# skit-ai/N-Best-ASR-Transformer

Hardware: AMD Instinct MI355X
Metric: utterances/sec fine-tune (bert-base, seq128, n_best=5) (higher is better)
Workload: dtype bf16

## Files before the change

include/nbest_hip.h:

```cpp
#ifndef NBEST_HIP_H
#define NBEST_HIP_H

#include <stddef.h>
#include <stdint.h>

#ifdef __cplusplus
extern "C" {
#endif

#define NBEST_ABI_VERSION 1

enum { NBEST_OK = 0, NBEST_ERR_ARG = -1, NBEST_ERR_SHAPE = -2, NBEST_ERR_DTYPE = -3, NBEST_ERR_ALIGN = -4,
       NBEST_ERR_LAUNCH = -5, NBEST_ERR_WORKSPACE = -6 };
enum { NBEST_F32 = 0, NBEST_BF16 = 1 };

typedef void* nbest_stream_t;

int nbest_version(void);
int nbest_last_error(char* buf, size_t n);

int nbest_embed_ln_fwd(const int64_t* ids, const int64_t* seg, const int64_t* pos, const void* word,
                       const void* type, const void* ptab, const float* gamma, const float* beta, void* out,
                       float* stats, int64_t M, int H, float eps, int dtype, float drop_p, uint64_t seed,
                       uint32_t drop_stream, nbest_stream_t stream);
int nbest_embed_ln_bwd(const int64_t* ids, const int64_t* seg, const int64_t* pos, const int32_t* perm, const void* word,
                       const void* type, const void* ptab, const float* gamma, const float* stats,
                       const void* dout, float* dword, float* dtype_tab, float* dptab, float* dgamma,
                       float* dbeta, int B, int S, int H, int n_types, int dtype, int64_t word_pad_id,
                       int64_t pos_pad_id, int accumulate, int tables_accumulate, float drop_p, uint64_t seed,
                       uint32_t drop_stream, void* ws, size_t ws_bytes, nbest_stream_t stream);
size_t nbest_embed_bwd_ws_bytes(int64_t M, int64_t H);
int nbest_embed_ln_fwd_interp(const int64_t* ids, const int64_t* base_ids, const float* alpha, const int64_t* seg, const int64_t* pos,
                              const void* word, const void* type, const void* ptab, const float* gamma, const float* beta, void* out,
                              float* stats, int B, int S, int H, float eps, int dtype, float drop_p, uint64_t seed, uint32_t drop_stream,
                              nbest_stream_t stream);
int nbest_embed_attrib(const int64_t* ids, const int64_t* base_ids, const float* alpha, const int64_t* seg, const int64_t* pos,
                       const void* word, const void* type, const void* ptab, const float* gamma, const void* dhidden, float* attr,
                       int pairs, int m, int S, int H, float eps, int dtype, nbest_stream_t stream);

int nbest_rows_gather(const float* table, const int64_t* rows, int64_t n_rows, int64_t cap, int64_t* ids_out, float* vals_out, int H,
                      nbest_stream_t stream);
int nbest_rows_zero(float* table, const int64_t* ids, int64_t n, int H, nbest_stream_t stream);
int nbest_rows_add(float* table, const int64_t* ids, const float* vals, int64_t n, int H, nbest_stream_t stream);

enum {
  NBEST_EPI_NONE = 0,
  NBEST_EPI_BIAS = 1,
  NBEST_EPI_BIAS_GELU = 2,
  NBEST_EPI_BIAS_DROP_RES = 3,
  NBEST_EPI_DGELU = 4,
  NBEST_EPI_RES = 5,
  NBEST_EPI_F32_SPLITK = 6
};
typedef struct nbest_gemm_args {
  const void* A;
  const void* B;
  void* C;
  const float* bias;
  const void* R;
  void* U;
  void* ws;
  size_t ws_bytes;
  int64_t M, N, K;
  int64_t lda, ldb, ldc, ldr, ldu;
  int32_t trans_a, trans_b;
  int32_t epilogue;
  int32_t dtype;
  int32_t accumulate;
  float drop_p;
  uint32_t drop_stream;
  uint64_t seed;
  float* colsum_out;
  int32_t colsum_accumulate;
  int32_t flags;
  const void* B_packed;
  int32_t b_pack_bn;
  int32_t pad_;
} nbest_gemm_args;
#define NBEST_GEMM_DEFER_REDUCE 1
size_t nbest_gemm_ws_bytes(const nbest_gemm_args* a);
int nbest_gemm(const nbest_gemm_args* a, nbest_stream_t stream);

size_t nbest_wgrad_pair_ws_bytes(const nbest_gemm_args* a, const nbest_gemm_args* b);
int nbest_wgrad_pair(const nbest_gemm_args* a, const nbest_gemm_args* b, nbest_stream_t stream);

typedef struct nbest_gemm_fp8_args {
  const void* A;
  const void* B;
  void* C;
  const float* bias;
  const void* R;
  void* U;
  void* C8;
  int64_t M, N, K;
  int64_t lda, ldb, ldc, ldr, ldu, ldc8;
  int32_t epilogue;
  float out_scale;
  float drop_p;
  uint32_t drop_stream;
  uint64_t seed;
  const float* out_scale_dev;
  const uint32_t* a_amax;
  const uint32_t* c8_amax_prev;
  uint32_t* c8_amax_new;
  float* colsum_out;
  int32_t colsum_accumulate;
  int32_t pad;
  void* ws;
  size_t ws_bytes;
  const void* B_packed;
  int32_t b_pack_bn;
  int32_t pad3;
} nbest_gemm_fp8_args;
size_t nbest_gemm_fp8_ws_bytes(const nbest_gemm_fp8_args* a);
int nbest_gemm_fp8(const nbest_gemm_fp8_args* a, nbest_stream_t stream);
size_t nbest_wgrad_fp8_ws_bytes(int64_t M, int64_t N, int64_t K);
int nbest_wgrad_fp8(const void* dY8, const void* X8, float* dW, int64_t M, int64_t N, int64_t K, int64_t lda, int64_t ldb,
                    int64_t ldc, const uint32_t* a_amax, const uint32_t* x_amax, int accumulate, void* ws, size_t ws_bytes,
                    nbest_stream_t stream);
size_t nbest_wgrad_fp8_pair_ws_bytes(int64_t Ma, int64_t Mb, int64_t N, int64_t K);
int nbest_wgrad_fp8_pair(const void* dY8a, const void* X8a, float* dWa, int64_t Ma, int64_t lda_a, int64_t ldb_a, int64_t ldc_a,
                         const uint32_t* amax_a, const uint32_t* xamax_a, const void* dY8b, const void* X8b, float* dWb, int64_t Mb,
                         int64_t lda_b, int64_t ldb_b, int64_t ldc_b, const uint32_t* amax_b, const uint32_t* xamax_b, int64_t N, int64_t K,
                         int accumulate, void* ws, size_t ws_bytes, nbest_stream_t stream);
int nbest_cast_bf16_to_fp8(const void* src, void* dst, int64_t n, nbest_stream_t stream);

int nbest_attention_fwd(const void* qkv, const uint8_t* key_mask, void* ctx, float* lse, int B, int S,
                        int heads, int d, int dtype, float drop_p, uint64_t seed, uint32_t drop_stream,
                        nbest_stream_t stream);
int nbest_attention_cls_fwd(const void* q, int64_t ldq, const void* kv, int64_t ldkv, const uint8_t* key_mask, void* ctx,
                            int64_t ldctx, int B, int S, int heads, int d, int dtype, nbest_stream_t stream);
int nbest_attention_probs(const void* qkv, const uint8_t* key_mask, const float* lse, float* probs, int B, int S, int heads, int d,
                          int dtype, nbest_stream_t stream);
int nbest_attention_cls_probs(const void* q, int64_t ldq, const void* kv, int64_t ldkv, const uint8_t* key_mask, float* probs,
                              int64_t ldp, int B, int S, int heads, int d, int dtype, nbest_stream_t stream);
size_t nbest_attention_bwd_ws_bytes(int B, int S, int heads);
int nbest_attention_bwd(const void* qkv, const uint8_t* key_mask, const void* ctx, const void* dctx,
                        const float* lse, void* dqkv, float* dbias, int accumulate, void* ws, size_t ws_bytes,
                        int B, int S, int heads, int d, int dtype, float drop_p, uint64_t seed,
                        uint32_t drop_stream, nbest_stream_t stream);

size_t nbest_attention_keep_bytes(int B, int S, int heads);
int nbest_attention_fwd_keep(const void* qkv, const uint8_t* key_mask, void* ctx, float* lse, int B, int S,
                             int heads, int d, int dtype, float drop_p, uint64_t seed, uint32_t drop_stream,
                             void* keep, nbest_stream_t stream);
int nbest_attention_bwd_keep(const void* qkv, const uint8_t* key_mask, const void* ctx, const void* dctx,
                             const float* lse, void* dqkv, float* dbias, int accumulate, void* ws, size_t ws_bytes,
                             int B, int S, int heads, int d, int dtype, float drop_p, uint64_t seed,
                             uint32_t drop_stream, const void* keep, nbest_stream_t stream);

int nbest_layernorm_fwd(const void* x, const float* gamma, const float* beta, void* y, float* stats,
                        int64_t M, int H, float eps, int dtype, nbest_stream_t stream);
int nbest_layernorm_bwd(const void* dy, const void* x, const float* stats, const float* gamma, void* dx,
                        void* dx_drop, float* dgamma, float* dbeta, float* dbias, int64_t M, int H, int dtype,
                        int accumulate, float drop_p, uint64_t seed, uint32_t drop_stream, void* ws,
                        size_t ws_bytes, nbest_stream_t stream);
size_t nbest_rowred_ws_bytes(int64_t M, int64_t N);
int nbest_colsum(const void* X, float* out, int64_t M, int64_t N, int64_t ld, int dtype, int accumulate,
                 void* ws, size_t ws_bytes, nbest_stream_t stream);

typedef struct nbest_label_space {
  int32_t n_top, n_bottom, n_rows;
  const int32_t* bottom_off;
  const int32_t* bottom_ids;
  const int32_t* head_row;
} nbest_label_space;
size_t nbest_heads_ws_bytes(int B, int R, int H);
int nbest_stc_heads(const void* hidden, int64_t cls_stride, const float* Wh, const float* bh,
                    const nbest_label_space* ls, const float* labels, float* top, float* bott, float* final_scores,
                    float* loss_parts, float* dcls, float* dWh, float* dbh, int B, int H, int dtype,
                    int need_grad, int accumulate, float drop_p, uint64_t seed, uint32_t drop_stream, void* ws,
                    size_t ws_bytes, nbest_stream_t stream);
int nbest_stc_heads_vjp(const float* Wh, const nbest_label_space* ls, const float* top, const float* bott, const float* dtop,
                        const float* dbott, const float* dfin, float* dcls, float* dWh, float* dbh, int B, int H, int accumulate,
                        float drop_p, uint64_t seed, uint32_t drop_stream, void* ws, size_t ws_bytes, nbest_stream_t stream);

int nbest_cls_mse(const void* hidden_a, int64_t stride_a, const void* hidden_t, int64_t stride_t, float* loss,
                  float* da, float* dt, int B, int H, int dtype, float grad_scale, nbest_stream_t stream);

int nbest_cls_grad_scatter(const float* dcls, void* dhidden, int B, int S, int H, int dtype,
                           nbest_stream_t stream);

int nbest_stc_decode(const float* top, const float* bott, const nbest_label_space* ls,
                     const uint8_t* none_flag, int32_t* pred, int B, nbest_stream_t stream);
int nbest_stream_stamp(int32_t* flag, int32_t value, nbest_stream_t stream);

typedef struct nbest_tensor_desc {
  int64_t offset;
  int64_t numel;
  float lr;
  float wd;
  int32_t active;
  int32_t block_start;
} nbest_tensor_desc;
int nbest_bertadam_chunk(void);
int nbest_bertadam_step(float* p, float* g, float* m, float* v, void* p_lowp, const nbest_tensor_desc* descs,
                        int n_tensors, int n_blocks, float lr_mult, float b1, float b2, float eps,
                        float max_grad_norm, void* ws, size_t ws_bytes, nbest_stream_t stream);
int nbest_bertadam_norms(const float* g, const nbest_tensor_desc* descs, int n_tensors, int n_blocks, int blk_lo, int blk_hi,
                         float* partial, nbest_stream_t stream);
int nbest_bertadam_update(float* p, const float* g, float* m, float* v, void* p_lowp, const nbest_tensor_desc* descs,
                          int n_tensors, int n_blocks, int blk_lo, int blk_hi, const float* partial, float* coef,
                          float lr_mult, float b1, float b2, float eps, float max_grad_norm, nbest_stream_t stream);
enum { NBEST_ADAM_L2 = 0, NBEST_ADAMW = 1 };
int nbest_adam_clip_coef(const float* partial, int n_partial, float max_grad_norm, float* clip, nbest_stream_t stream);
int nbest_adam_update(int mode, float* p, const float* g, float* m, float* v, void* p_lowp, const nbest_tensor_desc* descs,
                      int n_tensors, int n_blocks, int blk_lo, int blk_hi, const float* clip, float lr_mult, float bc1,
                      float bc2_sqrt, double b1, double b2, float eps, nbest_stream_t stream);
int nbest_adam_step(int mode, float* p, float* g, float* m, float* v, void* p_lowp, const nbest_tensor_desc* descs,
                    int n_tensors, int n_blocks, float lr_mult, float bc1, float bc2_sqrt, double b1, double b2, float eps,
                    float max_grad_norm, void* ws, size_t ws_bytes, nbest_stream_t stream);
typedef struct nbest_matrix_desc {
  int64_t offset;
  int32_t rows, cols;
  int32_t tile_start, pad;
} nbest_matrix_desc;
#define NBEST_AMAX_TENSOR_WORDS 1024
int nbest_fp8_amax_fold(void* slots, void* out, int32_t n_tensors, nbest_stream_t stream);
int nbest_quantize_weights_fp8(const float* master, void* w8, void* w8t, const nbest_matrix_desc* descs, int n_matrices,
                               int n_tiles, float* inv_scale, void* ws, size_t ws_bytes, nbest_stream_t stream);
int nbest_transpose_weights(const void* src, void* dst, const nbest_matrix_desc* descs, int n_matrices, int n_tiles,
                            nbest_stream_t stream);
int nbest_pack_bn(int64_t N);
int nbest_pack_bn_fp8(int64_t N, int64_t K);
int nbest_pack_weights_fp8(const void* src, void* dst, const nbest_matrix_desc* descs, int n_matrices, int n_stages, nbest_stream_t stream);
int nbest_pack_weights(const void* src, void* dst, const nbest_matrix_desc* descs, int n_matrices, int n_stages, nbest_stream_t stream);
int nbest_cast_f32_to_bf16(const float* src, void* dst, int64_t n, nbest_stream_t stream);

typedef struct nbest_layer_offsets {
  int64_t wqkv, bqkv, wo, bo, ln1_g, ln1_b, w1, b1, w2, b2, ln2_g, ln2_b;
} nbest_layer_offsets;
typedef struct nbest_encoder_desc {
  int32_t dtype, B, S, H, L, heads, F;
  int32_t vocab, max_pos, n_types;
  float ln_eps, hidden_drop, attn_drop;
  int64_t word_pad_id, pos_pad_id;
  int64_t off_word, off_pos, off_type, off_emb_ln_g, off_emb_ln_b;
  const nbest_layer_offsets* layers_host;
  uint64_t seed;
  uint32_t drop_stream_base;
  int32_t wgrad_events_n;
  void** wgrad_events;
  const void* w8;
  const float* w8_inv_scale;
  const void* w8t;
  const uint32_t* gamax_prev;
  uint32_t* gamax_new;
  int32_t fp8_bwd;
  int32_t pad2;
  const void* wpk;
  const void* wpkt;
  const void* w8p;
  const void* w8tp;
  const int32_t* word_perm;
  const uint32_t* aamax_prev;
  uint32_t* aamax_new;
  int32_t fp8_act;
  int32_t pad4;
  int32_t first_trainable;
  int32_t no_input_grad;
  const uint8_t* wgrad_skip_host;
  const int64_t* base_ids;
  const float* alpha;
  int32_t no_param_grad;
  int32_t pad5;
} nbest_encoder_desc;
size_t nbest_encoder_act_bytes(const nbest_encoder_desc* d);
int nbest_encoder_act_view(const nbest_encoder_desc* d, void* act, int layer, void** qkv, float** lse);
size_t nbest_encoder_ws_bytes(const nbest_encoder_desc* d);
int nbest_encoder_wgrad_launches_per_layer(const nbest_encoder_desc* d);
int nbest_encoder_forward(const nbest_encoder_desc* d, const void* wts, const float* prm, const int64_t* ids,
                          const int64_t* seg, const int64_t* pos, const uint8_t* key_mask, void* act,
                          size_t act_bytes, void* ws, size_t ws_bytes, void** hidden_out, nbest_stream_t stream);
int nbest_encoder_backward(const nbest_encoder_desc* d, const void* wts, const void* wts_t, const float* prm, float* grad,
                           const int64_t* ids, const int64_t* seg, const int64_t* pos, const uint8_t* key_mask,
                           void* act, size_t act_bytes, void* dhidden, void* ws, size_t ws_bytes, int accumulate,
                           int layer_begin, int layer_end, int with_embeddings, nbest_stream_t stream);

size_t nbest_encoder_infer_ws_bytes(const nbest_encoder_desc* d);
int nbest_encoder_infer(const nbest_encoder_desc* d, const void* wts, const float* prm, const int64_t* ids, const int64_t* seg,
                        const int64_t* pos, const uint8_t* key_mask, void* ws, size_t ws_bytes, void* cls_out, nbest_stream_t stream);
int nbest_encoder_infer_attn(const nbest_encoder_desc* d, const void* wts, const float* prm, const int64_t* ids, const int64_t* seg,
                             const int64_t* pos, const uint8_t* key_mask, void* ws, size_t ws_bytes, void* cls_out, float* cls_attn,
                             nbest_stream_t stream);

#ifdef __cplusplus
}
#endif
#endif
```

n-best-asr-transformer_amd/csrc/encoder.hip:

```cpp
#include <algorithm>

#include "common.h"

namespace {

static inline size_t al(size_t x) { return (x + 255) & ~(size_t)255; }
static inline size_t take(size_t& o, size_t bytes) { const size_t at = o; o += bytes; return at; }

struct Sizes {
  size_t esz, MH, MF, M3H, MH8, MF8, st, lse;
  int64_t M;
};

static Sizes sizes(const nbest_encoder_desc* d) {
  Sizes z;
  z.esz = d->dtype == NBEST_BF16 ? 2 : 4;
  z.M = (int64_t)d->B * d->S;
  const size_t MHe = (size_t)z.M * d->H, MFe = (size_t)z.M * d->F;
  z.MH = al(MHe * z.esz); z.MF = al(MFe * z.esz); z.M3H = al(3 * MHe * z.esz);
  z.MH8 = al(MHe); z.MF8 = al(MFe);
  z.st = al((size_t)z.M * 2 * sizeof(float));
  z.lse = al((size_t)d->B * d->heads * d->S * sizeof(float));
  return z;
}

struct ActLayout {
  size_t X, emb_stats, layer0, layer_stride;
  size_t o_qkv, o_ctx, o_lse, o_r1, o_st1, o_x1, o_u, o_hact, o_r2, o_st2;
  size_t o_x8, o_ctx8, o_x18, o_h8;
  size_t o_keep, keep_bytes;
  size_t total;
  int K;
};

static int first_trainable(const nbest_encoder_desc* d) { return d->first_trainable < 0 ? 0 : (d->first_trainable > d->L ? d->L : d->first_trainable); }

static ActLayout act_layout(const nbest_encoder_desc* d, const Sizes& z) {
  ActLayout a;
  const bool bf16 = d->dtype == NBEST_BF16;
  a.K = first_trainable(d);
  size_t o = 0, p = 0;
  a.X = take(o, (size_t)(d->L + 1 - a.K) * z.MH);
  a.emb_stats = take(o, a.K ? 0 : z.st);
  a.layer0 = o;
  a.o_qkv = take(p, z.M3H); a.o_ctx = take(p, z.MH); a.o_lse = take(p, z.lse);
  a.o_r1 = take(p, z.MH); a.o_st1 = take(p, z.st); a.o_x1 = take(p, z.MH);
  a.o_u = take(p, bf16 ? z.MF8 : z.MF);
  a.o_hact = take(p, z.MF); a.o_r2 = take(p, z.MH); a.o_st2 = take(p, z.st);
  a.keep_bytes = bf16 ? nbest_internal_attention_keep_bytes(d->B, d->S, d->heads) : 0;
  a.o_keep = take(p, al(a.keep_bytes));
  a.o_x8 = a.o_ctx8 = a.o_x18 = a.o_h8 = 0;
  if (d->w8) {
    a.o_x8 = take(p, z.MH8); a.o_ctx8 = take(p, z.MH8); a.o_x18 = take(p, z.MH8); a.o_h8 = take(p, z.MF8);
  }
  a.layer_stride = p;
  a.total = o + (size_t)(d->L - a.K) * p;
  return a;
}

struct WsLayout {
  size_t dR, dRd, dB1, dctx, dBig, dqkv, red, slab, slab_bytes, red_bytes, emb, emb_bytes, f8, f8_bytes, total;
  size_t fz_x0, fz_x1, fz_emb_stats, fz_lse, fz_st1, fz_st2, fz_u;
};

static nbest_gemm_args wgrad_args(int dtype, int64_t rows, int64_t cols, int64_t tokens) {
  nbest_gemm_args g = {};
  g.M = rows; g.N = cols; g.K = tokens; g.lda = rows; g.ldb = cols; g.ldc = cols;
  g.trans_a = g.trans_b = 1; g.epilogue = NBEST_EPI_F32_SPLITK; g.dtype = dtype;
  return g;
}

static size_t wgrad_pair_bytes(const nbest_encoder_desc* d, bool fp8) {
  const int64_t H = d->H, M = (int64_t)d->B * d->S;
  if (fp8) return nbest_wgrad_fp8_pair_ws_bytes(3 * H, H, H, M);
  const nbest_gemm_args g1 = wgrad_args(NBEST_BF16, 3 * H, H, M), g2 = wgrad_args(NBEST_BF16, H, H, M);
  return nbest_wgrad_pair_ws_bytes(&g1, &g2);
}

static size_t max_splitk_bytes(const nbest_encoder_desc* d, int64_t M) {
  size_t mx = 0;
  const int64_t shapes[4][2] = {{3 * (int64_t)d->H, d->H}, {d->H, d->H}, {d->F, d->H}, {d->H, d->F}};
  for (int i = 0; i < 4; ++i) {
    const nbest_gemm_args g = wgrad_args(d->dtype, shapes[i][0], shapes[i][1], M);
    mx = std::max(mx, nbest_gemm_ws_bytes(&g));
    if (d->dtype == NBEST_BF16 && shapes[i][0] % 256 == 0 && shapes[i][1] % 256 == 0)
      mx = std::max(mx, nbest_wgrad_fp8_ws_bytes(shapes[i][0], shapes[i][1], M));
  }
  if (d->dtype == NBEST_BF16) mx = std::max(mx, std::max(wgrad_pair_bytes(d, false), wgrad_pair_bytes(d, true)));
  return mx;
}

static bool wgrad_paired(const nbest_encoder_desc* d, bool f8b) { return d->dtype == NBEST_BF16 && wgrad_pair_bytes(d, f8b) > 0; }

static WsLayout ws_layout(const nbest_encoder_desc* d, const Sizes& z) {
  WsLayout w;
  const int64_t M = z.M;
  size_t o = 0;
  w.dR = take(o, z.MH); w.dRd = take(o, z.MH); w.dB1 = take(o, z.MH); w.dctx = take(o, z.MH);
  w.dBig = take(o, z.MF); w.dqkv = take(o, z.M3H);
  const int64_t maxN = d->F > 3 * d->H ? d->F : 3 * d->H;
  w.red_bytes = al(nbest_rowred_ws_bytes(M, maxN));
  w.red_bytes = std::max(w.red_bytes, al(nbest_attention_bwd_ws_bytes(d->B, d->S, d->heads)));
  w.red_bytes = std::max(w.red_bytes, al((size_t)((M + 127) / 128) * 2 * d->F * sizeof(float)));
  w.red = take(o, 4 * w.red_bytes);
  w.slab_bytes = al(max_splitk_bytes(d, M));
  w.slab = take(o, w.slab_bytes);
  w.emb_bytes = al(nbest_embed_bwd_ws_bytes(M, d->H));
  w.emb = take(o, w.emb_bytes);
  w.f8_bytes = (d->dtype == NBEST_BF16) ? 4 * z.MH8 + z.MF8 : 0;
  w.f8 = take(o, w.f8_bytes);
  w.fz_x0 = w.fz_x1 = w.fz_emb_stats = w.fz_lse = w.fz_st1 = w.fz_st2 = w.fz_u = o;
  if (first_trainable(d) > 0) {
    w.fz_x0 = take(o, z.MH); w.fz_x1 = take(o, z.MH); w.fz_emb_stats = take(o, z.st);
    w.fz_lse = take(o, z.lse); w.fz_st1 = take(o, z.st); w.fz_st2 = take(o, z.st);
    w.fz_u = take(o, d->w8 ? z.MF8 : 0);
  }
  w.total = o;
  return w;
}

static bool fp8_forward_active(const nbest_encoder_desc* d) {
  return d->dtype == NBEST_BF16 && d->w8 && d->w8_inv_scale && d->fp8_act && d->aamax_prev;
}
static bool fp8_backward_active(const nbest_encoder_desc* d) {
  return fp8_forward_active(d) && d->fp8_bwd && d->w8t && d->gamax_prev && d->gamax_new;
}

static int check_desc(const nbest_encoder_desc* d) {
  NB_CHECK(d && d->layers_host, NBEST_ERR_ARG, "encoder: null descriptor");
  NB_CHECK(d->dtype == NBEST_F32 || d->dtype == NBEST_BF16, NBEST_ERR_DTYPE, "encoder: bad dtype %d", d->dtype);
  NB_CHECK(d->B > 0 && d->S > 0 && d->L > 0 && d->heads > 0, NBEST_ERR_SHAPE, "encoder: bad shape");
  NB_CHECK(d->H == d->heads * 64, NBEST_ERR_SHAPE, "encoder: hidden %d != heads %d x 64", d->H, d->heads);
  NB_CHECK(d->S + (d->pos_pad_id >= 0 ? (int)d->pos_pad_id + 1 : 0) <= d->max_pos, NBEST_ERR_SHAPE,
           "encoder: S=%d does not fit the position table (%d rows)", d->S, d->max_pos);
  NB_CHECK(d->S <= 512, NBEST_ERR_SHAPE, "encoder: S=%d > 512", d->S);
  if (d->dtype == NBEST_BF16)
    NB_CHECK(d->H % 128 == 0 && d->F % 128 == 0, NBEST_ERR_SHAPE, "encoder(bf16): H and F must be multiples of 128");
  if (d->w8) NB_CHECK(d->dtype == NBEST_BF16 && d->w8_inv_scale && d->H % 256 == 0 && d->H <= 1024 && d->F % 256 == 0, NBEST_ERR_SHAPE,
                      "encoder(fp8 forward): needs the bf16 path, inverse scales and H, F multiples of 256");
  NB_CHECK(0 <= d->first_trainable && d->first_trainable <= d->L, NBEST_ERR_ARG, "encoder: first_trainable %d outside [0, L=%d]",
           d->first_trainable, d->L);
  NB_CHECK(!d->base_ids == !d->alpha, NBEST_ERR_ARG, "encoder: interpolated embeddings need both base_ids and alpha (or neither)");
  return NBEST_OK;
}

struct Ptrs {
  const char* wts;
  const float* prm;
  size_t esz;
  const void* W(int64_t off) const { return wts + (size_t)off * esz; }
  const float* P(int64_t off) const { return prm + off; }
};

#define RUN(x) do { int rc__ = (x); if (rc__) return rc__; } while (0)

static nbest_gemm_args gemm_nt(int dtype, const void* A, const void* B, void* C, int64_t M, int64_t N, int64_t K) {
  nbest_gemm_args g = {};
  g.A = A; g.B = B; g.C = C; g.dtype = dtype;
  g.M = M; g.N = N; g.K = K; g.lda = K; g.ldb = K; g.ldc = N;
  return g;
}

static void use_packed(nbest_gemm_args& g, const void* arena, int64_t off) {
  if (!arena || g.dtype != NBEST_BF16 || g.trans_a || g.trans_b) return;
  g.B_packed = (const char*)arena + off * 2;
  g.b_pack_bn = nbest_pack_bn(g.N);
}
static void use_packed(nbest_gemm_fp8_args& g, const void* arena, int64_t off) {
  if (!arena) return;
  g.B_packed = (const uint8_t*)arena + off;
  g.b_pack_bn = nbest_pack_bn_fp8(g.N, g.K);
}

struct GemmPass {
  int dtype; int64_t M; nbest_stream_t stream;
  uint64_t seed;
  Ptrs W; const void* packed; bool b_kn;
  bool fp8; const void *w8, *w8_packed; const float* inv_scale; const uint32_t* amax_prev; uint32_t* amax_new;
  void* colsum_ws; size_t colsum_ws_bytes; int accumulate;
};
struct GemmOp {
  const void* A; const uint8_t* A8; int a_idx;
  int64_t w_off; int mat;
  void* C; int64_t N, K; int epilogue;
  const float* bias;
  const void* R; float drop_p; uint32_t drop_stream;
  void* U; float* colsum;
  uint8_t* C8; int c_idx;
};

static int layer_gemm(const GemmPass& c, const GemmOp& o) {
  if (c.fp8) {
    nbest_gemm_fp8_args g = {};
    g.A = o.A8; g.B = (const uint8_t*)c.w8 + o.w_off; g.C = o.C; g.bias = o.bias; g.R = o.R; g.U = o.U; g.C8 = o.C8;
    g.M = c.M; g.N = o.N; g.K = o.K;
    g.lda = g.ldb = o.K; g.ldc = g.ldr = g.ldu = g.ldc8 = o.N;
    use_packed(g, c.w8_packed, o.w_off);
    g.epilogue = o.epilogue; g.out_scale = 1.f; g.out_scale_dev = c.inv_scale + o.mat;
    g.drop_p = o.drop_p; g.drop_stream = o.drop_stream; g.seed = c.seed;
    g.a_amax = c.amax_prev + o.a_idx;
    if (o.C8) {
      g.c8_amax_prev = c.amax_prev + o.c_idx;
      g.c8_amax_new = c.amax_new ? c.amax_new + (int64_t)o.c_idx * NBEST_AMAX_TENSOR_WORDS : nullptr;
    }
    g.colsum_out = o.colsum; g.colsum_accumulate = c.accumulate; g.ws = c.colsum_ws; g.ws_bytes = c.colsum_ws_bytes;
    return nbest_gemm_fp8(&g, c.stream);
  }
  nbest_gemm_args g = gemm_nt(c.dtype, o.A, c.W.W(o.w_off), o.C, c.M, o.N, o.K);
  if (c.b_kn) { g.trans_b = 1; g.ldb = o.N; }
  g.epilogue = o.epilogue; g.bias = o.bias;
  if (o.R) { g.R = o.R; g.ldr = o.N; }
  if (o.epilogue == NBEST_EPI_BIAS_DROP_RES) { g.drop_p = o.drop_p; g.drop_stream = o.drop_stream; g.seed = c.seed; }
  if (o.epilogue == NBEST_EPI_BIAS_GELU || o.epilogue == NBEST_EPI_DGELU) { g.U = o.U; g.ldu = o.N; }
  if (o.epilogue == NBEST_EPI_DGELU) {
    g.colsum_out = o.colsum; g.colsum_accumulate = g.accumulate = c.accumulate; g.ws = c.colsum_ws; g.ws_bytes = c.colsum_ws_bytes;
  }
  use_packed(g, c.packed, o.w_off);
  return nbest_gemm(&g, c.stream);
}

struct LayerBufs {
  void *qkv, *ctx, *r1, *x1, *u, *hact, *r2;
  float *lse, *st1, *st2;
  uint32_t* keep;
  uint8_t *x8, *ctx8, *x18, *h8;
};

static LayerBufs stashed_layer(const nbest_encoder_desc* d, const ActLayout& a, void* act, int l) {
  char* Lb = (char*)act + a.layer0 + (size_t)(l - a.K) * a.layer_stride;
  LayerBufs b = {};
  b.qkv = Lb + a.o_qkv; b.ctx = Lb + a.o_ctx; b.lse = (float*)(Lb + a.o_lse);
  b.r1 = Lb + a.o_r1; b.st1 = (float*)(Lb + a.o_st1); b.x1 = Lb + a.o_x1;
  b.u = Lb + a.o_u; b.r2 = Lb + a.o_r2; b.st2 = (float*)(Lb + a.o_st2);
  b.hact = fp8_backward_active(d) ? nullptr : Lb + a.o_hact;
  if (a.keep_bytes && d->attn_drop > 0.f) b.keep = (uint32_t*)(Lb + a.o_keep);
  if (fp8_forward_active(d)) {
    b.x8 = (uint8_t*)(Lb + a.o_x8); b.ctx8 = (uint8_t*)(Lb + a.o_ctx8);
    b.x18 = (uint8_t*)(Lb + a.o_x18); b.h8 = (uint8_t*)(Lb + a.o_h8);
  }
  return b;
}

static LayerBufs frozen_layer(const nbest_encoder_desc* d, const WsLayout& w, const Sizes& z, void* ws) {
  char* W = (char*)ws;
  const bool f8 = fp8_forward_active(d);
  LayerBufs b = {};
  b.qkv = W + w.dqkv; b.ctx = W + w.dctx; b.lse = (float*)(W + w.fz_lse);
  b.r1 = W + w.dR; b.st1 = (float*)(W + w.fz_st1); b.x1 = W + w.dRd;
  b.r2 = W + w.dB1; b.st2 = (float*)(W + w.fz_st2);
  b.u = f8 ? W + w.fz_u : nullptr; b.hact = f8 ? nullptr : W + w.dBig;
  if (f8) { b.x8 = (uint8_t*)(W + w.f8); b.ctx8 = b.x8 + z.MH8; b.x18 = b.ctx8 + z.MH8; b.h8 = b.x18 + z.MH8; }
  return b;
}

struct Fwd {
  const nbest_encoder_desc* d;
  GemmPass g;
  const uint8_t* key_mask;
  bool arec;
  const uint32_t* AP(int idx) const { return g.fp8 ? d->aamax_prev + idx : nullptr; }
  uint32_t* AN(int idx) const { return (g.fp8 && arec) ? d->aamax_new + (int64_t)idx * NBEST_AMAX_TENSOR_WORDS : nullptr; }
  int calib(const void* t, int64_t n, int idx) const {
    if (!arec || g.fp8) return NBEST_OK;
    return nbest_internal_amax_bf16(t, n, d->aamax_new + (int64_t)idx * NBEST_AMAX_TENSOR_WORDS, (hipStream_t)g.stream);
  }
};

static Fwd make_fwd(const nbest_encoder_desc* d, const void* wts, const float* prm, const Sizes& z, const uint8_t* key_mask,
                    nbest_stream_t stream) {
  const GemmPass g = {d->dtype, z.M, stream, d->seed, Ptrs{(const char*)wts, prm, z.esz}, d->wpk, false, fp8_forward_active(d),
                      d->w8, d->w8p, d->w8_inv_scale, d->aamax_prev, d->aamax_new, nullptr, 0, 0};
  return Fwd{d, g, key_mask, d->w8 && d->aamax_new && d->dtype == NBEST_BF16};
}

static int layer_forward(const Fwd& c, int l, const void* xin, void* xout, const LayerBufs& b, uint8_t* x8_next, float* cls_probs) {
  const nbest_encoder_desc* d = c.d;
  const nbest_layer_offsets& o = d->layers_host[l];
  const Ptrs& P = c.g.W;
  const nbest_stream_t stream = c.g.stream;
  const int64_t M = c.g.M;
  const int H = d->H, F = d->F, dt = d->dtype, t = 4 * l;
  const uint32_t s0 = d->drop_stream_base + 1 + 4 * l;
  if (c.g.fp8 && l == 0)
    RUN(nbest_internal_cast_bf16_to_fp8(xin, b.x8, M * H, c.AP(0), c.AN(0), (hipStream_t)stream));
  const GemmOp wqkv = {xin, b.x8, t + 0, o.wqkv, t + 0, b.qkv, 3 * H, H, NBEST_EPI_BIAS, P.P(o.bqkv)};
  RUN(layer_gemm(c.g, wqkv));
  if (cls_probs)
    RUN(nbest_internal_attention_cls_probs(b.qkv, (int64_t)d->S * H * 3, (const char*)b.qkv + H * P.esz, 3 * H, c.key_mask, cls_probs, d->S,
                                           d->B, d->S, d->heads, 64, dt, stream));
  RUN(c.calib(xin, M * H, t + 0));
  RUN(nbest_internal_attention_fwd8(b.qkv, c.key_mask, b.ctx, b.ctx8, b.lse, d->B, d->S, d->heads, 64, dt, d->attn_drop, d->seed, s0 + 0,
                                    stream, b.keep, c.AP(t + 1), c.AN(t + 1)));
  RUN(c.calib(b.ctx, M * H, t + 1));
  GemmOp wo = {b.ctx, b.ctx8, t + 1, o.wo, t + 1, b.r1, H, H, NBEST_EPI_BIAS_DROP_RES, P.P(o.bo)};
  wo.R = xin; wo.drop_p = d->hidden_drop; wo.drop_stream = s0 + 1;
  RUN(layer_gemm(c.g, wo));
  RUN(nbest_internal_layernorm_fwd8(b.r1, P.P(o.ln1_g), P.P(o.ln1_b), b.x1, b.x18, b.st1, M, H, d->ln_eps, dt, stream, c.AP(t + 2), c.AN(t + 2)));
  RUN(c.calib(b.x1, M * H, t + 2));
  GemmOp w1 = {b.x1, b.x18, t + 2, o.w1, t + 2, b.hact, F, H, NBEST_EPI_BIAS_GELU, P.P(o.b1)};
  w1.U = b.u; w1.C8 = b.h8; w1.c_idx = t + 3;
  RUN(layer_gemm(c.g, w1));
  GemmOp w2 = {b.hact, b.h8, t + 3, o.w2, t + 3, b.r2, H, F, NBEST_EPI_BIAS_DROP_RES, P.P(o.b2)};
  w2.R = b.x1; w2.drop_p = d->hidden_drop; w2.drop_stream = s0 + 2;
  RUN(layer_gemm(c.g, w2));
  RUN(c.calib(b.hact, M * F, t + 3));
  RUN(nbest_internal_layernorm_fwd8(b.r2, P.P(o.ln2_g), P.P(o.ln2_b), xout, x8_next, b.st2, M, H, d->ln_eps, dt, stream,
                                    x8_next ? c.AP(t + 4) : nullptr, x8_next ? c.AN(t + 4) : nullptr));
  return NBEST_OK;
}

}

extern "C" size_t nbest_encoder_act_bytes(const nbest_encoder_desc* d) { return d ? act_layout(d, sizes(d)).total : 0; }

extern "C" int nbest_encoder_act_view(const nbest_encoder_desc* d, void* act, int layer, void** qkv, float** lse) {
  RUN(check_desc(d));
  NB_CHECK(act && qkv && lse, NBEST_ERR_ARG, "encoder_act_view: null pointer");
  NB_CHECK(0 <= layer && layer < d->L, NBEST_ERR_ARG, "encoder_act_view: layer %d outside [0, L=%d)", layer, d->L);
  const ActLayout a = act_layout(d, sizes(d));
  NB_CHECK(layer >= a.K, NBEST_ERR_ARG, "encoder_act_view: layer %d < first_trainable %d (frozen layers are not stashed)", layer, a.K);
  const LayerBufs b = stashed_layer(d, a, act, layer);
  *qkv = b.qkv; *lse = b.lse;
  return NBEST_OK;
}
extern "C" size_t nbest_encoder_ws_bytes(const nbest_encoder_desc* d) { return d ? ws_layout(d, sizes(d)).total : 0; }
extern "C" int nbest_encoder_wgrad_launches_per_layer(const nbest_encoder_desc* d) {
  return d ? (wgrad_paired(d, fp8_backward_active(d)) ? 3 : 4) : 0;
}

extern "C" int nbest_encoder_forward(const nbest_encoder_desc* d, const void* wts, const float* prm, const int64_t* ids,
                                     const int64_t* seg, const int64_t* pos, const uint8_t* key_mask, void* act, size_t act_bytes,
                                     void* ws, size_t ws_bytes, void** hidden_out, nbest_stream_t stream) {
  RUN(check_desc(d));
  NB_CHECK(wts && prm && ids && pos && key_mask && act, NBEST_ERR_ARG, "encoder_forward: null pointer");
  const Sizes z = sizes(d);
  const ActLayout a = act_layout(d, z);
  NB_CHECK(act_bytes >= a.total, NBEST_ERR_WORKSPACE, "encoder_forward: activation stash too small (%zu < %zu)", act_bytes, a.total);
  const Fwd c = make_fwd(d, wts, prm, z, key_mask, stream);
  const WsLayout wl = ws_layout(d, z);
  const int FT = a.K;
  if (c.g.fp8 || FT > 0)
    NB_CHECK(ws && ws_bytes >= wl.total, NBEST_ERR_WORKSPACE, "encoder_forward(%s): workspace too small (%zu < %zu)",
             FT > 0 ? "first_trainable > 0" : "fp8", ws_bytes, wl.total);
  const Ptrs& P = c.g.W;
  char *A = (char*)act, *W = (char*)ws;
  const int H = d->H, dt = d->dtype;
  auto X = [&](int l) { return l >= FT ? (void*)(A + a.X + (size_t)(l - FT) * z.MH) : (void*)(W + ((l & 1) ? wl.fz_x1 : wl.fz_x0)); };
  auto bufs = [&](int l) { return l >= FT ? stashed_layer(d, a, act, l) : frozen_layer(d, wl, z, ws); };

  float* emb_stats = (float*)(FT > 0 ? W + wl.fz_emb_stats : A + a.emb_stats);
  if (d->base_ids)
    RUN(nbest_embed_ln_fwd_interp(ids, d->base_ids, d->alpha, seg, pos, P.W(d->off_word), P.W(d->off_type), P.W(d->off_pos),
                                  P.P(d->off_emb_ln_g), P.P(d->off_emb_ln_b), X(0), emb_stats, d->B, d->S, H, d->ln_eps, dt,
                                  d->hidden_drop, d->seed, d->drop_stream_base, (hipStream_t)stream));
  else
    RUN(nbest_embed_ln_fwd(ids, seg, pos, P.W(d->off_word), P.W(d->off_type), P.W(d->off_pos), P.P(d->off_emb_ln_g),
                           P.P(d->off_emb_ln_b), X(0), emb_stats, z.M, H, d->ln_eps, dt, d->hidden_drop, d->seed, d->drop_stream_base,
                           (hipStream_t)stream));
  for (int l = 0; l < d->L; ++l) {
    uint8_t* x8_next = (l + 1 < d->L) ? bufs(l + 1).x8 : nullptr;
    RUN(layer_forward(c, l, X(l), X(l + 1), bufs(l), x8_next, nullptr));
  }
  if (hidden_out) *hidden_out = X(d->L);
  return NBEST_OK;
}

namespace {
struct WGrad {
  const void *dY, *X;
  const uint8_t *dY8, *X8;
  int64_t w_off, rows, cols;
  int g_idx, a_idx;
};
}

extern "C" int nbest_encoder_backward(const nbest_encoder_desc* d, const void* wts, const void* wts_t, const float* prm, float* grad,
                                      const int64_t* ids, const int64_t* seg, const int64_t* pos, const uint8_t* key_mask,
                                      void* act, size_t act_bytes, void* dhidden, void* ws, size_t ws_bytes, int accumulate,
                                      int layer_begin, int layer_end, int with_embeddings, nbest_stream_t stream) {
  RUN(check_desc(d));
  NB_CHECK(0 <= layer_begin && layer_begin <= layer_end && layer_end <= d->L, NBEST_ERR_ARG, "encoder_backward: bad layer range");
  const bool npg = d->no_param_grad != 0;
  NB_CHECK(!npg || (!with_embeddings && d->first_trainable == 0 && !d->no_input_grad && !d->w8), NBEST_ERR_ARG,
           "encoder_backward: no_param_grad refuses with_embeddings (%d), first_trainable > 0 (%d), no_input_grad (%d) and the fp8 "
           "forward (w8): it forms the input gradient only, of a full stash", with_embeddings, d->first_trainable, d->no_input_grad);
  NB_CHECK(wts && prm && (grad || npg) && ids && pos && key_mask && act && dhidden && ws, NBEST_ERR_ARG, "encoder_backward: null pointer");
  NB_CHECK(!with_embeddings || d->word_perm, NBEST_ERR_ARG, "encoder_backward: desc.word_perm (stable argsort of this pass's ids) is required");
  NB_CHECK(layer_begin >= d->first_trainable, NBEST_ERR_ARG, "encoder_backward: layer_begin %d < first_trainable %d (those layers are not stashed)",
           layer_begin, d->first_trainable);
  NB_CHECK(!with_embeddings || (d->first_trainable == 0 && !d->no_input_grad), NBEST_ERR_ARG,
           "encoder_backward: with_embeddings needs first_trainable == 0 and no_input_grad == 0");
  const Sizes z = sizes(d);
  const ActLayout a = act_layout(d, z);
  const WsLayout w = ws_layout(d, z);
  NB_CHECK(act_bytes >= a.total, NBEST_ERR_WORKSPACE, "encoder_backward: activation stash too small");
  NB_CHECK(ws_bytes >= w.total, NBEST_ERR_WORKSPACE, "encoder_backward: workspace too small (%zu < %zu)", ws_bytes, w.total);
  hipStream_t st = (hipStream_t)stream;
  const Ptrs P{(const char*)wts, prm, z.esz};
  const bool wt = (wts_t != nullptr);
  char *A = (char*)act, *W = (char*)ws;
  const int64_t M = z.M;
  const int H = d->H, F = d->F, dt = d->dtype;
  const int FT = a.K;
  auto X = [&](int l) { return (void*)(A + a.X + (size_t)(l - FT) * z.MH); };
  auto G = [&](int64_t off) { return grad + off; };
  auto GP = [&](int64_t off) -> float* { return npg ? nullptr : grad + off; };
  auto skip = [&](int l, int j) -> bool { return npg || (d->wgrad_skip_host && d->wgrad_skip_host[4 * l + j]); };
  void* dA = dhidden; void* dR = W + w.dR;
  const bool hdrop = d->hidden_drop > 0.f;
  void* dRd = hdrop ? (void*)(W + w.dRd) : dR;
  void* dB1 = W + w.dB1; void* dctx = W + w.dctx; void* dBig = W + w.dBig; void* dqkv = W + w.dqkv;
  void* red = W + w.red; void* slab = W + w.slab;
  void* red1 = W + w.red + w.red_bytes; void* red2 = W + w.red + 2 * w.red_bytes; void* red3 = W + w.red + 3 * w.red_bytes;
  const bool f8b = fp8_backward_active(d);
  const bool paired = wgrad_paired(d, f8b);
  int ev_i = (paired ? 3 : 4) * (d->L - layer_end);
  auto stamp = [&](int which) {
    if (d->wgrad_events && 2 * ev_i + which < d->wgrad_events_n) (void)hipEventRecord((hipEvent_t)d->wgrad_events[2 * ev_i + which], st);
    ev_i += which;
  };

  const bool rec = !npg && d->gamax_new && dt == NBEST_BF16;
  uint8_t* dqkv8 = f8b ? (uint8_t*)W + w.f8 : nullptr;
  uint8_t* dBig8 = f8b ? dqkv8 + 3 * z.MH8 : nullptr;
  uint8_t* dRd8 = f8b ? dBig8 + z.MF8 : nullptr;
  auto GN = [&](int idx) { return d->gamax_new + (int64_t)idx * NBEST_AMAX_TENSOR_WORDS; };
  auto fg = [&](uint8_t* out8, int idx) -> Fp8Grad {
    if (!rec) return Fp8Grad{nullptr, nullptr, nullptr};
    return Fp8Grad{f8b ? out8 : nullptr, f8b ? d->gamax_prev + idx : nullptr, GN(idx)};
  };
  const GemmPass dg = {dt, M, stream, 0, Ptrs{(const char*)(wt ? wts_t : wts), prm, z.esz}, wt ? d->wpkt : nullptr, !wt, f8b,
                       d->w8t, d->w8tp, d->w8_inv_scale, d->gamax_prev, d->gamax_new, red1, w.red_bytes, accumulate};
  auto wgrad = [&](int l, const WGrad* wg, int j, int j2) -> int {
    const WGrad* p = skip(l, j) ? nullptr : wg + j;
    const WGrad* q = (j2 >= 0 && !skip(l, j2)) ? wg + j2 : nullptr;
    if (!p) { p = q; q = nullptr; }
    stamp(0);
    if (p && f8b) {
      const uint32_t *gp = d->gamax_prev, *ap = d->aamax_prev;
      if (q)
        RUN(nbest_wgrad_fp8_pair(p->dY8, p->X8, G(p->w_off), p->rows, p->rows, p->cols, p->cols, gp + p->g_idx, ap + p->a_idx, q->dY8, q->X8,
                                 G(q->w_off), q->rows, q->rows, q->cols, q->cols, gp + q->g_idx, ap + q->a_idx, p->cols, M, accumulate, slab,
                                 w.slab_bytes, stream));
      else
        RUN(nbest_wgrad_fp8(p->dY8, p->X8, G(p->w_off), p->rows, p->cols, M, p->rows, p->cols, p->cols, gp + p->g_idx, ap + p->a_idx,
                            accumulate, slab, w.slab_bytes, stream));
    } else if (p) {
      auto args = [&](const WGrad* x) {
        nbest_gemm_args g = wgrad_args(dt, x->rows, x->cols, M);
        g.A = x->dY; g.B = x->X; g.C = G(x->w_off); g.accumulate = accumulate;
        return g;
      };
      nbest_gemm_args g1 = args(p), g2 = args(q ? q : p);
      g1.ws = slab; g1.ws_bytes = w.slab_bytes;
      RUN(q ? nbest_wgrad_pair(&g1, &g2, stream) : nbest_gemm(&g1, stream));
    }
    stamp(1);
    return NBEST_OK;
  };

  struct BatchGuard { ~BatchGuard() { nbest_internal_rowred_batch_abort(); } } batch_guard;
  for (int l = layer_end - 1; l >= layer_begin; --l) {
    const nbest_layer_offsets& o = d->layers_host[l];
    const LayerBufs b = stashed_layer(d, a, act, l);
    const bool input_grad = !(d->no_input_grad && l == FT);
    const int t = 4 * l;
    const uint32_t s0 = d->drop_stream_base + 1 + 4 * l;
    const WGrad wg[4] = {{dqkv, X(l), dqkv8, b.x8, o.wqkv, 3 * H, H, t + 3, t + 0},
                         {dRd, b.ctx, dRd8, b.ctx8, o.wo, H, H, t + 2, t + 1},
                         {dBig, b.x1, dBig8, b.x18, o.w1, F, H, t + 1, t + 2},
                         {dRd, b.hact, dRd8, b.h8, o.w2, H, F, t + 0, t + 3}};
    if (!npg) nbest_internal_rowred_batch_begin();
    RUN(nbest_internal_layernorm_bwd8(dA, b.r2, b.st2, P.P(o.ln2_g), dR, (hdrop && !f8b) ? dRd : nullptr, GP(o.ln2_g), GP(o.ln2_b), GP(o.b2), M, H,
                                      dt, accumulate, d->hidden_drop, d->seed, s0 + 2, red, w.red_bytes, stream, fg(dRd8, t + 0)));
    GemmOp dw2 = {dRd, dRd8, t + 0, o.w2, t + 3, f8b ? nullptr : dBig, F, H, NBEST_EPI_DGELU};
    dw2.U = b.u; dw2.colsum = GP(o.b1); dw2.C8 = dBig8; dw2.c_idx = t + 1;
    RUN(layer_gemm(dg, dw2));
    if (rec && !f8b) RUN(nbest_internal_amax_bf16(dBig, M * F, GN(t + 1), st));
    RUN(wgrad(l, wg, 3, -1));
    GemmOp dw1 = {dBig, dBig8, t + 1, o.w1, t + 2, dB1, H, F, NBEST_EPI_RES};
    dw1.R = dR;
    RUN(layer_gemm(dg, dw1));
    RUN(wgrad(l, wg, 2, -1));
    RUN(nbest_internal_layernorm_bwd8(dB1, b.r1, b.st1, P.P(o.ln1_g), dR, (hdrop && !f8b) ? dRd : nullptr, GP(o.ln1_g), GP(o.ln1_b), GP(o.bo), M, H,
                                      dt, accumulate, d->hidden_drop, d->seed, s0 + 1, red2, w.red_bytes, stream, fg(dRd8, t + 2)));
    const GemmOp dwo = {dRd, dRd8, t + 2, o.wo, t + 1, dctx, H, H, NBEST_EPI_NONE};
    RUN(layer_gemm(dg, dwo));
    if (!paired) RUN(wgrad(l, wg, 1, -1));
    RUN(nbest_internal_attention_bwd8(b.qkv, key_mask, b.ctx, dctx, b.lse, f8b ? nullptr : dqkv, GP(o.bqkv), accumulate, red3, w.red_bytes, d->B, d->S,
                                      d->heads, 64, dt, d->attn_drop, d->seed, s0 + 0, stream, fg(dqkv8, t + 3), b.keep));
    if (input_grad) {
      GemmOp dwqkv = {dqkv, dqkv8, t + 3, o.wqkv, t + 0, dA, H, 3 * H, NBEST_EPI_RES};
      dwqkv.R = dR;
      RUN(layer_gemm(dg, dwqkv));
    }
    RUN(wgrad(l, wg, 0, paired ? 1 : -1));
    if (!npg) RUN(nbest_internal_rowred_batch_flush(st));
  }
  if (!with_embeddings) return NBEST_OK;
  if (!accumulate) {
    hipError_t e = hipMemsetAsync(G(d->off_word), 0, (size_t)d->vocab * H * sizeof(float), st);
    if (e == hipSuccess) e = hipMemsetAsync(G(d->off_pos), 0, (size_t)d->max_pos * H * sizeof(float), st);
    if (e == hipSuccess) e = hipMemsetAsync(G(d->off_type), 0, (size_t)d->n_types * H * sizeof(float), st);
    NB_CHECK(e == hipSuccess, NBEST_ERR_LAUNCH, "encoder_backward: memset failed: %s", hipGetErrorString(e));
  }
  RUN(nbest_embed_ln_bwd(ids, seg, pos, d->word_perm, P.W(d->off_word), P.W(d->off_type), P.W(d->off_pos), P.P(d->off_emb_ln_g),
                         (const float*)(A + a.emb_stats), dA, G(d->off_word), G(d->off_type), G(d->off_pos), G(d->off_emb_ln_g),
                         G(d->off_emb_ln_b), d->B, d->S, H, d->n_types, dt, d->word_pad_id, d->pos_pad_id, accumulate, accumulate,
                         d->hidden_drop, d->seed, d->drop_stream_base, W + w.emb, w.emb_bytes, stream));
  return NBEST_OK;
}

namespace {
struct InferLayout {
  size_t X0, X1, emb_stats, qkv, ctx, r1, x1, r2, hact, lse, st1, st2, total;
};
static InferLayout infer_layout(const Sizes& z) {
  InferLayout w;
  size_t o = 0;
  w.X0 = take(o, z.MH); w.X1 = take(o, z.MH); w.emb_stats = take(o, z.st);
  w.qkv = take(o, z.M3H); w.ctx = take(o, z.MH); w.r1 = take(o, z.MH); w.x1 = take(o, z.MH); w.r2 = take(o, z.MH);
  w.hact = take(o, z.MF); w.lse = take(o, z.lse); w.st1 = take(o, z.st); w.st2 = take(o, z.st);
  w.total = o;
  return w;
}
static LayerBufs infer_layer(const InferLayout& w, void* ws) {
  char* W = (char*)ws;
  LayerBufs b = {};
  b.qkv = W + w.qkv; b.ctx = W + w.ctx; b.lse = (float*)(W + w.lse);
  b.r1 = W + w.r1; b.st1 = (float*)(W + w.st1); b.x1 = W + w.x1;
  b.hact = W + w.hact; b.r2 = W + w.r2; b.st2 = (float*)(W + w.st2);
  return b;
}
}

extern "C" size_t nbest_encoder_infer_ws_bytes(const nbest_encoder_desc* d) { return d ? infer_layout(sizes(d)).total : 0; }

extern "C" int nbest_encoder_infer_attn(const nbest_encoder_desc* d, const void* wts, const float* prm, const int64_t* ids, const int64_t* seg,
                                        const int64_t* pos, const uint8_t* key_mask, void* ws, size_t ws_bytes, void* cls_out,
                                        float* cls_attn, nbest_stream_t stream) {
  RUN(check_desc(d));
  NB_CHECK(d->hidden_drop == 0.f && d->attn_drop == 0.f, NBEST_ERR_ARG,
           "encoder_infer: dropout must be 0 (hidden_drop=%g, attn_drop=%g): inference has no dropout", d->hidden_drop, d->attn_drop);
  NB_CHECK(!d->w8, NBEST_ERR_ARG, "encoder_infer: the fp8 forward (desc.w8) is not supported; pass the bf16 weights without w8");
  NB_CHECK(!d->base_ids && !d->alpha, NBEST_ERR_ARG, "encoder_infer: interpolated embeddings (desc.base_ids / alpha) are not supported; "
                                                     "run nbest_encoder_forward");
  NB_CHECK(wts && prm && ids && pos && key_mask && ws && cls_out, NBEST_ERR_ARG, "encoder_infer: null pointer");
  const Sizes z = sizes(d);
  const InferLayout w = infer_layout(z);
  NB_CHECK(ws_bytes >= w.total, NBEST_ERR_WORKSPACE, "encoder_infer: workspace too small (%zu < %zu)", ws_bytes, w.total);
  const Fwd c = make_fwd(d, wts, prm, z, key_mask, stream);
  const Ptrs& P = c.g.W;
  char* W = (char*)ws;
  const int64_t M = z.M, B = d->B, SH = (int64_t)d->S * d->H;
  const int H = d->H, F = d->F, dt = d->dtype;
  void* X[2] = {W + w.X0, W + w.X1};
  const LayerBufs b = infer_layer(w, ws);
  auto probs = [&](int l) { return cls_attn ? cls_attn + (int64_t)l * B * d->heads * d->S : nullptr; };

  RUN(nbest_embed_ln_fwd(ids, seg, pos, P.W(d->off_word), P.W(d->off_type), P.W(d->off_pos), P.P(d->off_emb_ln_g), P.P(d->off_emb_ln_b),
                         X[0], (float*)(W + w.emb_stats), M, H, d->ln_eps, dt, d->hidden_drop, d->seed, d->drop_stream_base,
                         (hipStream_t)stream));
  for (int l = 0; l + 1 < d->L; ++l) RUN(layer_forward(c, l, X[l & 1], X[(l + 1) & 1], b, nullptr, probs(l)));
  const int l = d->L - 1;
  const nbest_layer_offsets& o = d->layers_host[l];
  const void* xin = X[l & 1];
  void* kv = b.qkv; void* q = b.ctx; void* cctx = b.r1; void* cx1 = b.x1; void* ch = b.hact; void* cr = b.r2;
  nbest_gemm_args g = gemm_nt(dt, xin, P.W(o.wqkv + (int64_t)H * H), kv, M, 2 * H, H);
  g.epilogue = NBEST_EPI_BIAS; g.bias = P.P(o.bqkv + H);
  RUN(nbest_gemm(&g, stream));
  g = gemm_nt(dt, xin, P.W(o.wqkv), q, B, H, H);
  g.lda = SH; g.epilogue = NBEST_EPI_BIAS; g.bias = P.P(o.bqkv);
  RUN(nbest_gemm(&g, stream));
  if (cls_attn) RUN(nbest_internal_attention_cls_probs(q, H, kv, 2 * H, key_mask, probs(l), d->S, d->B, d->S, d->heads, 64, dt, stream));
  RUN(nbest_attention_cls_fwd_internal(q, H, kv, 2 * H, key_mask, cctx, H, d->B, d->S, d->heads, 64, dt, stream));
  g = gemm_nt(dt, cctx, P.W(o.wo), cr, B, H, H);
  g.epilogue = NBEST_EPI_BIAS_DROP_RES; g.bias = P.P(o.bo); g.R = xin; g.ldr = SH;
  RUN(nbest_gemm(&g, stream));
  RUN(nbest_internal_layernorm_fwd8(cr, P.P(o.ln1_g), P.P(o.ln1_b), cx1, nullptr, b.st1, B, H, d->ln_eps, dt, stream, nullptr, nullptr));
  g = gemm_nt(dt, cx1, P.W(o.w1), ch, B, F, H);
  g.epilogue = NBEST_EPI_BIAS_GELU; g.bias = P.P(o.b1); g.ldu = F;
  RUN(nbest_gemm(&g, stream));
  g = gemm_nt(dt, ch, P.W(o.w2), cr, B, H, F);
  g.epilogue = NBEST_EPI_BIAS_DROP_RES; g.bias = P.P(o.b2); g.R = cx1; g.ldr = H;
  RUN(nbest_gemm(&g, stream));
  RUN(nbest_internal_layernorm_fwd8(cr, P.P(o.ln2_g), P.P(o.ln2_b), cls_out, nullptr, b.st2, B, H, d->ln_eps, dt, stream, nullptr, nullptr));
  return NBEST_OK;
}

extern "C" int nbest_encoder_infer(const nbest_encoder_desc* d, const void* wts, const float* prm, const int64_t* ids, const int64_t* seg,
                                   const int64_t* pos, const uint8_t* key_mask, void* ws, size_t ws_bytes, void* cls_out,
                                   nbest_stream_t stream) {
  return nbest_encoder_infer_attn(d, wts, prm, ids, seg, pos, key_mask, ws, ws_bytes, cls_out, nullptr, stream);
}
```

n-best-asr-transformer_amd/csrc/gemm.hip:

```cpp
#include "common.h"

namespace {

__global__ __launch_bounds__(256) void splitk_reduce_kernel(const float* __restrict__ slab, float* __restrict__ C, int64_t MN,
                                                            int64_t N, int64_t ldc, int splits, int accumulate,
                                                            float* __restrict__ C2, int64_t m_split, int64_t ldc2) {
  for (int64_t i = ((int64_t)blockIdx.x * blockDim.x + threadIdx.x) * 4; i < MN; i += (int64_t)gridDim.x * blockDim.x * 4) {
    f32x4 s = *(const f32x4*)(slab + i);
    for (int z = 1; z < splits; ++z) s += *(const f32x4*)(slab + (int64_t)z * MN + i);
    const int64_t m = i / N, n = i - m * N;
    float* c = (m < m_split) ? C + m * ldc + n : C2 + (m - m_split) * ldc2 + n;
    if (accumulate) s += *(const f32x4*)c;
    *(f32x4*)c = s;
  }
}

int check_epilogue_operands(const nbest_gemm_args* a, int64_t ld_mult, uintptr_t align) {
  const int epi = a->epilogue;
  if (epi == NBEST_EPI_BIAS || epi == NBEST_EPI_BIAS_GELU || epi == NBEST_EPI_BIAS_DROP_RES)
    NB_CHECK(a->bias, NBEST_ERR_ARG, "gemm: epilogue %d needs bias", epi);
  if (epi == NBEST_EPI_BIAS_DROP_RES || epi == NBEST_EPI_RES)
    NB_CHECK(a->R && a->ldr % ld_mult == 0 && ((uintptr_t)a->R & (align - 1)) == 0, NBEST_ERR_ARG, "gemm: epilogue %d needs R", epi);
  if ((epi == NBEST_EPI_BIAS_GELU && a->U) || epi == NBEST_EPI_DGELU)
    NB_CHECK(a->U && a->ldu % ld_mult == 0 && ((uintptr_t)a->U & (align - 1)) == 0, NBEST_ERR_ARG, "gemm: epilogue %d needs U", epi);
  return NBEST_OK;
}

int check_bf16(const nbest_gemm_args* a) {
  NB_CHECK(!(a->trans_a && !a->trans_b), NBEST_ERR_ARG, "gemm(bf16): trans_a without trans_b is not built");
  NB_CHECK(!a->trans_a || a->M % 128 == 0, NBEST_ERR_SHAPE, "gemm(bf16): trans_a needs M %% 128 == 0");
  NB_CHECK(a->lda % 8 == 0 && a->ldb % 8 == 0 && a->ldc % 8 == 0, NBEST_ERR_ALIGN, "gemm(bf16): leading dimensions must be multiples of 8");
  NB_CHECK(((uintptr_t)a->A & 15) == 0 && ((uintptr_t)a->B & 15) == 0 && ((uintptr_t)a->C & 15) == 0, NBEST_ERR_ALIGN,
           "gemm(bf16): pointers must be 16-byte aligned");
  const int64_t a_rows = a->trans_a ? a->K : a->M, a_cols = a->trans_a ? a->M : a->K;
  const int64_t b_rows = a->trans_b ? a->K : a->N, b_cols = a->trans_b ? a->N : a->K;
  const int64_t ab = ((a_rows - 1) * a->lda + a_cols) * 2, bb = ((b_rows - 1) * a->ldb + b_cols) * 2;
  NB_CHECK(ab < ((int64_t)1 << 32) && bb < ((int64_t)1 << 32), NBEST_ERR_SHAPE, "gemm(bf16): operand larger than 4 GiB");
  NB_CHECK(a->M * a->N < ((int64_t)1 << 32) || make_drop(a->drop_p, a->seed, a->drop_stream).thr16 == 0, NBEST_ERR_SHAPE,
           "gemm(bf16): dropout counter overflow");
  return check_epilogue_operands(a, 8, 16);
}

}

void nb_splitk_plan(int64_t tiles, int64_t K, int64_t slots, int64_t min_blocks, int* splits, int64_t* k_per_split) {
  const int64_t maxs = (K / 512 < 1) ? 1 : ((K / 512 > 32) ? 32 : K / 512);
  int64_t best_s = 1;
  double best = -1.0;
  for (int64_t s = 1; s <= maxs; ++s) {
    const int64_t blocks = tiles * s;
    const double eff = (double)blocks / (double)(((blocks + slots - 1) / slots) * slots);
    if (eff > best + 1e-9) { best = eff; best_s = s; }
    if (blocks >= min_blocks && eff >= 0.93) { best_s = s; break; }
  }
  const int64_t k = round_up((K + best_s - 1) / best_s, 64);
  *splits = (int)((K + k - 1) / k);
  *k_per_split = k;
}

int nbest_internal_splitk_reduce(const float* slab, float* C, int64_t M, int64_t N, int64_t ldc, int splits, int accumulate,
                                 float* C2, int64_t m_split, int64_t ldc2, hipStream_t st) {
  const int64_t MN = M * N;
  int64_t g = (MN / 4 + 255) / 256;
  if (g > 2048) g = 2048;
  splitk_reduce_kernel<<<(int)g, 256, 0, st>>>(slab, C, MN, N, ldc, splits, accumulate, C2, m_split, ldc2);
  NB_LAUNCH_CHECK();
  return NBEST_OK;
}

extern "C" size_t nbest_gemm_ws_bytes(const nbest_gemm_args* a) {
  if (!a) return 0;
  if (a->dtype == NBEST_F32) return (a->colsum_out && a->epilogue != NBEST_EPI_F32_SPLITK) ? nbest_rowred_ws_bytes(a->M, a->N) : 0;
  if (a->dtype != NBEST_BF16) return 0;
  const size_t w1 = nbest_gemm_bf16_ws_bytes(a), w2 = nbest_gemm_bf16_v2_ws_bytes(a);
  return w1 > w2 ? w1 : w2;
}

extern "C" int nbest_gemm(const nbest_gemm_args* a, nbest_stream_t stream) {
  NB_CHECK(a && a->A && a->B && a->C, NBEST_ERR_ARG, "gemm: null pointer");
  NB_CHECK(a->M > 0 && a->N > 0 && a->K > 0, NBEST_ERR_SHAPE, "gemm: bad shape %lld x %lld x %lld", (long long)a->M,
           (long long)a->N, (long long)a->K);
  if (a->dtype == NBEST_F32) {
    if (int rc = check_epilogue_operands(a, 1, 1)) return rc;
    if (int rc = nbest_gemm_f32(a, (hipStream_t)stream)) return rc;
    if (a->colsum_out && a->epilogue != NBEST_EPI_F32_SPLITK) {
      NB_CHECK(a->ws && a->ws_bytes >= nbest_rowred_ws_bytes(a->M, a->N), NBEST_ERR_WORKSPACE, "gemm(f32): column-sum workspace too small");
      return nbest_colsum(a->C, a->colsum_out, a->M, a->N, a->ldc, NBEST_F32, a->colsum_accumulate, a->ws, a->ws_bytes, stream);
    }
    return NBEST_OK;
  }
  if (a->dtype == NBEST_BF16) {
    if (int rc = check_bf16(a)) return rc;
    return nbest_gemm_bf16_v2_wins(a) ? nbest_gemm_bf16_v2(a, (hipStream_t)stream) : nbest_gemm_bf16(a, (hipStream_t)stream);
  }
  nbest_set_error("gemm: bad dtype %d", a->dtype);
  return NBEST_ERR_DTYPE;
}

extern "C" int nbest_pack_bn(int64_t N) { return nbest_pack_bn_internal(N); }
extern "C" int nbest_pack_weights(const void* src, void* dst, const nbest_matrix_desc* descs, int n_matrices, int n_stages,
                                  nbest_stream_t stream) {
  NB_CHECK(src && dst && descs && n_matrices > 0 && n_stages > 0 && src != dst, NBEST_ERR_ARG, "pack_weights: bad arguments");
  return nbest_pack_weights_bf16(src, dst, descs, n_matrices, n_stages, (hipStream_t)stream);
}

extern "C" size_t nbest_wgrad_pair_ws_bytes(const nbest_gemm_args* a, const nbest_gemm_args* b) {
  if (!a || !b) return 0;
  return nbest_wgrad_pair_bf16_ws_bytes(a, b);
}

extern "C" int nbest_wgrad_pair(const nbest_gemm_args* a, const nbest_gemm_args* b, nbest_stream_t stream) {
  NB_CHECK(a && b && a->A && a->B && a->C && b->A && b->B && b->C, NBEST_ERR_ARG, "wgrad_pair: null pointer");
  NB_CHECK(a->M > 0 && b->M > 0 && a->N > 0 && a->K > 0, NBEST_ERR_SHAPE, "wgrad_pair: bad shape");
  NB_CHECK(nbest_wgrad_pair_bf16_ws_bytes(a, b) > 0, NBEST_ERR_SHAPE,
           "wgrad_pair: needs two bf16 F32_SPLITK problems (trans_a = trans_b = 1) with equal N, K and accumulate, M1, M2, N multiples of 256 "
           "and at least 18 output tiles in all");
  if (int rc = check_bf16(a)) return rc;
  if (int rc = check_bf16(b)) return rc;
  return nbest_wgrad_pair_bf16(a, b, (hipStream_t)stream);
}
```

n-best-asr-transformer_amd/csrc/gemm_bf16_v2.hip:

```cpp
#include "common.h"
#include <type_traits>

namespace {

constexpr int BK = 32;

struct GemmP2 {
  const bf16* A; const bf16* B; void* C; const float* bias; const bf16* R; bf16* U; float* slab; float* colpart;
  int64_t M, N, K, lda, ldb, ldc, ldr, ldu;
  int64_t k_per_split;
  int tiles_m, tiles_n, splits, accumulate;
  uint32_t a_bytes, b_bytes;
  uint32_t c_bytes, r_bytes, u_bytes;
  DropCfg drop;
  int stream_out;
  int gn;
  const bf16* A2; const bf16* B2;
  int64_t lda2, ldb2, m_split;
  uint32_t a2_bytes, b2_bytes;
  const bf16* Bp;
  uint32_t bp_bytes;
  int bp_bn;
};

// ... 29 lines not shown
    __builtin_amdgcn_raw_ptr_buffer_load_lds(rs, LDS_PTR(dst), 16, voff, 0, 0, 0);
  }
}

template <int ROWS, int NT>
__device__ __forceinline__ void stage_tile_packed(__amdgpu_buffer_rsrc_t rs, char* tile, uint32_t stage_byte0, int tid, char* dump = nullptr) {
  const int wave = tid >> 6;
  constexpr int NI = (ROWS * 4 + NT - 1) / NT;
#pragma unroll
  for (int i = 0; i < NI; ++i) {
    uint32_t voff = stage_byte0 + (uint32_t)(i * NT + tid) * 16u;
    char* dst = tile + (i * NT + wave * 64) * 16;
    if constexpr ((ROWS * 4) % NT != 0) {
      if (i == NI - 1 && (i * NT + wave * 64) * 16 >= ROWS * 64) {
        voff = 0xFFFFFFF0u;
        dst = dump + (wave % (NT / 64)) * 1024;
      }
    }
    __builtin_amdgcn_raw_ptr_buffer_load_lds(rs, LDS_PTR(dst), 16, voff, 0, 0, 0);
  }
}

__device__ __forceinline__ void wait_vm_even(int n) {
  switch (n) {
    case 0: asm volatile("s_waitcnt vmcnt(0)" ::: "memory"); break;
    case 2: asm volatile("s_waitcnt vmcnt(2)" ::: "memory"); break;
    case 4: asm volatile("s_waitcnt vmcnt(4)" ::: "memory"); break;
    case 6: asm volatile("s_waitcnt vmcnt(6)" ::: "memory"); break;
    case 8: asm volatile("s_waitcnt vmcnt(8)" ::: "memory"); break;
    case 10: asm volatile("s_waitcnt vmcnt(10)" ::: "memory"); break;
    default: asm volatile("s_waitcnt vmcnt(12)" ::: "memory"); break;
  }
}

__device__ __forceinline__ bf16x4 ds_read_tr_asm(const char* addr) {
  bf16x4 v;
  const uint32_t a = (uint32_t)(uintptr_t)(const __attribute__((address_space(3))) char*)addr;
  asm volatile("ds_read_b64_tr_b16 %0, %1" : "=v"(v) : "v"(a) : "memory");
  return v;
}

template <bool TR, int ROWS, bool ASM = false>
__device__ __forceinline__ bf16x8 read_frag2(const char* tile, int row_base, int lane) {
  if (!TR) {
    const int row = row_base + (lane & 15);
    const int kc = lane >> 4;
    return *(const bf16x8*)(tile + row * 64 + ((kc ^ ((-(row >> 2)) & 3)) << 4));
  } else {
    const int g = lane >> 4, i = lane & 15, q = i >> 2, pq = i & 3;
    const int col = row_base + 4 * pq;
    bf16x8 out;
#pragma unroll
    for (int half = 0; half < 2; ++half) {
      const int krow = 8 * g + 4 * half + q;
      const int f = 2 * (krow & 3) + 8 * ((krow >> 3) & 1);
      const char* addr = tile + krow * (ROWS * 2) + (((col >> 3) ^ f) << 4) + ((col & 4) ? 8 : 0);
      const bf16x4 v = ASM ? ds_read_tr_asm(addr)
                           : __builtin_amdgcn_ds_read_tr16_b64_v4bf16((bf16x4 __attribute__((address_space(3)))*)addr);
      out[4 * half + 0] = v[0]; out[4 * half + 1] = v[1]; out[4 * half + 2] = v[2]; out[4 * half + 3] = v[3];
    }
    return out;
  }
}

template <int N> __device__ __forceinline__ void wait_vm() {
  static_assert(N >= 0 && N <= 63, "vmcnt is a 6-bit field");
  asm volatile("s_waitcnt vmcnt(%0)" ::"n"(N) : "memory");
}

template <int NB_, int STAGE, int A_BYTES, int NIA, int NIB, int NT, int BN>
__device__ __forceinline__ void pp_issue(__amdgpu_buffer_rsrc_t rsA, __amdgpu_buffer_rsrc_t rsB, char* lds, const uint32_t* voA,
                                         const uint32_t* voB, int wv, bool dumpB, char* dump, uint32_t sA, uint32_t sB) {
#pragma unroll
  for (int i = 0; i < NIA; ++i)
    __builtin_amdgcn_raw_ptr_buffer_load_lds(rsA, LDS_PTR(lds + NB_ * STAGE + (i * NT + wv * 64) * 16), 16, voA[i], sA, 0, 0);
#pragma unroll
  for (int i = 0; i < NIB; ++i) {
    char* dst = lds + NB_ * STAGE + A_BYTES + (i * NT + wv * 64) * 16;
    const bool d = ((BN * 4) % NT != 0) && i == NIB - 1 && dumpB;
    if (d) dst = dump;
    __builtin_amdgcn_raw_ptr_buffer_load_lds(rsB, LDS_PTR(dst), 16, voB[i], d ? 0u : sB, 0, 0);
  }
}
template <int B_, int STAGE, int A_BYTES, int BM, int BN, int TMt, int TNt>
__device__ __forceinline__ void pp_frags(const char* lds, bf16x8* af, bf16x8* bfr, int row0, int col0, int lane) {
  const char* cur = lds + B_ * STAGE;
#pragma unroll
  for (int j = 0; j < TNt; ++j) bfr[j] = read_frag2<false, BN>(cur + A_BYTES, col0 + j * 16, lane);
#pragma unroll
  for (int i = 0; i < TMt; ++i) af[i] = read_frag2<false, BM>(cur, row0 + i * 16, lane);
}
template <int TMt, int TNt>
__device__ __forceinline__ void pp_mfma_slot(const bf16x8* af, const bf16x8* bfr, f32x4 (&acc)[TMt][TNt]) {
  __builtin_amdgcn_sched_barrier(0);
  __builtin_amdgcn_s_barrier();
  __builtin_amdgcn_sched_barrier(0);
  __builtin_amdgcn_s_setprio(1);
#pragma unroll
  for (int i = 0; i < TMt; ++i)
#pragma unroll
    for (int j = 0; j < TNt; ++j) acc[i][j] = __builtin_amdgcn_mfma_f32_16x16x32_bf16(af[i], bfr[j], acc[i][j], 0, 0, 0);
  __builtin_amdgcn_s_setprio(0);
  __builtin_amdgcn_sched_barrier(0);
  __builtin_amdgcn_s_barrier();
  __builtin_amdgcn_sched_barrier(0);
}

template <int OFF> __device__ __forceinline__ bf16x4 ds_read_tr_off(uint32_t a) {
  bf16x4 v;
  asm volatile("ds_read_b64_tr_b16 %0, %1 offset:%2" : "=v"(v) : "v"(a), "n"(OFF) : "memory");
  return v;
}
template <int B_, int STAGES, int NF>
__device__ __forceinline__ void tt_frags(const uint32_t* base, bf16x8* fr) {
  constexpr int HALF = 2 * STAGES * 1024;
#pragma unroll
  for (int t = 0; t < NF; ++t) {
    const bf16x4 lo = ds_read_tr_off<B_ * 1024>(base[t]);
    const bf16x4 hi = ds_read_tr_off<B_ * 1024 + HALF>(base[t]);
    fr[t] = bf16x8{lo[0], lo[1], lo[2], lo[3], hi[0], hi[1], hi[2], hi[3]};
  }
}
template <int NB_, int STAGES>
__device__ __forceinline__ void tt_issue(__amdgpu_buffer_rsrc_t rsA, __amdgpu_buffer_rsrc_t rsB, char* ldsA, char* ldsB, const uint32_t* voA,
                                         const uint32_t* voB, int wv) {
#pragma unroll
  for (int i = 0; i < 2; ++i)
    __builtin_amdgcn_raw_ptr_buffer_load_lds(rsA, LDS_PTR(ldsA + ((i * 8 + wv) * STAGES + NB_) * 1024), 16, voA[i], 0, 0, 0);
#pragma unroll
  for (int i = 0; i < 2; ++i)
    __builtin_amdgcn_raw_ptr_buffer_load_lds(rsB, LDS_PTR(ldsB + ((i * 8 + wv) * STAGES + NB_) * 1024), 16, voB[i], 0, 0, 0);
}
template <int TMt, int TNt>
__device__ __forceinline__ void tt_frags_ready(bf16x8* af, bf16x8* bfr) {
  asm volatile("s_waitcnt lgkmcnt(0)" ::: "memory");
#pragma unroll
  for (int i = 0; i < TMt; ++i) asm volatile("" : "+v"(af[i]));
#pragma unroll
  for (int j = 0; j < TNt; ++j) asm volatile("" : "+v"(bfr[j]));
}
template <int TMt, int TNt>
__device__ __forceinline__ void tt_mfma(const bf16x8* af, const bf16x8* bfr, f32x4 (&acc)[TMt][TNt]) {
  __builtin_amdgcn_sched_barrier(0);
  __builtin_amdgcn_s_setprio(1);
#pragma unroll
  for (int i = 0; i < TMt; ++i)
#pragma unroll
    for (int j = 0; j < TNt; ++j) acc[i][j] = __builtin_amdgcn_mfma_f32_16x16x32_bf16(bfr[j], af[i], acc[i][j], 0, 0, 0);
  __builtin_amdgcn_s_setprio(0);
  __builtin_amdgcn_sched_barrier(0);
}

template <int BM, int BN, int WM, int WN, int STAGES, bool TA, bool TB, int EPI>
__global__ __launch_bounds__(WM * WN * 64, 2) void gemm2_kernel(GemmP2 p) {
  extern __shared__ __attribute__((aligned(16))) char lds[];
  constexpr int NT = WM * WN * 64;
  constexpr int WTM = BM / WM, WTN = BN / WN;
  constexpr int TMt = WTM / 16, TNt = WTN / 16;
  constexpr bool kDirect = (!TA && !TB && EPI != NBEST_EPI_F32_SPLITK);
  constexpr int kPW = kDirect ? WTN : 0;
  static_assert(kDirect ? (WTN == 64 || WTN == 96 || WTN == 128) : WTN == 64, "LDS-restaged epilogue assumes 64-column wave tiles");
  static_assert(TNt != 6 || (EPI != NBEST_EPI_BIAS_GELU && EPI != kEpiBiasGeluNoU && EPI != NBEST_EPI_DGELU), "96-column wave tiles: no GELU epilogues (8-bit rows)");
  constexpr int A_BYTES = BM * BK * 2, B_BYTES = BN * BK * 2, STAGE = A_BYTES + B_BYTES;
  constexpr int NDMA = (BM * 4 + NT - 1) / NT + (BN * 4 + NT - 1) / NT;
  const int tid = threadIdx.x, lane = tid & 63, wave = tid >> 6;
  const int wm = wave / WN, wn = wave % WN;

  const int nwg = gridDim.x;
  const int id = xcd_remap(blockIdx.x, nwg);
  const int tiles = p.tiles_m * p.tiles_n;
  const int z = id / tiles, t = id - z * tiles;
  int tile_m, tile_n;
  nb_tile_coords(t, p.tiles_m, p.gn, tile_m, tile_n);
  const int64_t m0 = (int64_t)tile_m * BM, n0 = (int64_t)tile_n * BN;
  const int64_t kbeg = (int64_t)z * p.k_per_split;
  const int64_t kend = (kbeg + p.k_per_split < p.K) ? kbeg + p.k_per_split : p.K;
  const int nk = (int)((kend - kbeg + BK - 1) / BK);

  const bf16* opA = p.A; const bf16* opB = p.B;
  int64_t lda_ = p.lda, ldb_ = p.ldb, m0a = m0;
  uint32_t a_bytes = p.a_bytes, b_bytes = p.b_bytes;
  if constexpr (TA && TB && EPI == NBEST_EPI_F32_SPLITK) {
    if (p.m_split > 0 && m0 >= p.m_split) {
      opA = p.A2; opB = p.B2; lda_ = p.lda2; ldb_ = p.ldb2; m0a = m0 - p.m_split; a_bytes = p.a2_bytes; b_bytes = p.b2_bytes;
    }
  }
  const __amdgpu_buffer_rsrc_t rsA = __builtin_amdgcn_make_buffer_rsrc((void*)opA, 0, a_bytes, 0x00020000);
  const bool b_packed = kDirect && NT == 512 && p.Bp != nullptr;
  const __amdgpu_buffer_rsrc_t rsB = __builtin_amdgcn_make_buffer_rsrc(b_packed ? (void*)p.Bp : (void*)opB, 0, b_packed ? p.bp_bytes : b_bytes, 0x00020000);
  const int nkt = (int)(p.K / BK);

  constexpr bool kHasBias = (EPI == NBEST_EPI_BIAS || EPI == NBEST_EPI_BIAS_GELU || EPI == kEpiBiasGeluNoU || EPI == NBEST_EPI_BIAS_DROP_RES);
  constexpr bool kHasR = (EPI == NBEST_EPI_BIAS_DROP_RES || EPI == NBEST_EPI_RES);
  constexpr bool kHasUin = (EPI == NBEST_EPI_DGELU);
  constexpr bool kPre = kHasR || kHasUin;
  const int64_t en8 = n0 + wn * WTN + (lane & 7) * 8;
  const int64_t erow0 = m0 + wm * WTM + (lane >> 3);
  auto load_pre = [&](int64_t m) -> i32x4 {
    if constexpr (kHasR) {
      return (m < p.M) ? *(const i32x4*)(p.R + m * p.ldr + en8) : i32x4{0, 0, 0, 0};
    } else {
      const i32x2 q = (m < p.M) ? *(const i32x2*)((const uint8_t*)p.U + m * p.ldu + en8) : i32x2{0, 0};
      return i32x4{q[0], q[1], 0, 0};
    }
  };
  f32x4 pb0 = {0, 0, 0, 0}, pb1 = {0, 0, 0, 0};
  if (kHasBias && !kDirect) { pb0 = *(const f32x4*)(p.bias + en8); pb1 = *(const f32x4*)(p.bias + en8 + 4); }
  i32x4 pre[TMt / 2][4];
  if (kPre && !kDirect) {
#pragma unroll
    for (int it = 0; it < 4; ++it) pre[0][it] = load_pre(erow0 + it * 8);
  }
  const int dg = lane >> 4, dc = lane & 15;
  const int64_t dcol = n0 + wn * WTN + TNt * dc;
  const int64_t drow0 = m0 + wm * WTM + 4 * dg;
  float db[TNt];
  u32x4 dpre[TMt][4];
  const __amdgpu_buffer_rsrc_t rsC = __builtin_amdgcn_make_buffer_rsrc(p.C, 0, p.c_bytes, 0x00020000);
  const __amdgpu_buffer_rsrc_t rsR = __builtin_amdgcn_make_buffer_rsrc((void*)p.R, 0, p.r_bytes, 0x00020000);
  const __amdgpu_buffer_rsrc_t rsU = __builtin_amdgcn_make_buffer_rsrc((void*)p.U, 0, p.u_bytes, 0x00020000);
  const uint32_t voR = (uint32_t)((drow0 * p.ldr + dcol) * 2), voU = (uint32_t)(drow0 * p.ldu + dcol);
  const uint32_t svR = (uint32_t)(2 * p.ldr), svU = (uint32_t)p.ldu;
  auto load_dpre = [&](int i) {
#pragma unroll
    for (int e = 0; e < 4; ++e) {
      const uint32_t rr = (uint32_t)(16 * i + e);
      if constexpr (kHasR) {
        if constexpr (TNt == 8) dpre[i][e] = __builtin_amdgcn_raw_buffer_load_b128(rsR, voR + rr * svR, 0, 0);
        else if constexpr (TNt == 6) { const u32x3 q = __builtin_amdgcn_raw_buffer_load_b96(rsR, voR + rr * svR, 0, 0); dpre[i][e] = u32x4{q[0], q[1], q[2], 0}; }
        else { const u32x2 q = __builtin_amdgcn_raw_buffer_load_b64(rsR, voR + rr * svR, 0, 0); dpre[i][e] = u32x4{q[0], q[1], 0, 0}; }
      } else if constexpr (kHasUin) {
        if constexpr (TNt == 8) { const u32x2 q = __builtin_amdgcn_raw_buffer_load_b64(rsU, voU + rr * svU, 0, 0); dpre[i][e] = u32x4{q[0], q[1], 0, 0}; }
        else dpre[i][e] = u32x4{__builtin_amdgcn_raw_buffer_load_b32(rsU, voU + rr * svU, 0, 0), 0, 0, 0};
      }
    }
  };
  auto load_bias = [&]() {
    if (kHasBias) {
#pragma unroll
      for (int q = 0; q < TNt / 2; ++q) {
        const f32x2 b2 = *(const f32x2*)(p.bias + dcol + 2 * q);
        db[2 * q] = b2[0]; db[2 * q + 1] = b2[1];
      }
    }
  };
  if constexpr (kDirect) {
    load_bias();
    if (kHasR || kHasUin) load_dpre(0);
  }

  f32x4 acc[TMt][TNt];
#pragma unroll
  for (int i = 0; i < TMt; ++i)
#pragma unroll
    for (int j = 0; j < TNt; ++j) acc[i][j] = f32x4{0, 0, 0, 0};

  if constexpr (NT == 512 && kDirect) {
    const int wv = __builtin_amdgcn_readfirstlane(wave);
    const int grp = wv >> 2;
    constexpr int NIA = (BM * 4) / NT, NIB = (BN * 4 + NT - 1) / NT;
    static_assert((BM * 4) % NT == 0, "A tile: whole LDS-DMA instructions");
    uint32_t voA[NIA], voB[NIB];
#pragma unroll
    for (int i = 0; i < NIA; ++i) {
      const int pp = i * NT + tid, row = pp >> 2, slot = pp & 3, kc = slot ^ ((-(row >> 2)) & 3);
      voA[i] = (uint32_t)(((m0a + row) * lda_ + kc * 8) * 2);
    }
    bool dumpB = false;
#pragma unroll
    for (int i = 0; i < NIB; ++i) {
      const int pp = i * NT + tid;
      if (b_packed) {
        const int per = p.bp_bn * 4;
        const int blk = pp / per;
        voB[i] = (uint32_t)blk * (uint32_t)nkt * (uint32_t)(per * 16) + (uint32_t)(pp - blk * per) * 16u;
      } else {
        const int row = pp >> 2, slot = pp & 3, kc = slot ^ ((-(row >> 2)) & 3);
        int grow = row;
        if constexpr (kPW > 0) { const int x = row % kPW; grow = row - x + (kPW / 16) * (x & 15) + (x >> 4); }
        voB[i] = (uint32_t)(((n0 + grow) * ldb_ + kc * 8) * 2);
      }
      if ((BN * 4) % NT != 0 && i == NIB - 1 && (i * NT + wv * 64) * 16 >= BN * 64) { voB[i] = 0xFFFFFFF0u; dumpB = true; }
    }
    const uint32_t sB0 = b_packed ? (uint32_t)(tile_n * nkt) * (uint32_t)B_BYTES : (uint32_t)(kbeg * 2);
    const uint32_t sBstep = b_packed ? (uint32_t)(p.bp_bn * BK * 2) : (uint32_t)(BK * 2);
    char* const dump = lds + STAGES * STAGE + (wv % (NT / 64)) * 1024;
    bf16x8 af[TMt], bfr[TNt];
    const uint32_t sA0 = (uint32_t)(kbeg * 2);
#define PP_ISSUE(ST, NB_) pp_issue<(NB_), STAGE, A_BYTES, NIA, NIB, NT, BN>(rsA, rsB, lds, voA, voB, wv, dumpB, dump, sA0 + (uint32_t)(ST) * (uint32_t)(BK * 2), sB0 + (uint32_t)(ST) * sBstep)
#define PP_FRAGS(B_) pp_frags<(B_), STAGE, A_BYTES, BM, BN, TMt, TNt>(lds, af, bfr, wm * WTM, wn * WTN, lane)
#define PP_MFMA() pp_mfma_slot<TMt, TNt>(af, bfr, acc)
#define PP_STEADY(KT, B_)                                  \
    do {                                                   \
      PP_ISSUE((KT) + STAGES - 1, ((B_) + STAGES - 1) % STAGES); \
      PP_FRAGS(B_);                                        \
      wait_vm<(STAGES - 2) * NDMA>();                      \
      PP_MFMA();                                           \
    } while (0)
#define PP_GENERIC(KT, B_)                                                                          \
    do {                                                                                            \
      if ((KT) + STAGES - 1 < nk) PP_ISSUE((KT) + STAGES - 1, ((B_) + STAGES - 1) % STAGES);        \
      PP_FRAGS(B_);                                                                                 \
      const int c_ = (nk - 1 - (KT) < STAGES - 1) ? nk - 1 - (KT) : STAGES - 1;                     \
      if (STAGES >= 5 && c_ >= 4) wait_vm<3 * NDMA>();                                              \
      else if (c_ >= 3) wait_vm<2 * NDMA>();                                                        \
      else if (c_ == 2) wait_vm<NDMA>();                                                            \
      else if (c_ == 1) wait_vm<0>();                                                               \
      PP_MFMA();                                                                                    \
    } while (0)
    if (0 < nk) PP_ISSUE(0, 0);
    if (1 < nk) PP_ISSUE(1, 1 % STAGES);
    if (STAGES > 3 && 2 < nk) PP_ISSUE(2, 2 % STAGES);
    if (STAGES > 4 && 3 < nk) PP_ISSUE(3, 3 % STAGES);
    {
      const int younger = (nk - 1 < STAGES - 2) ? nk - 1 : STAGES - 2;
      if (STAGES >= 5 && younger >= 3) wait_vm<3 * NDMA>();
      else if (younger >= 2) wait_vm<2 * NDMA>();
      else if (younger == 1) wait_vm<NDMA>();
      else wait_vm<0>();
    }
    __builtin_amdgcn_s_barrier();
    asm volatile("" ::: "memory");
// ... 286 lines not shown
          for (int j = 0; j < TNt; ++j) v[j] = (k >> j & 1) ? v[j] * p.drop.scale : 0.f;
        }
        if (kHasR) {
          const bf16x8 r8 = __builtin_bit_cast(bf16x8, dpre[i][e]);
#pragma unroll
          for (int j = 0; j < TNt; ++j) v[j] += (float)r8[j];
        }
        if (kHasUin) {
          float gd[8];
          gd_unpack4(dpre[i][e][0], gd);
          if constexpr (TNt == 8) gd_unpack4(dpre[i][e][1], gd + 4);
#pragma unroll
          for (int j = 0; j < TNt; ++j) v[j] *= gd[j];
        }
        if constexpr (TNt == 8) nb_bstore_bf16x8(rsC, voC + rr * svC, v);
        else if constexpr (TNt == 6) {
          bf16x2 o0 = {(bf16)v[0], (bf16)v[1]}, o1 = {(bf16)v[2], (bf16)v[3]}, o2 = {(bf16)v[4], (bf16)v[5]};
          __builtin_amdgcn_raw_buffer_store_b96(u32x3{__builtin_bit_cast(uint32_t, o0), __builtin_bit_cast(uint32_t, o1), __builtin_bit_cast(uint32_t, o2)},
                                                rsC, voC + rr * svC, 0, 2);
        } else {
          bf16x4 o;
#pragma unroll
          for (int j = 0; j < 4; ++j) o[j] = (bf16)v[j];
          __builtin_amdgcn_raw_buffer_store_b64(__builtin_bit_cast(u32x2, o), rsC, voC + rr * svC, 0, 2);
        }
        if constexpr (kCols) {
          const bool live = want_cols && (drow0 + rr) < p.M;
#pragma unroll
          for (int j = 0; j < TNt; ++j) colacc[j] += live ? v[j] : 0.f;
        }
      }
    }
    if (kCols && want_cols) {
#pragma unroll
      for (int j = 0; j < TNt; ++j) {
        float x = colacc[j];
        x += __shfl_xor(x, 16, 64); x += __shfl_xor(x, 32, 64);
        colacc[j] = x;
      }
      if (dg == 0) {
        float* o = p.colpart + ((int64_t)tile_m * WM + wm) * p.N + dcol;
#pragma unroll
        for (int q = 0; q < TNt / 2; ++q) *(f32x2*)(o + 2 * q) = f32x2{colacc[2 * q], colacc[2 * q + 1]};
      }
    }
    return;
  }
  float* ep = (float*)lds + wave * 2048;
  float colacc[8] = {0, 0, 0, 0, 0, 0, 0, 0};
  if (kPre) {
#pragma unroll
    for (int c = 1; c < TMt / 2; ++c)
#pragma unroll
      for (int it = 0; it < 4; ++it) pre[c][it] = load_pre(erow0 + c * 32 + it * 8);
  }
  __builtin_amdgcn_s_barrier();
  asm volatile("" ::: "memory");
  int64_t oC = erow0 * p.ldc + en8, oU = erow0 * p.ldu + en8;
  int64_t oS = ((int64_t)z * p.M + erow0) * p.N + en8;
  const int64_t sC = 8 * p.ldc, sU = 8 * p.ldu, sS = 8 * p.N;
  uint32_t dbase = (uint32_t)(erow0 * p.N + en8);
  const uint32_t sD = 8u * (uint32_t)p.N;
#pragma unroll
  for (int c = 0; c < TMt / 2; ++c) {
#pragma unroll
    for (int ii = 0; ii < 2; ++ii) {
      const int row = ii * 16 + (lane & 15);
#pragma unroll
      for (int j = 0; j < TNt; ++j) {
        const int cidx = j * 4 + (lane >> 4);
        *(f32x4*)(ep + row * 64 + ((cidx ^ (row & 15)) << 2)) = acc[2 * c + ii][j];
      }
    }
    asm volatile("s_waitcnt lgkmcnt(0)" ::: "memory");
#pragma unroll
    for (int it = 0; it < 4; ++it) {
      const int pidx = it * 64 + lane, row = pidx >> 3, c8 = pidx & 7;
      const int64_t m = m0 + wm * WTM + c * 32 + row;
      f32x4 v0 = *(const f32x4*)(ep + row * 64 + (((2 * c8) ^ (row & 15)) << 2));
      f32x4 v1 = *(const f32x4*)(ep + row * 64 + (((2 * c8 + 1) ^ (row & 15)) << 2));
      if (m < p.M) {
      if (EPI == NBEST_EPI_F32_SPLITK) {
        float* cp = (p.splits > 1) ? p.slab + oS : (float*)p.C + oC;
        if (p.splits == 1 && p.accumulate) { v0 += *(const f32x4*)cp; v1 += *(const f32x4*)(cp + 4); }
        *(f32x4*)cp = v0;
        *(f32x4*)(cp + 4) = v1;
      } else {
      float v[8] = {v0[0], v0[1], v0[2], v0[3], v1[0], v1[1], v1[2], v1[3]};
      if (kHasBias) {
#pragma unroll
        for (int e = 0; e < 4; ++e) { v[e] += pb0[e]; v[4 + e] += pb1[e]; }
      }
      if (EPI == kEpiBiasGeluNoU) {
#pragma unroll
        for (int e = 0; e < 8; e += 2) {
          f32x2 h2, g2;
          gelu_pair_fast(f32x2{v[e], v[e + 1]}, h2, g2);
          v[e] = h2[0]; v[e + 1] = h2[1];
        }
      }
      if (EPI == NBEST_EPI_BIAS_GELU) {
        float gp[8];
#pragma unroll
        for (int e = 0; e < 8; e += 2) {
          f32x2 h2, g2;
          gelu_pair_fast(f32x2{v[e], v[e + 1]}, h2, g2);
          gp[e] = g2[0]; gp[e + 1] = g2[1]; v[e] = h2[0]; v[e + 1] = h2[1];
        }
        st_stream((i32x2*)((uint8_t*)p.U + oU), i32x2{(int)gd_pack4(gp), (int)gd_pack4(gp + 4)}, p.stream_out);
      }
      if (EPI == NBEST_EPI_BIAS_DROP_RES && p.drop.thr16) {
        const uint32_t k = nb_keep4(p.drop, dbase) | (nb_keep4(p.drop, dbase + 4) << 4);
#pragma unroll
        for (int e = 0; e < 8; ++e) v[e] = (k >> e & 1) ? v[e] * p.drop.scale : 0.f;
      }
      if (kHasR) {
        const bf16x8 r = __builtin_bit_cast(bf16x8, pre[c][it]);
#pragma unroll
        for (int e = 0; e < 8; ++e) v[e] += (float)r[e];
      }
      if (kHasUin) {
        float gd[8];
        gd_unpack4((uint32_t)pre[c][it][0], gd);
        gd_unpack4((uint32_t)pre[c][it][1], gd + 4);
#pragma unroll
        for (int e = 0; e < 8; ++e) v[e] *= gd[e];
      }
      st_stream_bf16x8((bf16*)p.C + oC, v, p.stream_out);
      if (EPI != NBEST_EPI_F32_SPLITK && p.colpart) {
#pragma unroll
        for (int e = 0; e < 8; ++e) colacc[e] += v[e];
      }
      }
      }
      oC += sC; oU += sU; oS += sS; dbase += sD;
    }
    asm volatile("" ::: "memory");
  }
  if (EPI != NBEST_EPI_F32_SPLITK && p.colpart) {
#pragma unroll
    for (int e = 0; e < 8; ++e) {
      float x = colacc[e];
      x += __shfl_xor(x, 8, 64); x += __shfl_xor(x, 16, 64); x += __shfl_xor(x, 32, 64);
      colacc[e] = x;
    }
    if ((lane >> 3) == 0) {
      float* o = p.colpart + ((int64_t)tile_m * WM + wm) * p.N + en8;
      *(f32x4*)o = f32x4{colacc[0], colacc[1], colacc[2], colacc[3]};
      *(f32x4*)(o + 4) = f32x4{colacc[4], colacc[5], colacc[6], colacc[7]};
    }
  }
}

__global__ __launch_bounds__(256) void pack_b_kernel(const bf16* __restrict__ src, bf16* __restrict__ dst,
                                                     const nbest_matrix_desc* __restrict__ descs, int n) {
  int lo = 0, hi = n - 1;
  while (lo < hi) {
    const int mid = (lo + hi + 1) >> 1;
    if (descs[mid].tile_start <= (int)blockIdx.x) lo = mid; else hi = mid - 1;
  }
  const nbest_matrix_desc d = descs[lo];
  const int bn = d.pad, pw = (bn == 256) ? 128 : 96;
  const int nk = d.cols / BK, t = blockIdx.x - d.tile_start, tile_n = t / nk, kt = t - tile_n * nk;
  const bf16* s = src + d.offset + ((int64_t)tile_n * bn) * d.cols + (int64_t)kt * BK;
  bf16* o = dst + d.offset + ((int64_t)tile_n * nk + kt) * bn * BK;
  for (int p = threadIdx.x; p < bn * 4; p += blockDim.x) {
    const int row = p >> 2, slot = p & 3;
    const int kc = slot ^ ((-(row >> 2)) & 3);
    const int x = row % pw;
    const int grow = row - x + (pw / 16) * (x & 15) + (x >> 4);
    *(i32x4*)(o + (int64_t)p * 8) = *(const i32x4*)(s + (int64_t)grow * d.cols + kc * 8);
  }
}

struct Plan {
  int bm, bn, splits;
  int64_t kps;
};

static Plan make_plan(const nbest_gemm_args* a) {
  Plan pl;
  pl.bn = 128;
  const int64_t t256 = ((a->M + 255) / 256) * (a->N / 128);
  pl.bm = (!a->trans_a && t256 >= 1024) ? 256 : 128;
  const bool ok256 = (a->N % 256 == 0) && (!a->trans_a || a->M % 256 == 0);
  if (!a->trans_a && !a->trans_b && a->N % 256 == 0 &&
      [&] {
        const int64_t t = ((a->M + 255) / 256) * (a->N / 256);
        return t >= 1024 || (t >= 256 && (double)t / (double)(((t + 255) / 256) * 256) >= 0.85);
      }()) {
    pl.bm = 256; pl.bn = 256;
  } else if (a->trans_a && a->trans_b && a->epilogue == NBEST_EPI_F32_SPLITK && ok256 && (a->M / 256) * (a->N / 256) >= 18) {
    pl.bm = 256; pl.bn = 256;
  }
  {
    const bool epi192 = a->epilogue == NBEST_EPI_NONE || a->epilogue == NBEST_EPI_BIAS || a->epilogue == NBEST_EPI_BIAS_DROP_RES ||
                        a->epilogue == NBEST_EPI_RES;
    if (!a->trans_a && !a->trans_b && a->N % 192 == 0 && epi192) {
      const int64_t rows = (a->M + 255) / 256, t192 = rows * (a->N / 192);
      auto eff = [](int64_t t) { return (double)t / (double)(((t + 255) / 256) * 256); };
      const double e256 = (a->N % 256 == 0) ? eff(rows * (a->N / 256)) : 0.0;
      if (t192 >= 256 && 0.85 * eff(t192) > e256) { pl.bm = 256; pl.bn = 192; }
    }
    if (pl.bm == 256 && pl.bn == 192 && a->N % 384 == 0 && a->K % BK == 0) { pl.bm = 128; pl.bn = 384; }
    if (pl.bm == 256 && pl.bn == 256 && !a->trans_a && !a->trans_b && epi192 && a->N % 512 == 0 && a->N <= 2048 && a->K % BK == 0) { pl.bm = 128; pl.bn = 512; }
  }
  const int64_t tiles = ((a->M + pl.bm - 1) / pl.bm) * (a->N / pl.bn);
  const int64_t slots = (pl.bn >= 192) ? 256 : 512;
  pl.splits = 1;
  pl.kps = round_up(a->K, 64);
  if (a->epilogue == NBEST_EPI_F32_SPLITK) nb_splitk_plan(tiles, a->K, slots, (4 * slots + 4) / 5, &pl.splits, &pl.kps);
  return pl;
}

template <int BM, int BN, int WM, int WN, int STAGES, bool TA, bool TB>
static int launch2(const GemmP2& p, int epi, int grid, hipStream_t st) {
  constexpr int NT = WM * WN * 64;
  constexpr int lds_bytes = STAGES * (BM + BN) * BK * 2 + (((BN * 4) % NT) ? (NT / 64) * 1024 : 0);
#define L(E)                                                                                                        \
  case E:                                                                                                           \
    (void)hipFuncSetAttribute((const void*)gemm2_kernel<BM, BN, WM, WN, STAGES, TA, TB, E>, hipFuncAttributeMaxDynamicSharedMemorySize, lds_bytes); \
    gemm2_kernel<BM, BN, WM, WN, STAGES, TA, TB, E><<<grid, NT, lds_bytes, st>>>(p);                                 \
    break;
  if constexpr (BN / WN == 64) {
    if (epi == NBEST_EPI_F32_SPLITK) {
      switch (epi) { L(NBEST_EPI_F32_SPLITK) }
      NB_LAUNCH_CHECK();
      return NBEST_OK;
    }
  }
  if constexpr (BN / WN == 96) {
    switch (epi) {
      L(NBEST_EPI_NONE) L(NBEST_EPI_BIAS) L(NBEST_EPI_BIAS_DROP_RES) L(NBEST_EPI_RES)
      default:
        nbest_set_error("gemm: epilogue %d is not built for 192-column tiles", epi);
        return NBEST_ERR_ARG;
    }
  } else {
    switch (epi) {
      L(NBEST_EPI_NONE) L(NBEST_EPI_BIAS) L(NBEST_EPI_BIAS_GELU) L(NBEST_EPI_BIAS_DROP_RES) L(NBEST_EPI_DGELU)
      L(NBEST_EPI_RES) L(kEpiBiasGeluNoU)
      default:
        nbest_set_error("gemm: bad epilogue %d", epi);
        return NBEST_ERR_ARG;
    }
  }
#undef L
  NB_LAUNCH_CHECK();
  return NBEST_OK;
}

}

bool nbest_gemm_bf16_v2_wins(const nbest_gemm_args* a) {
  if (a->colsum_out && a->epilogue != NBEST_EPI_DGELU && a->epilogue != NBEST_EPI_F32_SPLITK && !a->trans_a && !a->trans_b) return false;
  const Plan pl = make_plan(a);
  return pl.bm == 256 || (pl.bm == 128 && pl.bn >= 384);
}

size_t nbest_gemm_bf16_v2_ws_bytes(const nbest_gemm_args* a) {
  if (a->epilogue != NBEST_EPI_F32_SPLITK) {
    if (!a->colsum_out) return 0;
    const Plan pl0 = make_plan(a);
    return (size_t)((a->M + pl0.bm - 1) / pl0.bm) * 4 * a->N * sizeof(float);
  }
  const Plan pl = make_plan(a);
  return pl.splits > 1 ? (size_t)pl.splits * a->M * a->N * sizeof(float) : 0;
}

static int gemm_v2_impl(const nbest_gemm_args* a, const nbest_gemm_args* b2, int64_t m_split, hipStream_t st) {
  NB_CHECK(a->N % 64 == 0, NBEST_ERR_SHAPE, "gemm(bf16): N=%lld must be a multiple of 64", (long long)a->N);
  NB_CHECK(a->trans_a || a->K % BK == 0, NBEST_ERR_SHAPE, "gemm(bf16): K=%lld must be a multiple of %d", (long long)a->K, BK);
  const Plan pl = make_plan(a);
  GemmP2 p;
  p.A = (const bf16*)a->A; p.B = (const bf16*)a->B; p.C = a->C; p.bias = a->bias; p.R = (const bf16*)a->R; p.U = (bf16*)a->U;
  p.M = a->M; p.N = a->N; p.K = a->K; p.lda = a->lda; p.ldb = a->ldb; p.ldc = a->ldc; p.ldr = a->ldr; p.ldu = a->ldu;
  p.tiles_m = (int)((a->M + pl.bm - 1) / pl.bm);
  p.tiles_n = (int)(a->N / pl.bn);
  p.splits = pl.splits;
  p.k_per_split = pl.kps;
  p.accumulate = a->accumulate;
  p.slab = (float*)a->ws;
  p.colpart = nullptr;
  p.A2 = p.B2 = nullptr; p.lda2 = p.ldb2 = p.m_split = 0; p.a2_bytes = p.b2_bytes = 0;
  p.Bp = nullptr; p.bp_bytes = 0; p.bp_bn = 0;
  if (a->B_packed && ((a->b_pack_bn == pl.bn && pl.bm == 256 && (pl.bn == 256 || pl.bn == 192)) || (pl.bm == 128 && pl.bn == 384 && a->b_pack_bn == 192) || (pl.bm == 128 && pl.bn == 512 && a->b_pack_bn == 256)) &&
      !a->trans_a && !a->trans_b &&
      a->epilogue != NBEST_EPI_F32_SPLITK && a->K % BK == 0 && a->N * a->K * 2 < ((int64_t)1 << 32) && ((uintptr_t)a->B_packed & 15) == 0) {
    p.Bp = (const bf16*)a->B_packed;
    p.bp_bytes = (uint32_t)(a->N * a->K * 2);
    p.bp_bn = a->b_pack_bn;
  }
  if (a->colsum_out && a->epilogue != NBEST_EPI_F32_SPLITK) {
    NB_CHECK(a->epilogue == NBEST_EPI_DGELU || a->trans_a || a->trans_b, NBEST_ERR_ARG,
             "gemm(bf16, generation 2): column sums are fused into the x GELU' epilogue only (nbest_gemm routes the others to generation 1)");
    NB_CHECK(a->ws && a->ws_bytes >= nbest_gemm_bf16_v2_ws_bytes(a), NBEST_ERR_WORKSPACE, "gemm: column-sum workspace too small");
    p.colpart = (float*)a->ws;
  }
  const int64_t a_rows = a->trans_a ? a->K : a->M, a_cols = a->trans_a ? (b2 ? m_split : a->M) : a->K;
  const int64_t b_rows = a->trans_b ? a->K : a->N, b_cols = a->trans_b ? a->N : a->K;
  const int64_t ab = ((a_rows - 1) * a->lda + a_cols) * 2, bb = ((b_rows - 1) * a->ldb + b_cols) * 2;
  p.a_bytes = (uint32_t)ab; p.b_bytes = (uint32_t)bb;
  if (b2) {
    const int64_t ab2 = ((a->K - 1) * b2->lda + b2->M) * 2, bb2 = ((a->K - 1) * b2->ldb + a->N) * 2;
    p.A2 = (const bf16*)b2->A; p.B2 = (const bf16*)b2->B; p.lda2 = b2->lda; p.ldb2 = b2->ldb; p.m_split = m_split;
    p.a2_bytes = (uint32_t)ab2; p.b2_bytes = (uint32_t)bb2;
    NB_CHECK(pl.bm == 256 && pl.bn == 256 && pl.splits > 1 && m_split % 256 == 0, NBEST_ERR_SHAPE, "wgrad pair: not a 256 x 256 split-K plan");
  }
  p.c_bytes = p.r_bytes = p.u_bytes = 0;
  if (a->epilogue != NBEST_EPI_F32_SPLITK) {
    const int64_t mpad = a->M + 256;
    NB_CHECK(mpad * a->ldc * 2 < ((int64_t)1 << 32) && mpad * a->ldr * 2 < ((int64_t)1 << 32) && mpad * a->ldu < ((int64_t)1 << 32),
             NBEST_ERR_SHAPE, "gemm(bf16): output / residual larger than 4 GiB");
    p.c_bytes = (uint32_t)(a->M * a->ldc * 2);
    p.r_bytes = a->R ? (uint32_t)(a->M * a->ldr * 2) : 0;
    p.u_bytes = a->U ? (uint32_t)(a->M * a->ldu) : 0;
  }
  p.drop = make_drop(a->drop_p, a->seed, a->drop_stream);
  p.stream_out = 1;
  p.gn = (!a->trans_a && !a->trans_b) ? nb_group_cols(a->N / pl.bn, (int64_t)pl.bn * a->K * 2, 2400) : (int)(a->N / pl.bn);
  if (pl.bm == 128 && pl.bn >= 384 && (a->N / pl.bn) % 2 == 0) p.gn = 2;
  const int epi = a->epilogue;
  if (epi == NBEST_EPI_F32_SPLITK && p.splits > 1)
    NB_CHECK(a->ws && a->ws_bytes >= (size_t)p.splits * a->M * a->N * sizeof(float), NBEST_ERR_WORKSPACE,
             "gemm: split-K workspace too small (%zu < %zu)", a->ws_bytes, (size_t)p.splits * a->M * a->N * sizeof(float));
  const int grid = p.tiles_m * p.tiles_n * p.splits;
  const int kepi = nb_kernel_epilogue(epi, a->U);
  int rc, wave_rows = 2;
  NB_CHECK(a->N % pl.bn == 0, NBEST_ERR_SHAPE, "gemm(bf16): N=%lld is not a multiple of the %d-column tile", (long long)a->N, pl.bn);
  if (pl.bm == 128 && pl.bn == 512) {
    rc = launch2<128, 512, 2, 4, 4, false, false>(p, kepi, grid, st);
  } else if (pl.bm == 128 && pl.bn == 384) {
    if (a->K >= 2048) rc = launch2<128, 384, 2, 4, 5, false, false>(p, kepi, grid, st);
    else rc = launch2<128, 384, 2, 4, 4, false, false>(p, kepi, grid, st);
  } else if (pl.bm == 256 && pl.bn == 192) {
    if (a->K >= 2048) rc = launch2<256, 192, 4, 2, 5, false, false>(p, kepi, grid, st);
    else rc = launch2<256, 192, 4, 2, 4, false, false>(p, kepi, grid, st);
    wave_rows = 4;
  } else if (pl.bm == 256 && pl.bn == 256) {
    if (!a->trans_a && !a->trans_b && epi != NBEST_EPI_F32_SPLITK) {
      if (a->K >= 2048) rc = launch2<256, 256, 4, 2, 5, false, false>(p, kepi, grid, st);
      else rc = launch2<256, 256, 4, 2, 4, false, false>(p, kepi, grid, st);
      wave_rows = 4;
    }
    else if (!a->trans_a && !a->trans_b) rc = launch2<256, 256, 2, 4, 4, false, false>(p, kepi, grid, st);
    else if (!a->trans_a && a->trans_b) rc = launch2<256, 256, 2, 4, 4, false, true>(p, kepi, grid, st);
    else rc = launch2<256, 256, 2, 4, 4, true, true>(p, kepi, grid, st);
  } else if (pl.bm == 256) {
    if (!a->trans_b && epi != NBEST_EPI_F32_SPLITK) { rc = launch2<256, 128, 4, 1, 3, false, false>(p, kepi, grid, st); wave_rows = 4; }
    else if (!a->trans_b) rc = launch2<256, 128, 2, 2, 3, false, false>(p, kepi, grid, st);
    else rc = launch2<256, 128, 2, 2, 3, false, true>(p, kepi, grid, st);
  } else {
    nbest_set_error("gemm(bf16, generation 2): no kernel for the %d x %d plan", pl.bm, pl.bn);
    return NBEST_ERR_SHAPE;
  }
  if (rc) return rc;
  if (p.colpart) return nbest_internal_partial_rows_sum(p.colpart, p.tiles_m * wave_rows, (int)a->N, a->colsum_out, a->colsum_accumulate, st);
  if (epi == NBEST_EPI_F32_SPLITK && p.splits > 1 && !(a->flags & NBEST_GEMM_DEFER_REDUCE))
    return nbest_internal_splitk_reduce(p.slab, (float*)a->C, a->M, a->N, a->ldc, p.splits, a->accumulate, b2 ? (float*)b2->C : nullptr,
                                        b2 ? m_split : a->M, b2 ? b2->ldc : 0, st);
  return NBEST_OK;
}

int nbest_gemm_bf16_v2(const nbest_gemm_args* a, hipStream_t st) { return gemm_v2_impl(a, nullptr, 0, st); }

static bool pair_virtual(const nbest_gemm_args* a, const nbest_gemm_args* b, nbest_gemm_args* v) {
  if (a->dtype != NBEST_BF16 || b->dtype != NBEST_BF16 || !a->trans_a || !a->trans_b || !b->trans_a || !b->trans_b) return false;
  if (a->epilogue != NBEST_EPI_F32_SPLITK || b->epilogue != NBEST_EPI_F32_SPLITK) return false;
  if (a->N != b->N || a->K != b->K || a->accumulate != b->accumulate || a->M % 256 || b->M % 256 || a->N % 256) return false;
  if ((a->flags | b->flags) & NBEST_GEMM_DEFER_REDUCE) return false;
  *v = *a;
  v->M = a->M + b->M;
  const Plan pl = make_plan(v);
  return pl.bm == 256 && pl.bn == 256 && pl.splits > 1;
}
size_t nbest_wgrad_pair_bf16_ws_bytes(const nbest_gemm_args* a, const nbest_gemm_args* b) {
  nbest_gemm_args v;
  if (!pair_virtual(a, b, &v)) return 0;
  return nbest_gemm_bf16_v2_ws_bytes(&v);
}
int nbest_wgrad_pair_bf16(const nbest_gemm_args* a, const nbest_gemm_args* b, hipStream_t st) {
  nbest_gemm_args v;
  NB_CHECK(pair_virtual(a, b, &v), NBEST_ERR_SHAPE, "wgrad pair: the two problems do not share one 256 x 256 split-K launch");
  return gemm_v2_impl(&v, b, a->M, st);
}

int nbest_pack_bn_internal(int64_t N) {
  if (N % 256 == 0 && N >= 1024) return 256;
  if (N % 192 == 0) return 192;
  return 0;
}

int nbest_pack_weights_bf16(const void* src, void* dst, const nbest_matrix_desc* descs, int n_matrices, int n_stages, hipStream_t st) {
  pack_b_kernel<<<n_stages, 256, 0, st>>>((const bf16*)src, (bf16*)dst, descs, n_matrices);
  NB_LAUNCH_CHECK();
  return NBEST_OK;
}
```

n-best-asr-transformer_amd/csrc/internal.h:

```cpp
#pragma once
#include <hip/hip_runtime_api.h>
#include <stddef.h>
#include <stdint.h>

#include "../../include/nbest_hip.h"

struct Fp8Grad;

void nbest_set_error(const char* fmt, ...);

int nbest_internal_layernorm_fwd8(const void* x, const float* gamma, const float* beta, void* y, void* y8, float* stats,
                                  int64_t M, int H, float eps, int dtype, nbest_stream_t stream, const uint32_t* a_prev, uint32_t* a_new);
int nbest_internal_layernorm_bwd8(const void* dy, const void* x, const float* stats, const float* gamma, void* dx,
                                  void* dx_drop, float* dgamma, float* dbeta, float* dbias, int64_t M, int H, int dtype,
                                  int accumulate, float drop_p, uint64_t seed, uint32_t drop_stream, void* ws,
                                  size_t ws_bytes, nbest_stream_t stream, Fp8Grad f8);
int nbest_internal_partial_rows_sum(const float* part, int nrows, int N, float* out, int accumulate, hipStream_t st);
void nbest_internal_rowred_batch_begin();
void nbest_internal_rowred_batch_abort();
int nbest_internal_rowred_batch_flush(hipStream_t st);

int nbest_internal_attention_fwd8(const void* qkv, const uint8_t* key_mask, void* ctx, void* ctx8, float* lse, int B, int S, int heads,
                                  int d, int dtype, float drop_p, uint64_t seed, uint32_t drop_stream, nbest_stream_t stream,
                                  uint32_t* keep, const uint32_t* a_prev, uint32_t* a_new);
int nbest_internal_attention_bwd8(const void* qkv, const uint8_t* key_mask, const void* ctx, const void* dctx, const float* lse,
                                  void* dqkv, float* dbias, int accumulate, void* ws, size_t ws_bytes, int B, int S, int heads,
                                  int d, int dtype, float drop_p, uint64_t seed, uint32_t drop_stream, nbest_stream_t stream, Fp8Grad f8,
                                  const uint32_t* keep);
size_t nbest_internal_attention_keep_bytes(int B, int S, int heads);
int nbest_attention_cls_fwd_internal(const void* q, int64_t ldq, const void* kv, int64_t ldkv, const uint8_t* key_mask, void* ctx,
                                     int64_t ldctx, int B, int S, int heads, int d, int dtype, nbest_stream_t stream);
int nbest_internal_attention_cls_probs(const void* q, int64_t ldq, const void* kv, int64_t ldkv, const uint8_t* key_mask, float* probs,
                                       int64_t ldp, int B, int S, int heads, int d, int dtype, nbest_stream_t stream);

void nb_splitk_plan(int64_t tiles, int64_t K, int64_t slots, int64_t min_blocks, int* splits, int64_t* k_per_split);
int nbest_internal_splitk_reduce(const float* slab, float* C, int64_t M, int64_t N, int64_t ldc, int splits, int accumulate,
                                 float* C2, int64_t m_split, int64_t ldc2, hipStream_t st);

int nbest_gemm_f32(const nbest_gemm_args* a, hipStream_t st);
size_t nbest_gemm_bf16_ws_bytes(const nbest_gemm_args* a);
int nbest_gemm_bf16(const nbest_gemm_args* a, hipStream_t st);
size_t nbest_gemm_bf16_v2_ws_bytes(const nbest_gemm_args* a);
int nbest_gemm_bf16_v2(const nbest_gemm_args* a, hipStream_t st);
bool nbest_gemm_bf16_v2_wins(const nbest_gemm_args* a);
size_t nbest_wgrad_pair_bf16_ws_bytes(const nbest_gemm_args* a, const nbest_gemm_args* b);
int nbest_wgrad_pair_bf16(const nbest_gemm_args* a, const nbest_gemm_args* b, hipStream_t st);
int nbest_pack_bn_internal(int64_t N);
int nbest_pack_weights_bf16(const void* src, void* dst, const nbest_matrix_desc* descs, int n_matrices, int n_stages, hipStream_t st);

int nbest_internal_amax_bf16(const void* x, int64_t n, uint32_t* out, hipStream_t st);
int nbest_internal_cast_bf16_to_fp8(const void* src, void* dst, int64_t n, const uint32_t* a_prev, uint32_t* a_new, hipStream_t st);
```

n-best-asr-transformer_amd/hipabi.py:

```python
import ctypes as C
import os

import torch

_HERE = os.path.dirname(os.path.abspath(__file__))
LIB_PATH = os.environ.get("NBEST_LIB") or os.path.join(_HERE, "csrc", "libnbest_hip.so")

F32, BF16 = 0, 1
ADAM_L2, ADAMW = 0, 1
EPI_NONE, EPI_BIAS, EPI_BIAS_GELU, EPI_BIAS_DROP_RES, EPI_DGELU, EPI_RES, EPI_F32_SPLITK = range(7)

EXPORTS = [
    "nbest_version", "nbest_last_error", "nbest_embed_ln_fwd", "nbest_embed_ln_bwd", "nbest_embed_bwd_ws_bytes", "nbest_rows_gather", "nbest_rows_zero", "nbest_rows_add",
    "nbest_gemm_ws_bytes", "nbest_gemm", "nbest_wgrad_pair_ws_bytes", "nbest_wgrad_pair", "nbest_pack_bn", "nbest_pack_weights", "nbest_pack_bn_fp8", "nbest_pack_weights_fp8", "nbest_attention_fwd", "nbest_attention_bwd", "nbest_attention_bwd_ws_bytes", "nbest_attention_keep_bytes", "nbest_attention_fwd_keep", "nbest_attention_bwd_keep", "nbest_layernorm_fwd",
    "nbest_layernorm_bwd", "nbest_rowred_ws_bytes", "nbest_colsum", "nbest_heads_ws_bytes", "nbest_stc_heads",
    "nbest_stc_heads_vjp", "nbest_cls_mse", "nbest_cls_grad_scatter", "nbest_stc_decode", "nbest_stream_stamp", "nbest_fp8_amax_fold", "nbest_bertadam_chunk", "nbest_bertadam_step", "nbest_bertadam_norms", "nbest_bertadam_update",
    "nbest_adam_clip_coef", "nbest_adam_update", "nbest_adam_step",
    "nbest_cast_f32_to_bf16", "nbest_transpose_weights", "nbest_encoder_act_bytes", "nbest_encoder_ws_bytes", "nbest_encoder_wgrad_launches_per_layer", "nbest_encoder_forward",
    "nbest_encoder_backward", "nbest_gemm_fp8", "nbest_gemm_fp8_ws_bytes", "nbest_wgrad_fp8", "nbest_wgrad_fp8_ws_bytes", "nbest_wgrad_fp8_pair", "nbest_wgrad_fp8_pair_ws_bytes", "nbest_cast_bf16_to_fp8", "nbest_quantize_weights_fp8",
    "nbest_attention_cls_fwd", "nbest_encoder_infer_ws_bytes", "nbest_encoder_infer",
    "nbest_attention_probs", "nbest_attention_cls_probs", "nbest_encoder_act_view", "nbest_encoder_infer_attn",
    "nbest_embed_ln_fwd_interp", "nbest_embed_attrib",
]


class GemmArgs(C.Structure):
    _fields_ = [("A", C.c_void_p), ("B", C.c_void_p), ("C", C.c_void_p), ("bias", C.c_void_p), ("R", C.c_void_p),
                ("U", C.c_void_p), ("ws", C.c_void_p), ("ws_bytes", C.c_size_t),
                ("M", C.c_int64), ("N", C.c_int64), ("K", C.c_int64),
                ("lda", C.c_int64), ("ldb", C.c_int64), ("ldc", C.c_int64), ("ldr", C.c_int64), ("ldu", C.c_int64),
                ("trans_a", C.c_int32), ("trans_b", C.c_int32), ("epilogue", C.c_int32), ("dtype", C.c_int32),
                ("accumulate", C.c_int32), ("drop_p", C.c_float), ("drop_stream", C.c_uint32), ("seed", C.c_uint64),
                ("colsum_out", C.c_void_p), ("colsum_accumulate", C.c_int32), ("flags", C.c_int32),
                ("B_packed", C.c_void_p), ("b_pack_bn", C.c_int32), ("pad_", C.c_int32)]


class GemmFp8Args(C.Structure):
    _fields_ = [("A", C.c_void_p), ("B", C.c_void_p), ("C", C.c_void_p), ("bias", C.c_void_p), ("R", C.c_void_p), ("U", C.c_void_p),
                ("C8", C.c_void_p), ("M", C.c_int64), ("N", C.c_int64), ("K", C.c_int64),
                ("lda", C.c_int64), ("ldb", C.c_int64), ("ldc", C.c_int64), ("ldr", C.c_int64), ("ldu", C.c_int64), ("ldc8", C.c_int64),
                ("epilogue", C.c_int32), ("out_scale", C.c_float), ("drop_p", C.c_float), ("drop_stream", C.c_uint32), ("seed", C.c_uint64),
                ("out_scale_dev", C.c_void_p), ("a_amax", C.c_void_p), ("c8_amax_prev", C.c_void_p), ("c8_amax_new", C.c_void_p),
                ("colsum_out", C.c_void_p), ("colsum_accumulate", C.c_int32), ("pad", C.c_int32), ("ws", C.c_void_p), ("ws_bytes", C.c_size_t),
                ("B_packed", C.c_void_p), ("b_pack_bn", C.c_int32), ("pad3", C.c_int32)]


class LabelSpaceC(C.Structure):
    _fields_ = [("n_top", C.c_int32), ("n_bottom", C.c_int32), ("n_rows", C.c_int32),
                ("bottom_off", C.c_void_p), ("bottom_ids", C.c_void_p), ("head_row", C.c_void_p)]


class TensorDesc(C.Structure):
    _fields_ = [("offset", C.c_int64), ("numel", C.c_int64), ("lr", C.c_float), ("wd", C.c_float),
                ("active", C.c_int32), ("block_start", C.c_int32)]


class MatrixDesc(C.Structure):
    _fields_ = [("offset", C.c_int64), ("rows", C.c_int32), ("cols", C.c_int32), ("tile_start", C.c_int32), ("pad", C.c_int32)]


class LayerOffsets(C.Structure):
    _fields_ = [(n, C.c_int64) for n in ("wqkv", "bqkv", "wo", "bo", "ln1_g", "ln1_b", "w1", "b1", "w2", "b2", "ln2_g", "ln2_b")]


class EncoderDesc(C.Structure):
    _fields_ = [("dtype", C.c_int32), ("B", C.c_int32), ("S", C.c_int32), ("H", C.c_int32), ("L", C.c_int32),
                ("heads", C.c_int32), ("F", C.c_int32), ("vocab", C.c_int32), ("max_pos", C.c_int32), ("n_types", C.c_int32),
                ("ln_eps", C.c_float), ("hidden_drop", C.c_float), ("attn_drop", C.c_float),
                ("word_pad_id", C.c_int64), ("pos_pad_id", C.c_int64),
                ("off_word", C.c_int64), ("off_pos", C.c_int64), ("off_type", C.c_int64),
                ("off_emb_ln_g", C.c_int64), ("off_emb_ln_b", C.c_int64),
                ("layers_host", C.POINTER(LayerOffsets)), ("seed", C.c_uint64), ("drop_stream_base", C.c_uint32),
                ("wgrad_events_n", C.c_int32), ("wgrad_events", C.POINTER(C.c_void_p)),
                ("w8", C.c_void_p), ("w8_inv_scale", C.c_void_p), ("w8t", C.c_void_p), ("gamax_prev", C.c_void_p),
                ("gamax_new", C.c_void_p), ("fp8_bwd", C.c_int32), ("pad2", C.c_int32),
                ("wpk", C.c_void_p), ("wpkt", C.c_void_p), ("w8p", C.c_void_p), ("w8tp", C.c_void_p),
                ("word_perm", C.c_void_p), ("aamax_prev", C.c_void_p), ("aamax_new", C.c_void_p), ("fp8_act", C.c_int32), ("pad4", C.c_int32),
                ("first_trainable", C.c_int32), ("no_input_grad", C.c_int32), ("wgrad_skip_host", C.c_void_p),
                ("base_ids", C.c_void_p), ("alpha", C.c_void_p), ("no_param_grad", C.c_int32), ("pad5", C.c_int32)]


_lib = None


def lib():
    global _lib
    if _lib is None:
        if not os.path.exists(LIB_PATH):
            raise RuntimeError("nbest_amd: %s is missing - build it with `make -C %s` (hipcc, gfx950). "
                               "There is no CPU fallback for the product path." % (LIB_PATH, os.path.dirname(LIB_PATH)))
        L = C.CDLL(LIB_PATH)
        for name in EXPORTS:
            if not hasattr(L, name):
                raise RuntimeError("nbest_amd: %s does not export %s" % (LIB_PATH, name))
        for name in ("nbest_embed_bwd_ws_bytes", "nbest_gemm_ws_bytes", "nbest_wgrad_pair_ws_bytes", "nbest_rowred_ws_bytes", "nbest_heads_ws_bytes",
                     "nbest_attention_bwd_ws_bytes", "nbest_attention_keep_bytes",
                     "nbest_encoder_act_bytes", "nbest_encoder_ws_bytes", "nbest_encoder_infer_ws_bytes"):
            getattr(L, name).restype = C.c_size_t
        L.nbest_embed_bwd_ws_bytes.argtypes = [C.c_int64, C.c_int64]
        L.nbest_rows_gather.argtypes = [C.c_void_p, C.c_void_p, C.c_int64, C.c_int64, C.c_void_p, C.c_void_p, C.c_int, C.c_void_p]
        L.nbest_rows_zero.argtypes = [C.c_void_p, C.c_void_p, C.c_int64, C.c_int, C.c_void_p]
        L.nbest_rows_add.argtypes = [C.c_void_p, C.c_void_p, C.c_void_p, C.c_int64, C.c_int, C.c_void_p]
        L.nbest_rowred_ws_bytes.argtypes = [C.c_int64, C.c_int64]
        L.nbest_heads_ws_bytes.argtypes = [C.c_int, C.c_int, C.c_int]
        L.nbest_gemm_ws_bytes.argtypes = [C.POINTER(GemmArgs)]
        L.nbest_gemm.argtypes = [C.POINTER(GemmArgs), C.c_void_p]
        L.nbest_wgrad_pair_ws_bytes.argtypes = [C.POINTER(GemmArgs), C.POINTER(GemmArgs)]
        L.nbest_wgrad_pair.argtypes = [C.POINTER(GemmArgs), C.POINTER(GemmArgs), C.c_void_p]
        L.nbest_encoder_act_bytes.argtypes = [C.POINTER(EncoderDesc)]
        L.nbest_encoder_ws_bytes.argtypes = [C.POINTER(EncoderDesc)]
        L.nbest_encoder_wgrad_launches_per_layer.argtypes = [C.POINTER(EncoderDesc)]
        vp, i64, i32, f32, u64, u32, sz = C.c_void_p, C.c_int64, C.c_int, C.c_float, C.c_uint64, C.c_uint32, C.c_size_t
        L.nbest_embed_ln_fwd.argtypes = [vp] * 10 + [i64, i32, f32, i32, f32, u64, u32, vp]
        L.nbest_embed_ln_bwd.argtypes = [vp] * 15 + [i32, i32, i32, i32, i32, i64, i64, i32, i32, f32, u64, u32, vp, sz, vp]
        L.nbest_embed_ln_fwd_interp.argtypes = [vp] * 12 + [i32, i32, i32, f32, i32, f32, u64, u32, vp]
        L.nbest_embed_attrib.argtypes = [vp] * 11 + [i32, i32, i32, i32, f32, i32, vp]
        L.nbest_attention_fwd.argtypes = [vp] * 4 + [i32] * 5 + [f32, u64, u32, vp]
        L.nbest_attention_bwd.argtypes = [vp] * 7 + [i32, vp, sz] + [i32] * 5 + [f32, u64, u32, vp]
        L.nbest_attention_bwd_ws_bytes.argtypes = [i32, i32, i32]
        L.nbest_attention_keep_bytes.argtypes = [i32, i32, i32]
        L.nbest_attention_fwd_keep.argtypes = [vp] * 4 + [i32] * 5 + [f32, u64, u32, vp, vp]
        L.nbest_attention_bwd_keep.argtypes = [vp] * 7 + [i32, vp, sz] + [i32] * 5 + [f32, u64, u32, vp, vp]
        L.nbest_layernorm_fwd.argtypes = [vp] * 5 + [i64, i32, f32, i32, vp]
        L.nbest_layernorm_bwd.argtypes = [vp] * 9 + [i64, i32, i32, i32, f32, u64, u32, vp, sz, vp]
        L.nbest_colsum.argtypes = [vp, vp, i64, i64, i64, i32, i32, vp, sz, vp]
        L.nbest_stc_heads.argtypes = [vp, i64, vp, vp, C.POINTER(LabelSpaceC)] + [vp] * 8 + [i32] * 5 + [f32, u64, u32, vp, sz, vp]
        L.nbest_stc_heads_vjp.argtypes = [vp, C.POINTER(LabelSpaceC)] + [vp] * 8 + [i32, i32, i32, f32, u64, u32, vp, sz, vp]
        L.nbest_cls_mse.argtypes = [vp, i64, vp, i64, vp, vp, vp, i32, i32, i32, f32, vp]
        L.nbest_cls_grad_scatter.argtypes = [vp, vp, i32, i32, i32, i32, vp]
        L.nbest_stc_decode.argtypes = [vp, vp, C.POINTER(LabelSpaceC), vp, vp, i32, vp]
        L.nbest_stream_stamp.argtypes = [vp, i32, vp]
        L.nbest_fp8_amax_fold.argtypes = [vp, vp, i32, vp]
        L.nbest_bertadam_step.argtypes = [vp] * 6 + [i32, i32, f32, f32, f32, f32, f32, vp, sz, vp]
        L.nbest_bertadam_norms.argtypes = [vp, vp, i32, i32, i32, i32, vp, vp]
        L.nbest_bertadam_update.argtypes = [vp] * 6 + [i32, i32, i32, i32, vp, vp, f32, f32, f32, f32, f32, vp]
        L.nbest_adam_clip_coef.argtypes = [vp, i32, f32, vp, vp]
        f64 = C.c_double
        L.nbest_adam_update.argtypes = [i32] + [vp] * 6 + [i32, i32, i32, i32, vp, f32, f32, f32, f64, f64, f32, vp]
        L.nbest_adam_step.argtypes = [i32] + [vp] * 6 + [i32, i32, f32, f32, f32, f64, f64, f32, f32, vp, sz, vp]
        L.nbest_cast_f32_to_bf16.argtypes = [vp, vp, i64, vp]
        L.nbest_encoder_forward.argtypes = [C.POINTER(EncoderDesc)] + [vp] * 7 + [sz, vp, sz, C.POINTER(C.c_void_p), vp]
        L.nbest_encoder_infer_ws_bytes.argtypes = [C.POINTER(EncoderDesc)]
        L.nbest_encoder_infer.argtypes = [C.POINTER(EncoderDesc)] + [vp] * 7 + [sz, vp, vp]
        L.nbest_attention_cls_fwd.argtypes = [vp, i64, vp, i64, vp, vp, i64, i32, i32, i32, i32, i32, vp]
        L.nbest_encoder_infer_attn.argtypes = [C.POINTER(EncoderDesc)] + [vp] * 7 + [sz, vp, vp, vp]
        L.nbest_encoder_act_view.argtypes = [C.POINTER(EncoderDesc), vp, i32, C.POINTER(C.c_void_p), C.POINTER(C.c_void_p)]
        L.nbest_attention_probs.argtypes = [vp] * 4 + [i32] * 5 + [vp]
        L.nbest_attention_cls_probs.argtypes = [vp, i64, vp, i64, vp, vp, i64, i32, i32, i32, i32, i32, vp]
        L.nbest_encoder_backward.argtypes = [C.POINTER(EncoderDesc)] + [vp] * 9 + [sz, vp, vp, sz, i32, i32, i32, i32, vp]
        L.nbest_transpose_weights.argtypes = [vp, vp, vp, i32, i32, vp]
        L.nbest_pack_bn.argtypes = [i64]
        L.nbest_pack_weights.argtypes = [vp, vp, vp, i32, i32, vp]
        L.nbest_pack_bn_fp8.argtypes = [i64, i64]
        L.nbest_pack_weights_fp8.argtypes = [vp, vp, vp, i32, i32, vp]
        L.nbest_gemm_fp8.argtypes = [C.POINTER(GemmFp8Args), vp]
        L.nbest_cast_bf16_to_fp8.argtypes = [vp, vp, i64, vp]
        L.nbest_wgrad_fp8_ws_bytes.restype = C.c_size_t
        L.nbest_wgrad_fp8_ws_bytes.argtypes = [i64, i64, i64]
        L.nbest_wgrad_fp8.argtypes = [vp, vp, vp, i64, i64, i64, i64, i64, i64, vp, vp, i32, vp, sz, vp]
        L.nbest_wgrad_fp8_pair_ws_bytes.restype = C.c_size_t
        L.nbest_wgrad_fp8_pair_ws_bytes.argtypes = [i64, i64, i64, i64]
        L.nbest_wgrad_fp8_pair.argtypes = [vp, vp, vp, i64, i64, i64, i64, vp, vp, vp, vp, vp, i64, i64, i64, i64, vp, vp, i64, i64, i32, vp, sz, vp]
        L.nbest_quantize_weights_fp8.argtypes = [vp, vp, vp, vp, i32, i32, vp, vp, sz, vp]
        L.nbest_gemm_fp8_ws_bytes.restype = C.c_size_t
        L.nbest_gemm_fp8_ws_bytes.argtypes = [C.POINTER(GemmFp8Args)]
        L.nbest_last_error.argtypes = [C.c_char_p, sz]
        _lib = L
    return _lib


def last_error():
    buf = C.create_string_buffer(512)
    lib().nbest_last_error(buf, 512)
    return buf.value.decode(errors="replace")


def check(rc, what):
    if rc != 0:
        raise RuntimeError("nbest_hip %s failed (%d): %s" % (what, rc, last_error()))


def stream_ptr():
    return C.c_void_p(torch.cuda.current_stream().cuda_stream)


def dtype_code(t):
    if t == torch.float32:
        return F32
    if t == torch.bfloat16:
        return BF16
    raise RuntimeError("nbest_amd: unsupported activation dtype %s" % t)


def ptr(t):
    return C.c_void_p(0) if t is None else C.c_void_p(t.data_ptr())


def _ws(nbytes, device):
    return torch.empty(max(int(nbytes), 16), dtype=torch.uint8, device=device)


def gemm_prepared(A, B, M, N, K, out, trans_a=False, trans_b=False, epilogue=EPI_NONE, defer_reduce=False):
    g = GemmArgs()
    g.A, g.B, g.C = A.data_ptr(), B.data_ptr(), out.data_ptr()
    g.M, g.N, g.K = M, N, K
    g.lda, g.ldb, g.ldc = A.stride(0), B.stride(0), out.stride(0)
    g.trans_a, g.trans_b, g.epilogue, g.dtype = int(trans_a), int(trans_b), epilogue, dtype_code(A.dtype)
    g.flags = 1 if defer_reduce else 0
    ws = _ws(lib().nbest_gemm_ws_bytes(C.byref(g)), A.device)
    g.ws, g.ws_bytes = ws.data_ptr(), ws.numel()
    fn, ref, st = lib().nbest_gemm, C.byref(g), stream_ptr()

    def launch():
        rc = fn(ref, st)
        if rc:
            check(rc, "gemm")
    launch.keepalive = (g, ws, A, B, out)
    return launch


def pack_weight(W):
    N, K = W.shape
    bn = lib().nbest_pack_bn(N)
    if bn == 0 or K % 32 or N % bn:
        return None, 0
    d = (MatrixDesc * 1)()
    d[0].offset, d[0].rows, d[0].cols, d[0].tile_start, d[0].pad = 0, N, K, 0, bn
    dd = torch.frombuffer(bytearray(bytes(d)), dtype=torch.uint8).to(W.device)
    out = torch.empty_like(W)
    check(lib().nbest_pack_weights(ptr(W), ptr(out), ptr(dd), 1, (N // bn) * (K // 32), stream_ptr()), "pack_weights")
    return out, bn


def pack_weight_fp8(W8):
    N, K = W8.shape
    bn = lib().nbest_pack_bn_fp8(N, K)
    if bn == 0 or K % 64 or N % bn:
        return None, 0
    d = (MatrixDesc * 1)()
    d[0].offset, d[0].rows, d[0].cols, d[0].tile_start, d[0].pad = 0, N, K, 0, bn
    dd = torch.frombuffer(bytearray(bytes(d)), dtype=torch.uint8).to(W8.device)
    out = torch.empty_like(W8)
    check(lib().nbest_pack_weights_fp8(ptr(W8), ptr(out), ptr(dd), 1, (N // bn) * (K // 64), stream_ptr()), "pack_weights_fp8")
    return out, bn


def gemm(A, B, M, N, K, trans_a=False, trans_b=False, epilogue=EPI_NONE, bias=None, R=None, U=None, out=None,
         accumulate=False, drop_p=0.0, seed=0, drop_stream=0, colsum_out=None, defer_reduce=False, B_packed=None, b_pack_bn=0,
         want_u=True):
    dt = dtype_code(A.dtype)
    dev = A.device
    if out is None:
        out = torch.empty(M, N, dtype=torch.float32 if epilogue == EPI_F32_SPLITK else A.dtype, device=dev)
    if epilogue == EPI_BIAS_GELU and U is None and want_u:
        U = torch.empty(M, N, dtype=torch.float32 if A.dtype == torch.float32 else torch.uint8, device=dev)
    g = GemmArgs()
    g.A, g.B, g.C = A.data_ptr(), B.data_ptr(), out.data_ptr()
    g.bias = bias.data_ptr() if bias is not None else None
    g.R = R.data_ptr() if R is not None else None
    g.U = U.data_ptr() if U is not None else None
    g.M, g.N, g.K = M, N, K
    g.lda, g.ldb, g.ldc = A.stride(0), B.stride(0), out.stride(0)
    g.ldr = R.stride(0) if R is not None else 0
    g.ldu = U.stride(0) if U is not None else 0
    g.trans_a, g.trans_b, g.epilogue, g.dtype = int(trans_a), int(trans_b), epilogue, dt
    g.accumulate, g.drop_p, g.drop_stream, g.seed = int(accumulate), drop_p, drop_stream, seed
    g.colsum_out = colsum_out.data_ptr() if colsum_out is not None else None
    g.flags = 1 if defer_reduce else 0
    if B_packed is not None:
        g.B_packed, g.b_pack_bn = B_packed.data_ptr(), b_pack_bn
    nb = lib().nbest_gemm_ws_bytes(C.byref(g))
    ws = _ws(nb, dev)
    g.ws, g.ws_bytes = ws.data_ptr(), ws.numel()
    check(lib().nbest_gemm(C.byref(g), stream_ptr()), "gemm")
    return (out, U) if epilogue == EPI_BIAS_GELU and want_u else out


def wgrad_pair(dY1, X1, dY2, X2, out1=None, out2=None, accumulate=False):
    K, N = X1.shape
    outs, gs = [], []
    for dY, X, out in ((dY1, X1, out1), (dY2, X2, out2)):
        M = dY.shape[1]
        if out is None:
            out = torch.empty(M, N, dtype=torch.float32, device=X.device)
        g = GemmArgs()
        g.A, g.B, g.C = dY.data_ptr(), X.data_ptr(), out.data_ptr()
        g.M, g.N, g.K = M, N, K
        g.lda, g.ldb, g.ldc = dY.stride(0), X.stride(0), out.stride(0)
        g.trans_a = g.trans_b = 1
        g.epilogue, g.dtype, g.accumulate = EPI_F32_SPLITK, dtype_code(X.dtype), int(accumulate)
        outs.append(out)
        gs.append(g)
    nb = lib().nbest_wgrad_pair_ws_bytes(C.byref(gs[0]), C.byref(gs[1]))
    ws = _ws(nb, X1.device)
    gs[0].ws, gs[0].ws_bytes = ws.data_ptr(), ws.numel()
    check(lib().nbest_wgrad_pair(C.byref(gs[0]), C.byref(gs[1]), stream_ptr()), "wgrad_pair")
    return outs


def rows_gather(table, rows, cap):
    H = table.shape[1]
    ids = torch.empty(cap, dtype=torch.long, device=table.device)
    vals = torch.empty(cap, H, dtype=torch.float32, device=table.device)
    check(lib().nbest_rows_gather(ptr(table), ptr(rows), rows.numel(), cap, ptr(ids), ptr(vals), H, stream_ptr()), "rows_gather")
    return ids, vals


def rows_zero(table, ids):
    check(lib().nbest_rows_zero(ptr(table), ptr(ids), ids.numel(), table.shape[1], stream_ptr()), "rows_zero")


def rows_add(table, ids, vals):
    check(lib().nbest_rows_add(ptr(table), ptr(ids), ptr(vals), ids.numel(), table.shape[1], stream_ptr()), "rows_add")


def gelu_d_decode(U):
    return U if U.dtype == torch.float32 else (U.float() - 26.0) / 200.0


def gelu_d_encode(g):
    return torch.clamp(torch.round(g.float() * 200.0 + 26.0), 0, 255).to(torch.uint8)


def cast_fp8(x):
    out = torch.empty(x.shape, dtype=torch.uint8, device=x.device)
    check(lib().nbest_cast_bf16_to_fp8(ptr(x), ptr(out), x.numel(), stream_ptr()), "cast_bf16_to_fp8")
    return out


def gemm_fp8(A8, W8, M, N, K, bias, out_scale=1.0, epilogue=EPI_BIAS, R=None, drop_p=0.0, seed=0, drop_stream=0, out=None, B_packed=None, b_pack_bn=0):
    dev = A8.device
    if out is None:
        out = torch.empty(M, N, dtype=torch.bfloat16, device=dev)
    g = GemmFp8Args()
    g.A, g.B, g.C, g.bias = A8.data_ptr(), W8.data_ptr(), out.data_ptr(), bias.data_ptr()
    g.M, g.N, g.K, g.lda, g.ldb, g.ldc = M, N, K, A8.stride(0), W8.stride(0), out.stride(0)
    g.epilogue, g.out_scale, g.drop_p, g.drop_stream, g.seed = epilogue, out_scale, drop_p, drop_stream, seed
    U = C8 = None
    if epilogue == EPI_BIAS_GELU:
        U = torch.empty(M, N, dtype=torch.uint8, device=dev)
        C8 = torch.empty(M, N, dtype=torch.uint8, device=dev)
        g.U, g.C8, g.ldu, g.ldc8 = U.data_ptr(), C8.data_ptr(), N, N
    if R is not None:
        g.R, g.ldr = R.data_ptr(), R.stride(0)
    if B_packed is not None:
        g.B_packed, g.b_pack_bn = B_packed.data_ptr(), b_pack_bn
    check(lib().nbest_gemm_fp8(C.byref(g), stream_ptr()), "gemm_fp8")
    return (out, U, C8) if epilogue == EPI_BIAS_GELU else out


def wgrad_fp8(dY8, X8, M, N, K, a_amax=None, out=None, accumulate=False, x_amax=None):
    if out is None:
        out = torch.zeros(M, N, dtype=torch.float32, device=dY8.device)
    ws = _ws(lib().nbest_wgrad_fp8_ws_bytes(M, N, K), dY8.device)
    check(lib().nbest_wgrad_fp8(ptr(dY8), ptr(X8), ptr(out), M, N, K, dY8.stride(0), X8.stride(0), out.stride(0), ptr(a_amax), ptr(x_amax),
                                int(accumulate), ptr(ws), ws.numel(), stream_ptr()), "wgrad_fp8")
    return out


def wgrad_fp8_pair(dY8a, X8a, dY8b, X8b, amax_a=None, amax_b=None, outs=None, accumulate=False, xamax_a=None, xamax_b=None):
    K, N = X8a.shape
    Ma, Mb = dY8a.shape[1], dY8b.shape[1]
    oa, ob = outs if outs is not None else (torch.zeros(Ma, N, dtype=torch.float32, device=X8a.device),
                                            torch.zeros(Mb, N, dtype=torch.float32, device=X8a.device))
    ws = _ws(lib().nbest_wgrad_fp8_pair_ws_bytes(Ma, Mb, N, K), X8a.device)
    check(lib().nbest_wgrad_fp8_pair(ptr(dY8a), ptr(X8a), ptr(oa), Ma, dY8a.stride(0), X8a.stride(0), oa.stride(0), ptr(amax_a), ptr(xamax_a),
                                     ptr(dY8b), ptr(X8b), ptr(ob), Mb, dY8b.stride(0), X8b.stride(0), ob.stride(0), ptr(amax_b), ptr(xamax_b),
                                     N, K, int(accumulate), ptr(ws), ws.numel(), stream_ptr()), "wgrad_fp8_pair")
    return oa, ob


def layernorm_fwd(x, gamma, beta, eps):
    M, H = x.shape
    y = torch.empty_like(x)
    stats = torch.empty(M, 2, dtype=torch.float32, device=x.device)
    check(lib().nbest_layernorm_fwd(ptr(x), ptr(gamma), ptr(beta), ptr(y), ptr(stats), M, H, eps, dtype_code(x.dtype),
                                    stream_ptr()), "layernorm_fwd")
    return y, stats


def layernorm_bwd(dy, x, stats, gamma, want_dbias=True, drop_p=0.0, seed=0, drop_stream=0):
    M, H = x.shape
    dx = torch.empty_like(x)
    dxd = torch.empty_like(x) if drop_p > 0 else None
    dg = torch.zeros(H, dtype=torch.float32, device=x.device)
    db = torch.zeros_like(dg)
    dbias = torch.zeros_like(dg) if want_dbias else None
    ws = _ws(lib().nbest_rowred_ws_bytes(M, H), x.device)
    check(lib().nbest_layernorm_bwd(ptr(dy), ptr(x), ptr(stats), ptr(gamma), ptr(dx), ptr(dxd), ptr(dg), ptr(db), ptr(dbias),
                                    M, H, dtype_code(x.dtype), 0, drop_p, seed, drop_stream, ptr(ws), ws.numel(), stream_ptr()),
          "layernorm_bwd")
    return dx, dxd, dg, db, dbias


def colsum(X, accumulate=False, out=None):
    M, N = X.shape
    if out is None:
        out = torch.zeros(N, dtype=torch.float32, device=X.device)
    ws = _ws(lib().nbest_rowred_ws_bytes(M, N), X.device)
    check(lib().nbest_colsum(ptr(X), ptr(out), M, N, X.stride(0), dtype_code(X.dtype), int(accumulate), ptr(ws), ws.numel(),
                             stream_ptr()), "colsum")
    return out


def attention_fwd(qkv, key_mask, B, S, heads, drop_p=0.0, seed=0, drop_stream=0, want_keep=False):
    H = heads * 64
    ctx = torch.empty(B * S, H, dtype=qkv.dtype, device=qkv.device)
    lse = torch.empty(B, heads, S, dtype=torch.float32, device=qkv.device)
    if want_keep:
        nb = lib().nbest_attention_keep_bytes(B, S, heads) if qkv.dtype == torch.bfloat16 else 0
        keep = torch.zeros(nb // 4, dtype=torch.int32, device=qkv.device) if nb else None
        check(lib().nbest_attention_fwd_keep(ptr(qkv), ptr(key_mask), ptr(ctx), ptr(lse), B, S, heads, 64, dtype_code(qkv.dtype),
                                             drop_p, seed, drop_stream, ptr(keep), stream_ptr()), "attention_fwd_keep")
        return ctx, lse, keep
    check(lib().nbest_attention_fwd(ptr(qkv), ptr(key_mask), ptr(ctx), ptr(lse), B, S, heads, 64, dtype_code(qkv.dtype),
                                    drop_p, seed, drop_stream, stream_ptr()), "attention_fwd")
    return ctx, lse


def attention_cls_fwd(q, ldq, kv, ldkv, key_mask, B, S, heads, out=None):
    H = heads * 64
    ctx = torch.empty(B, H, dtype=kv.dtype, device=kv.device) if out is None else out
    check(lib().nbest_attention_cls_fwd(ptr(q), ldq, ptr(kv), ldkv, ptr(key_mask), ptr(ctx), ctx.stride(0), B, S, heads, 64,
                                        dtype_code(kv.dtype), stream_ptr()), "attention_cls_fwd")
    return ctx


def attention_probs(qkv, key_mask, lse, B, S, heads, out=None):
    probs = torch.empty(B, heads, S, S, dtype=torch.float32, device=qkv.device) if out is None else out
    check(lib().nbest_attention_probs(ptr(qkv), ptr(key_mask), ptr(lse), ptr(probs), B, S, heads, 64, dtype_code(qkv.dtype),
                                      stream_ptr()), "attention_probs")
    return probs


def attention_cls_probs(q, ldq, kv, ldkv, key_mask, B, S, heads, out=None):
    probs = torch.empty(B, heads, S, dtype=torch.float32, device=kv.device) if out is None else out
    check(lib().nbest_attention_cls_probs(ptr(q), ldq, ptr(kv), ldkv, ptr(key_mask), ptr(probs), probs.stride(1), B, S, heads, 64,
                                          dtype_code(kv.dtype), stream_ptr()), "attention_cls_probs")
    return probs


def encoder_act_view(desc, act, layer):
    q, l = C.c_void_p(), C.c_void_p()
    check(lib().nbest_encoder_act_view(C.byref(desc), ptr(act), layer, C.byref(q), C.byref(l)), "encoder_act_view")
    return q.value, l.value


def encoder_infer(desc, wts, prm, ids, seg, pos, key_mask, ws, cls_out, cls_attn=None):
    if cls_attn is None:
        check(lib().nbest_encoder_infer(C.byref(desc), ptr(wts), ptr(prm), ptr(ids), ptr(seg), ptr(pos), ptr(key_mask), ptr(ws),
                                        ws.numel(), ptr(cls_out), stream_ptr()), "encoder_infer")
    else:
# ... 178 lines not shown
```

n-best-asr-transformer_amd/model.py:

```python
import collections
import ctypes as C
import os

import torch
import torch.nn as nn

from . import hipabi as hb
from .arena import ParamArena
from .config import EncoderConfig, LabelSpace, NAMED


def position_ids_for(cfg, input_ids):
    B, S = input_ids.shape
    if cfg.family in ("roberta", "xlm-roberta"):
        nonpad = input_ids.ne(cfg.pad_token_id).long()
        return (torch.cumsum(nonpad, dim=1) * nonpad + cfg.pad_token_id).contiguous()
    return torch.arange(S, dtype=torch.long, device=input_ids.device).unsqueeze(0).expand(B, S).contiguous()


class _Holder(nn.Module):
    """module tree node that only carries arena-backed parameters under HF names"""


def _attach(root, dotted, param):
    mod = root
    parts = dotted.split(".")
    for p in parts[:-1]:
        if not hasattr(mod, p):
            mod.add_module(p, _Holder())
        mod = getattr(mod, p)
    mod.register_parameter(parts[-1], param)


class FreezePlan(collections.namedtuple("FreezePlan", "key trainable first_trainable no_input_grad with_embeddings skip")):
    __slots__ = ()

    @property
    def skip_ptr(self):
        return None if self.skip is None else C.cast(self.skip, C.c_void_p)


def freeze_plan(model):
    flags = tuple(p.requires_grad and "pooler" not in n for n, p in model._params)
    plan = model._plans.get(flags)
    if plan is not None:
        return plan
    trainable = frozenset(n for (n, _), f in zip(model._params, flags) if f)
    L = model.cfg.num_hidden_layers
    emb = any(n.startswith("bert_encoder.embeddings.") for n in trainable)
    layer = [any(n.startswith("bert_encoder.encoder.layer.%d." % l) for n in trainable) for l in range(L)]
    first = 0 if emb else next((l for l in range(L) if layer[l]), L)
    pre = "bert_encoder.encoder.layer.%d."
    mats = (["attention.self.%s.weight" % q for q in ("query", "key", "value")], ["attention.output.dense.weight"],
            ["intermediate.dense.weight"], ["output.dense.weight"])
    skip = [int(not any((pre % l) + m in trainable for m in ms)) for l in range(L) for ms in mats]
    plan = FreezePlan(flags, trainable, first, int(not emb), emb, (C.c_uint8 * len(skip))(*skip) if any(skip) else None)
    if len(model._plans) >= 64:
        model._plans.clear()
    model._plans[flags] = plan
    return plan


class _Pass:

    def __init__(self, model, B, S, slot, first_trainable=0):
        a, cfg = model.arena, model.cfg
        train = isinstance(slot, int)
        d = hb.EncoderDesc()
        d.dtype = hb.dtype_code(model.compute_dtype)
        d.B, d.S, d.H, d.L, d.heads, d.F = B, S, cfg.hidden_size, cfg.num_hidden_layers, cfg.num_attention_heads, cfg.intermediate_size
        d.vocab, d.max_pos, d.n_types = cfg.vocab_size, cfg.max_position_embeddings, cfg.type_vocab_size
        d.ln_eps = cfg.layer_norm_eps
        d.word_pad_id = cfg.pad_token_id
        d.pos_pad_id = cfg.pad_token_id if cfg.family in ("roberta", "xlm-roberta") else -1
        pre = "bert_encoder.embeddings."
        d.off_word = a.by_name[pre + "word_embeddings.weight"].offset
        d.off_pos = a.by_name[pre + "position_embeddings.weight"].offset
        d.off_type = a.by_name[pre + "token_type_embeddings.weight"].offset
        d.off_emb_ln_g = a.by_name[pre + "LayerNorm.weight"].offset
        d.off_emb_ln_b = a.by_name[pre + "LayerNorm.bias"].offset
        d.layers_host = C.cast(a.layer_offsets, C.POINTER(hb.LayerOffsets))
        d.drop_stream_base = 1000 * slot if train else 0
        d.first_trainable = first_trainable
        if model.fp8_forward and train:
            d.w8, d.w8_inv_scale = a.w8.data_ptr(), a.w8_inv_scale.data_ptr()
        self.desc = d
        self.act_bytes = hb.lib().nbest_encoder_act_bytes(C.byref(d))
        self.B, self.S = B, S


class _PassRecord(collections.namedtuple("_PassRecord", "ps slot inputs perm hidden gen plan")):
    __slots__ = ()

    @property
    def cls(self):
        return self.hidden.view(self.ps.B, self.ps.S, -1)[:, 0, :]


class _STCBridge(torch.autograd.Function):

    @staticmethod
    def forward(ctx, anchor, model, input_ids, trans_input_ids, seg_ids, trans_seg_ids, feats_from_transcript):
        ctx.set_materialize_grads(False)
        from_t = bool(feats_from_transcript and trans_input_ids is not None)
        ws = hb.heads_ws(input_ids.shape[0], model.dls.n_rows, model.cfg.hidden_size, model.device)
        plan = model._training_plan()
        ra, rt, (top, bott, fin, _, _, _, _) = model._passes_and_heads(input_ids, seg_ids, trans_input_ids, trans_seg_ids, True,
                                                                       from_transcript=from_t, ws=ws, plan=plan)
        ctx.model, ctx.ra, ctx.rt, ctx.ws, ctx.seed, ctx.from_t = model, ra, rt, ws, model._step_seed(), from_t
        ctx.save_for_backward(top, bott)
        trans_cls = rt.cls.float() if rt is not None else torch.zeros(0, device=model.device)
        return top, bott, fin, ra.cls.float(), trans_cls

    @staticmethod
    def backward(ctx, dtop, dbott, dfin, dasr, dtrans):
        m = ctx.model
        m._check_stash(ctx.ra, ctx.rt)
        _require_trainable(ctx.ra.plan)
        top, bott = ctx.saved_tensors
        B, H = top.shape[0], m.cfg.hidden_size
        z = lambda g, like: torch.zeros_like(like) if g is None else g.contiguous().float()
        fin_like = torch.empty(B, m.labels.n_bottom, dtype=torch.float32, device=m.device)
        dWh, dbh = m.arena.heads_grad_wb()
        dcls = hb.stc_heads_vjp(m.arena.heads_wb()[0], m.dls, top, bott, z(dtop, top), z(dbott, bott), z(dfin, fin_like), B, H, dWh, dbh, ctx.ws,
                                accumulate=True, drop_p=m.dropout, seed=ctx.seed, drop_stream=900)
        d_asr = dasr.contiguous().float() if dasr is not None else None
        d_tr = dtrans.contiguous().float() if (dtrans is not None and ctx.rt is not None) else None
        if ctx.from_t:
            d_tr = dcls if d_tr is None else d_tr + dcls
        else:
            d_asr = dcls if d_asr is None else d_asr + dcls
        if d_tr is not None and ctx.rt is not None:
            m._backward_pass(ctx.rt, d_tr, accumulate=True)
        if d_asr is not None:
            m._backward_pass(ctx.ra, d_asr, accumulate=True)
        m._end_of_step(True)
        return (None,) * 7


def _require_trainable(plan):
    if plan is not None and not plan.trainable:
        raise RuntimeError("nbest_amd: no parameter requires grad: a backward has nothing to compute (every tensor of the model "
                           "has requires_grad=False)")


class NBestSTCModel(nn.Module):
    def __init__(self, cfg: EncoderConfig, labels: LabelSpace, device="cuda", compute_dtype=torch.bfloat16, dropout=0.0,
                 seed=999, fp8_forward=False, fp8_backward=None):
        super().__init__()
        self.cfg, self.labels, self.compute_dtype = cfg, labels, compute_dtype
        self.dropout = float(dropout)
        self.device = torch.device(device)
        self.arena = ParamArena(cfg, labels, self.device, compute_dtype)
        self.fp8_forward = bool(fp8_forward)
        self.fp8_backward = self.fp8_forward if fp8_backward is None else bool(fp8_backward)
        self._gamax_valid = False
        self._aamax_valid = False
        if self.fp8_forward:
            if compute_dtype != torch.bfloat16:
                raise RuntimeError("nbest_amd: fp8_forward rides on the bf16 path")
            self.arena.enable_fp8_forward()
        elif self.fp8_backward:
            raise RuntimeError("nbest_amd: fp8_backward needs fp8_forward (it shares the e4m3 weight copy)")
        self.bert_encoder = _Holder()
        self.clf = _Holder()
        for s in self.arena.slots:
            p = nn.Parameter(self.arena.view(self.arena.p, s.name), requires_grad="pooler" not in s.name)
            if p.requires_grad:
                p.grad = self.arena.view(self.arena.g, s.name)
            root, rest = s.name.split(".", 1)
            _attach(getattr(self, root), rest, p)
        self._params = [(s.name, self.get_parameter(s.name)) for s in self.arena.slots]
        self._plans = {}
        self._plan_key = None
        self.dls = hb.DeviceLabelSpace(labels, self.device)
        self.seed = int(seed)
        self.step_counter = 0
        self._passes = {}
        self._stash = {}
        self._stash_gen = collections.Counter()
        self._ws = None
        self._dh = None
        self._infer_ws = None
        self._anchor = None

    def zero_grad(self, set_to_none=False):
        self.arena.g.zero_()

    def _drop_fp8_history(self):
        if self.fp8_backward and self._gamax_valid:
            self._gamax_valid = False
            self.arena.gamax.zero_()
            self.arena.gamax_slots.zero_()
        if self.fp8_forward and self._aamax_valid:
            self._aamax_valid = False
            self.arena.aamax.zero_()
            self.arena.aamax_slots.zero_()

    def load_reference_state(self, sd, strict=True):
        self._drop_fp8_history()
        return self.arena.load_state(sd, strict)

    def save_model(self, path):
        torch.save({k: v.detach().cpu() for k, v in self.state_dict().items()}, path)

    def load_model(self, path):
        self._drop_fp8_history()
        self.arena.load_state(torch.load(path, map_location="cpu", weights_only=True))

    def load_pretrained_encoder(self, path):
        import os
        if os.path.isdir(path):
            cands = [os.path.join(path, f) for f in ("model.safetensors", "pytorch_model.bin")]
            found = [c for c in cands if os.path.exists(c)]
            if not found:
                raise FileNotFoundError("no model.safetensors / pytorch_model.bin under %s" % path)
            path = found[0]
        self._drop_fp8_history()
        if path.endswith(".safetensors"):
            from safetensors.torch import load_file
            raw = load_file(path, device="cpu")
        else:
            raw = torch.load(path, map_location="cpu", weights_only=True)
        sd = {}
        for k, v in raw.items():
            for pre in ("bert_encoder.", "bert.", "roberta.", "xlm_roberta."):
                if k.startswith(pre):
                    k = k[len(pre):]
                    break
            k = k.replace("LayerNorm.gamma", "LayerNorm.weight").replace("LayerNorm.beta", "LayerNorm.bias")
            if k.startswith(("embeddings.", "encoder.", "pooler.")) and not k.endswith("position_ids"):
                sd["bert_encoder." + k] = v
        want = [s.name for s in self.arena.slots if s.name.startswith("bert_encoder.")]
        missing = [n for n in want if n not in sd]
        hard = [n for n in missing if "pooler" not in n]
        if hard:
            raise RuntimeError("checkpoint lacks encoder tensors: %s" % hard[:5])
        self.arena.load_state(sd, strict=False)
        return missing

    def _desc(self, B, S, slot, first_trainable=0):
        key = (B, S, slot, first_trainable)
        if key not in self._passes:
            if len(self._passes) >= 4096:
                self._passes.clear()
            self._passes[key] = _Pass(self, B, S, slot, first_trainable)
        return self._passes[key]

    def _training_plan(self):
        plan = freeze_plan(self)
        if plan.key != self._plan_key:
            for (n, p), f in zip(self._params, plan.key):
                if "pooler" in n:
                    continue
                if not f:
                    p.grad = None
                elif p.grad is None:
                    p.grad = self.arena.view(self.arena.g, n)
            if self._plan_key is not None and self.fp8_backward and self._gamax_valid:
                self._gamax_valid = False
                self.arena.gamax.zero_()
                self.arena.gamax_slots.zero_()
            self._plan_key = plan.key
        return plan

    def _grow(self, table, key, n, dtype=torch.uint8):
        buf = table.get(key)
        if buf is None or buf.numel() < n:
            table[key] = buf = None
            table[key] = buf = torch.empty(n, dtype=dtype, device=self.device)
        return buf

    def _pass(self, B, S, slot, first_trainable=0):
        ps = self._desc(B, S, slot, first_trainable)
        self._grow(self._stash, slot, ps.act_bytes)
        self._grow(vars(self), "_ws", hb.lib().nbest_encoder_ws_bytes(C.byref(ps.desc)))
        self._stash_gen[slot] += 1
        return ps

    def _check_stash(self, *records):
        for r in records:
            if r is not None and r.gen != self._stash_gen[r.slot]:
                raise RuntimeError("nbest_amd: another forward ran on this model between this forward() and its backward(): the "
                                   "activations of its %s pass are overwritten" % ("ASR", "transcript")[r.slot])

    def _step_seed(self):
        rank = 0
        if torch.distributed.is_available() and torch.distributed.is_initialized():
            rank = torch.distributed.get_rank()
        return self.seed + 7919 * self.step_counter + 15485863 * rank

    def _inputs(self, ids, seg):
        cfg = self.cfg
        ids = ids.contiguous()
        mask = (ids > 0).to(torch.uint8)
        pos = position_ids_for(cfg, ids)
        if cfg.family == "xlm-roberta":
            seg = None
        elif seg is not None:
            seg = seg.contiguous()
        return ids, seg, pos, mask

    def _encode(self, slot, ids, seg, train, perm=None, plan=None):
        B, S = ids.shape
        ps = self._pass(B, S, slot, plan.first_trainable if plan is not None else 0)
# ... 334 lines not shown
```

Measured before the change: 12080.

## Group weight-gradient GEMMs of two encoder layers into one grouped launch

Adds a grouped bf16 weight-gradient kernel that runs up to eight 256x256-tiled problems, each with no split-K, in a single launch. The encoder backward can now defer the four wgrad GEMMs of a layer, or of two consecutive layers, into that one launch, double-buffering the gradient scratch buffers so the deferred inputs stay valid. A cost model with hardcoded constants decides whether grouping beats the existing split-K per-GEMM path. This is meant to cut launch count and the split-K reduction overhead and to fill the GPU better, at the cost of extra workspace and longer per-tile K loops.

```diff
diff --git a/include/nbest_hip.h b/include/nbest_hip.h
--- a/include/nbest_hip.h
+++ b/include/nbest_hip.h
@@ -83,6 +83,7 @@
 
 size_t nbest_wgrad_pair_ws_bytes(const nbest_gemm_args* a, const nbest_gemm_args* b);
 int nbest_wgrad_pair(const nbest_gemm_args* a, const nbest_gemm_args* b, nbest_stream_t stream);
+int nbest_wgrad_group(const nbest_gemm_args* problems, int n, nbest_stream_t stream);
 
 typedef struct nbest_gemm_fp8_args {
   const void* A;
@@ -263,8 +264,9 @@
   const int64_t* base_ids;
   const float* alpha;
   int32_t no_param_grad;
-  int32_t pad5;
+  int32_t wgrad_group;
 } nbest_encoder_desc;
+enum { NBEST_WGRAD_GROUP_PLAN = 0, NBEST_WGRAD_GROUP_NEVER = 1, NBEST_WGRAD_GROUP_ALWAYS = 2 };
 size_t nbest_encoder_act_bytes(const nbest_encoder_desc* d);
 int nbest_encoder_act_view(const nbest_encoder_desc* d, void* act, int layer, void** qkv, float** lse);
 size_t nbest_encoder_ws_bytes(const nbest_encoder_desc* d);
diff --git a/n-best-asr-transformer_amd/csrc/encoder.hip b/n-best-asr-transformer_amd/csrc/encoder.hip
--- a/n-best-asr-transformer_amd/csrc/encoder.hip
+++ b/n-best-asr-transformer_amd/csrc/encoder.hip
@@ -60,6 +60,7 @@
 
 struct WsLayout {
   size_t dR, dRd, dB1, dctx, dBig, dqkv, red, slab, slab_bytes, red_bytes, emb, emb_bytes, f8, f8_bytes, total;
+  size_t gset[2][4];
   size_t fz_x0, fz_x1, fz_emb_stats, fz_lse, fz_st1, fz_st2, fz_u;
 };
 
@@ -92,12 +93,37 @@
 
 static bool wgrad_paired(const nbest_encoder_desc* d, bool f8b) { return d->dtype == NBEST_BF16 && wgrad_pair_bytes(d, f8b) > 0; }
 
+constexpr double kWgA = 24.5, kWgB = 0.705, kWgRed = 12.7;
+static double wgrad_splitk_us(int64_t rows, int64_t cols, int64_t M) {
+  const nbest_gemm_args g = wgrad_args(NBEST_BF16, rows, cols, M);
+  const size_t ws = nbest_gemm_ws_bytes(&g);
+  const int64_t splits = ws ? (int64_t)(ws / ((size_t)rows * cols * sizeof(float))) : 1;
+  const int64_t stages = ((M + splits - 1) / splits + 31) / 32, wgs = (rows / 256) * (cols / 256) * splits;
+  return kWgA + kWgB * (double)(stages * ((wgs + 255) / 256)) + (splits > 1 ? kWgRed : 0.0);
+}
+static int wgrad_group_layers(const nbest_encoder_desc* d) {
+  if (d->wgrad_group == NBEST_WGRAD_GROUP_NEVER) return 0;
+  if (d->dtype != NBEST_BF16 || d->w8 || d->H % 256 || d->F % 256) return 0;
+  const int64_t H = d->H, F = d->F, M = (int64_t)d->B * d->S;
+  const int64_t tiles = (4 * H * H + 2 * H * F) / (256 * 256);
+  if (d->wgrad_group == NBEST_WGRAD_GROUP_ALWAYS) return 2 * tiles <= 256 ? 2 : 1;
+  if (2 * tiles > 256 || !wgrad_paired(d, false)) return 0;
+  const double today = wgrad_splitk_us(4 * H, H, M) + wgrad_splitk_us(F, H, M) + wgrad_splitk_us(H, F, M);
+  const double grouped = (kWgA + kWgB * (double)((M + 31) / 32)) / 2.0;
+  return grouped < 0.95 * today ? 2 : 0;
+}
+
 static WsLayout ws_layout(const nbest_encoder_desc* d, const Sizes& z) {
   WsLayout w;
   const int64_t M = z.M;
   size_t o = 0;
   w.dR = take(o, z.MH); w.dRd = take(o, z.MH); w.dB1 = take(o, z.MH); w.dctx = take(o, z.MH);
   w.dBig = take(o, z.MF); w.dqkv = take(o, z.M3H);
+  for (int s = 0; s < 2; ++s) { w.gset[s][0] = w.dRd; w.gset[s][1] = w.dBig; w.gset[s][2] = w.dRd; w.gset[s][3] = w.dqkv; }
+  if (wgrad_group_layers(d) > 0) {
+    w.gset[0][2] = take(o, z.MH);
+    if (wgrad_group_layers(d) > 1) { w.gset[1][0] = take(o, z.MH); w.gset[1][1] = take(o, z.MF); w.gset[1][2] = take(o, z.MH); w.gset[1][3] = take(o, z.M3H); }
+  }
   const int64_t maxN = d->F > 3 * d->H ? d->F : 3 * d->H;
   w.red_bytes = al(nbest_rowred_ws_bytes(M, maxN));
   w.red_bytes = std::max(w.red_bytes, al(nbest_attention_bwd_ws_bytes(d->B, d->S, d->heads)));
@@ -325,7 +351,9 @@
 }
 extern "C" size_t nbest_encoder_ws_bytes(const nbest_encoder_desc* d) { return d ? ws_layout(d, sizes(d)).total : 0; }
 extern "C" int nbest_encoder_wgrad_launches_per_layer(const nbest_encoder_desc* d) {
-  return d ? (wgrad_paired(d, fp8_backward_active(d)) ? 3 : 4) : 0;
+  if (!d) return 0;
+  if (wgrad_group_layers(d) > 0) return 1;
+  return wgrad_paired(d, fp8_backward_active(d)) ? 3 : 4;
 }
 
 extern "C" int nbest_encoder_forward(const nbest_encoder_desc* d, const void* wts, const float* prm, const int64_t* ids,
@@ -414,7 +442,9 @@
   void* red1 = W + w.red + w.red_bytes; void* red2 = W + w.red + 2 * w.red_bytes; void* red3 = W + w.red + 3 * w.red_bytes;
   const bool f8b = fp8_backward_active(d);
   const bool paired = wgrad_paired(d, f8b);
-  int ev_i = (paired ? 3 : 4) * (d->L - layer_end);
+  const int gl = wgrad_group_layers(d);
+  const bool grouped = gl > 0;
+  int ev_i = (grouped ? 1 : paired ? 3 : 4) * (d->L - layer_end);
   auto stamp = [&](int which) {
     if (d->wgrad_events && 2 * ev_i + which < d->wgrad_events_n) (void)hipEventRecord((hipEvent_t)d->wgrad_events[2 * ev_i + which], st);
     ev_i += which;
@@ -431,11 +461,15 @@
   };
   const GemmPass dg = {dt, M, stream, 0, Ptrs{(const char*)(wt ? wts_t : wts), prm, z.esz}, wt ? d->wpkt : nullptr, !wt, f8b,
                        d->w8t, d->w8tp, d->w8_inv_scale, d->gamax_prev, d->gamax_new, red1, w.red_bytes, accumulate};
-  auto wgrad = [&](int l, const WGrad* wg, int j, int j2) -> int {
+  auto wgrad_args_of = [&](const WGrad* x) {
+    nbest_gemm_args g = wgrad_args(dt, x->rows, x->cols, M);
+    g.A = x->dY; g.B = x->X; g.C = G(x->w_off); g.accumulate = accumulate;
+    return g;
+  };
+  auto wgrad_launch = [&](int l, const WGrad* wg, int j, int j2) -> int {
     const WGrad* p = skip(l, j) ? nullptr : wg + j;
     const WGrad* q = (j2 >= 0 && !skip(l, j2)) ? wg + j2 : nullptr;
     if (!p) { p = q; q = nullptr; }
-    stamp(0);
     if (p && f8b) {
       const uint32_t *gp = d->gamax_prev, *ap = d->aamax_prev;
       if (q)
@@ -446,18 +480,20 @@
         RUN(nbest_wgrad_fp8(p->dY8, p->X8, G(p->w_off), p->rows, p->cols, M, p->rows, p->cols, p->cols, gp + p->g_idx, ap + p->a_idx,
                             accumulate, slab, w.slab_bytes, stream));
     } else if (p) {
-      auto args = [&](const WGrad* x) {
-        nbest_gemm_args g = wgrad_args(dt, x->rows, x->cols, M);
-        g.A = x->dY; g.B = x->X; g.C = G(x->w_off); g.accumulate = accumulate;
-        return g;
-      };
-      nbest_gemm_args g1 = args(p), g2 = args(q ? q : p);
+      nbest_gemm_args g1 = wgrad_args_of(p), g2 = wgrad_args_of(q ? q : p);
       g1.ws = slab; g1.ws_bytes = w.slab_bytes;
       RUN(q ? nbest_wgrad_pair(&g1, &g2, stream) : nbest_gemm(&g1, stream));
     }
+    return NBEST_OK;
+  };
+  auto wgrad = [&](int l, const WGrad* wg, int j, int j2) -> int {
+    stamp(0);
+    RUN(wgrad_launch(l, wg, j, j2));
     stamp(1);
     return NBEST_OK;
   };
+  nbest_gemm_args pend[8];
+  int n_pend = 0;
 
   struct BatchGuard { ~BatchGuard() { nbest_internal_rowred_batch_abort(); } } batch_guard;
   for (int l = layer_end - 1; l >= layer_begin; --l) {
@@ -466,35 +502,61 @@
     const bool input_grad = !(d->no_input_grad && l == FT);
     const int t = 4 * l;
     const uint32_t s0 = d->drop_stream_base + 1 + 4 * l;
-    const WGrad wg[4] = {{dqkv, X(l), dqkv8, b.x8, o.wqkv, 3 * H, H, t + 3, t + 0},
-                         {dRd, b.ctx, dRd8, b.ctx8, o.wo, H, H, t + 2, t + 1},
-                         {dBig, b.x1, dBig8, b.x18, o.w1, F, H, t + 1, t + 2},
-                         {dRd, b.hact, dRd8, b.h8, o.w2, H, F, t + 0, t + 3}};
+    const int gpos = grouped ? (layer_end - 1 - l) % gl : 0;
+    const bool group_ends = grouped && (gpos == gl - 1 || l == layer_begin);
+    void *dR2 = dR, *dR1 = dR, *dRd2 = dRd, *dRd1 = dRd, *dBigL = dBig, *dqkvL = dqkv;
+    if (grouped) {
+      dRd2 = W + w.gset[gpos][0]; dBigL = W + w.gset[gpos][1]; dRd1 = W + w.gset[gpos][2]; dqkvL = W + w.gset[gpos][3];
+      if (!hdrop) { dR2 = dRd2; dR1 = dRd1; }
+    }
+    const WGrad wg[4] = {{dqkvL, X(l), dqkv8, b.x8, o.wqkv, 3 * H, H, t + 3, t + 0},
+                         {dRd1, b.ctx, dRd8, b.ctx8, o.wo, H, H, t + 2, t + 1},
+                         {dBigL, b.x1, dBig8, b.x18, o.w1, F, H, t + 1, t + 2},
+                         {dRd2, b.hact, dRd8, b.h8, o.w2, H, F, t + 0, t + 3}};
     if (!npg) nbest_internal_rowred_batch_begin();
-    RUN(nbest_internal_layernorm_bwd8(dA, b.r2, b.st2, P.P(o.ln2_g), dR, (hdrop && !f8b) ? dRd : nullptr, GP(o.ln2_g), GP(o.ln2_b), GP(o.b2), M, H,
+    RUN(nbest_internal_layernorm_bwd8(dA, b.r2, b.st2, P.P(o.ln2_g), dR2, (hdrop && !f8b) ? dRd2 : nullptr, GP(o.ln2_g), GP(o.ln2_b), GP(o.b2), M, H,
                                       dt, accumulate, d->hidden_drop, d->seed, s0 + 2, red, w.red_bytes, stream, fg(dRd8, t + 0)));
-    GemmOp dw2 = {dRd, dRd8, t + 0, o.w2, t + 3, f8b ? nullptr : dBig, F, H, NBEST_EPI_DGELU};
+    GemmOp dw2 = {dRd2, dRd8, t + 0, o.w2, t + 3, f8b ? nullptr : dBigL, F, H, NBEST_EPI_DGELU};
     dw2.U = b.u; dw2.colsum = GP(o.b1); dw2.C8 = dBig8; dw2.c_idx = t + 1;
     RUN(layer_gemm(dg, dw2));
-    if (rec && !f8b) RUN(nbest_internal_amax_bf16(dBig, M * F, GN(t + 1), st));
-    RUN(wgrad(l, wg, 3, -1));
-    GemmOp dw1 = {dBig, dBig8, t + 1, o.w1, t + 2, dB1, H, F, NBEST_EPI_RES};
-    dw1.R = dR;
+    if (rec && !f8b) RUN(nbest_internal_amax_bf16(dBigL, M * F, GN(t + 1), st));
+    if (!grouped) RUN(wgrad(l, wg, 3, -1));
+    GemmOp dw1 = {dBigL, dBig8, t + 1, o.w1, t + 2, dB1, H, F, NBEST_EPI_RES};
+    dw1.R = dR2;
     RUN(layer_gemm(dg, dw1));
-    RUN(wgrad(l, wg, 2, -1));
-    RUN(nbest_internal_layernorm_bwd8(dB1, b.r1, b.st1, P.P(o.ln1_g), dR, (hdrop && !f8b) ? dRd : nullptr, GP(o.ln1_g), GP(o.ln1_b), GP(o.bo), M, H,
+    if (!grouped) RUN(wgrad(l, wg, 2, -1));
+    RUN(nbest_internal_layernorm_bwd8(dB1, b.r1, b.st1, P.P(o.ln1_g), dR1, (hdrop && !f8b) ? dRd1 : nullptr, GP(o.ln1_g), GP(o.ln1_b), GP(o.bo), M, H,
                                       dt, accumulate, d->hidden_drop, d->seed, s0 + 1, red2, w.red_bytes, stream, fg(dRd8, t + 2)));
-    const GemmOp dwo = {dRd, dRd8, t + 2, o.wo, t + 1, dctx, H, H, NBEST_EPI_NONE};
+    const GemmOp dwo = {dRd1, dRd8, t + 2, o.wo, t + 1, dctx, H, H, NBEST_EPI_NONE};
     RUN(layer_gemm(dg, dwo));
-    if (!paired) RUN(wgrad(l, wg, 1, -1));
-    RUN(nbest_internal_attention_bwd8(b.qkv, key_mask, b.ctx, dctx, b.lse, f8b ? nullptr : dqkv, GP(o.bqkv), accumulate, red3, w.red_bytes, d->B, d->S,
+    if (!paired && !grouped) RUN(wgrad(l, wg, 1, -1));
+    RUN(nbest_internal_attention_bwd8(b.qkv, key_mask, b.ctx, dctx, b.lse, f8b ? nullptr : dqkvL, GP(o.bqkv), accumulate, red3, w.red_bytes, d->B, d->S,
                                       d->heads, 64, dt, d->attn_drop, d->seed, s0 + 0, stream, fg(dqkv8, t + 3), b.keep));
     if (input_grad) {
-      GemmOp dwqkv = {dqkv, dqkv8, t + 3, o.wqkv, t + 0, dA, H, 3 * H, NBEST_EPI_RES};
-      dwqkv.R = dR;
+      GemmOp dwqkv = {dqkvL, dqkv8, t + 3, o.wqkv, t + 0, dA, H, 3 * H, NBEST_EPI_RES};
+      dwqkv.R = dR1;
       RUN(layer_gemm(dg, dwqkv));
     }
-    RUN(wgrad(l, wg, 0, paired ? 1 : -1));
+    if (!grouped) {
+      RUN(wgrad(l, wg, 0, paired ? 1 : -1));
+    } else if (group_ends && gpos + 1 < gl && d->wgrad_group != NBEST_WGRAD_GROUP_ALWAYS) {
+      stamp(0);
+      RUN(wgrad_launch(l, wg, 3, -1));
+      RUN(wgrad_launch(l, wg, 2, -1));
+      if (!paired) RUN(wgrad_launch(l, wg, 1, -1));
+      RUN(wgrad_launch(l, wg, 0, paired ? 1 : -1));
+      stamp(1);
+    } else {
+      for (int j = 0; j < 4; ++j)
+        if (!skip(l, j)) pend[n_pend++] = wgrad_args_of(wg + j);
+      if (group_ends) {
+        stamp(0);
+        if (n_pend) RUN(nbest_wgrad_group(pend, n_pend, stream));
+        stamp(1);
+        for (int i = 0; i < gpos; ++i) { stamp(0); stamp(1); }
+        n_pend = 0;
+      }
+    }
     if (!npg) RUN(nbest_internal_rowred_batch_flush(st));
   }
   if (!with_embeddings) return NBEST_OK;
diff --git a/n-best-asr-transformer_amd/csrc/gemm.hip b/n-best-asr-transformer_amd/csrc/gemm.hip
--- a/n-best-asr-transformer_amd/csrc/gemm.hip
+++ b/n-best-asr-transformer_amd/csrc/gemm.hip
@@ -119,3 +119,17 @@
   if (int rc = check_bf16(b)) return rc;
   return nbest_wgrad_pair_bf16(a, b, (hipStream_t)stream);
 }
+
+extern "C" int nbest_wgrad_group(const nbest_gemm_args* problems, int n, nbest_stream_t stream) {
+  NB_CHECK(problems && n >= 1 && n <= 8, NBEST_ERR_ARG, "wgrad_group: needs 1 .. 8 problems");
+  for (int i = 0; i < n; ++i) {
+    const nbest_gemm_args* a = problems + i;
+    NB_CHECK(a->A && a->B && a->C, NBEST_ERR_ARG, "wgrad_group: null pointer in problem %d", i);
+    NB_CHECK(a->M > 0 && a->N > 0 && a->K > 0, NBEST_ERR_SHAPE, "wgrad_group: bad shape in problem %d", i);
+    NB_CHECK(a->dtype == NBEST_BF16, NBEST_ERR_DTYPE, "wgrad_group: bf16 operands only");
+    NB_CHECK(a->M % 256 == 0 && a->N % 256 == 0, NBEST_ERR_SHAPE, "wgrad_group: problem %d: %lld x %lld is not a multiple of the 256 x 256 tile", i,
+             (long long)a->M, (long long)a->N);
+    if (int rc = check_bf16(a)) return rc;
+  }
+  return nbest_wgrad_group_bf16(problems, n, (hipStream_t)stream);
+}
diff --git a/n-best-asr-transformer_amd/csrc/gemm_bf16_v2.hip b/n-best-asr-transformer_amd/csrc/gemm_bf16_v2.hip
--- a/n-best-asr-transformer_amd/csrc/gemm_bf16_v2.hip
+++ b/n-best-asr-transformer_amd/csrc/gemm_bf16_v2.hip
@@ -205,7 +205,7 @@
 }
 
 template <int BM, int BN, int WM, int WN, int STAGES, bool TA, bool TB, int EPI>
-__global__ __launch_bounds__(WM * WN * 64, 2) void gemm2_kernel(GemmP2 p) {
+__device__ __forceinline__ void gemm2_body(const GemmP2& p, const int id) {
   extern __shared__ __attribute__((aligned(16))) char lds[];
   constexpr int NT = WM * WN * 64;
   constexpr int WTM = BM / WM, WTN = BN / WN;
@@ -219,8 +219,6 @@
   const int tid = threadIdx.x, lane = tid & 63, wave = tid >> 6;
   const int wm = wave / WN, wn = wave % WN;
 
-  const int nwg = gridDim.x;
-  const int id = xcd_remap(blockIdx.x, nwg);
   const int tiles = p.tiles_m * p.tiles_n;
   const int z = id / tiles, t = id - z * tiles;
   int tile_m, tile_n;
@@ -813,6 +811,44 @@
   }
 }
 
+template <int BM, int BN, int WM, int WN, int STAGES, bool TA, bool TB, int EPI>
+__global__ __launch_bounds__(WM * WN * 64, 2) void gemm2_kernel(GemmP2 p) {
+  gemm2_body<BM, BN, WM, WN, STAGES, TA, TB, EPI>(p, xcd_remap(blockIdx.x, gridDim.x));
+}
+
+constexpr int kMaxGroup = 8;
+struct WgradProb {
+  const bf16* A; const bf16* B; float* C;
+  int64_t lda, ldb, ldc;
+  uint32_t a_bytes, b_bytes;
+  int tiles_m, tiles_n, gn, tile_start;
+};
+struct WgradGroupP {
+  WgradProb pr[kMaxGroup];
+  int64_t K, k_pad;
+  int n, accumulate;
+};
+
+template <int BM, int BN, int WM, int WN, int STAGES, bool TA, bool TB, int EPI>
+__global__ __launch_bounds__(WM * WN * 64, 2) void gemm2_kernel_grouped(WgradGroupP g) {
+  static_assert(BM == 256 && BN == 256 && TA && TB && EPI == NBEST_EPI_F32_SPLITK, "grouped launch: the 256 x 256 weight-gradient program only");
+  const int id = xcd_remap(blockIdx.x, gridDim.x);
+  WgradProb q = g.pr[0];
+#pragma unroll
+  for (int i = 1; i < kMaxGroup; ++i)
+    if (i < g.n && id >= g.pr[i].tile_start) q = g.pr[i];
+  GemmP2 p = {};
+  p.A = q.A; p.B = q.B; p.C = q.C;
+  p.M = (int64_t)q.tiles_m * 256; p.N = (int64_t)q.tiles_n * 256; p.K = g.K;
+  p.lda = q.lda; p.ldb = q.ldb; p.ldc = q.ldc;
+  p.k_per_split = g.k_pad;
+  p.tiles_m = q.tiles_m; p.tiles_n = q.tiles_n; p.splits = 1; p.accumulate = g.accumulate;
+  p.a_bytes = q.a_bytes; p.b_bytes = q.b_bytes;
+  p.stream_out = 1;
+  p.gn = q.gn;
+  gemm2_body<BM, BN, WM, WN, STAGES, TA, TB, EPI>(p, id - q.tile_start);
+}
+
 __global__ __launch_bounds__(256) void pack_b_kernel(const bf16* __restrict__ src, bf16* __restrict__ dst,
                                                      const nbest_matrix_desc* __restrict__ descs, int n) {
   int lo = 0, hi = n - 1;
@@ -1046,6 +1082,35 @@
   return gemm_v2_impl(&v, b, a->M, st);
 }
 
+int nbest_wgrad_group_bf16(const nbest_gemm_args* pr, int n, hipStream_t st) {
+  NB_CHECK(n >= 1 && n <= kMaxGroup, NBEST_ERR_ARG, "wgrad_group: %d problems (1 .. %d)", n, kMaxGroup);
+  WgradGroupP g = {};
+  g.n = n; g.K = pr[0].K; g.k_pad = round_up(pr[0].K, 64); g.accumulate = pr[0].accumulate;
+  int tiles = 0;
+  for (int i = 0; i < n; ++i) {
+    const nbest_gemm_args* a = pr + i;
+    NB_CHECK(a->dtype == NBEST_BF16 && a->trans_a && a->trans_b && a->epilogue == NBEST_EPI_F32_SPLITK, NBEST_ERR_ARG,
+             "wgrad_group: problem %d is not a bf16 weight gradient (trans_a = trans_b = 1, NBEST_EPI_F32_SPLITK)", i);
+    NB_CHECK(a->M % 256 == 0 && a->N % 256 == 0, NBEST_ERR_SHAPE, "wgrad_group: problem %d: %lld x %lld is not a multiple of the 256 x 256 tile", i,
+             (long long)a->M, (long long)a->N);
+    NB_CHECK(a->K == g.K && a->accumulate == g.accumulate, NBEST_ERR_ARG, "wgrad_group: problem %d differs in K or accumulate", i);
+    WgradProb& q = g.pr[i];
+    q.A = (const bf16*)a->A; q.B = (const bf16*)a->B; q.C = (float*)a->C;
+    q.lda = a->lda; q.ldb = a->ldb; q.ldc = a->ldc;
+    q.a_bytes = (uint32_t)(((a->K - 1) * a->lda + a->M) * 2); q.b_bytes = (uint32_t)(((a->K - 1) * a->ldb + a->N) * 2);
+    q.tiles_m = (int)(a->M / 256); q.tiles_n = (int)(a->N / 256);
+    q.gn = (q.tiles_n > q.tiles_m && q.tiles_n % 3 == 0) ? 3 : q.tiles_n;
+    q.tile_start = tiles;
+    tiles += q.tiles_m * q.tiles_n;
+  }
+  constexpr int lds_bytes = 4 * (256 + 256) * BK * 2;
+  const auto kernel = gemm2_kernel_grouped<256, 256, 2, 4, 4, true, true, NBEST_EPI_F32_SPLITK>;
+  (void)hipFuncSetAttribute((const void*)kernel, hipFuncAttributeMaxDynamicSharedMemorySize, lds_bytes);
+  kernel<<<tiles, 512, lds_bytes, st>>>(g);
+  NB_LAUNCH_CHECK();
+  return NBEST_OK;
+}
+
 int nbest_pack_bn_internal(int64_t N) {
   if (N % 256 == 0 && N >= 1024) return 256;
   if (N % 192 == 0) return 192;
diff --git a/n-best-asr-transformer_amd/csrc/internal.h b/n-best-asr-transformer_amd/csrc/internal.h
--- a/n-best-asr-transformer_amd/csrc/internal.h
+++ b/n-best-asr-transformer_amd/csrc/internal.h
@@ -45,6 +45,7 @@
 bool nbest_gemm_bf16_v2_wins(const nbest_gemm_args* a);
 size_t nbest_wgrad_pair_bf16_ws_bytes(const nbest_gemm_args* a, const nbest_gemm_args* b);
 int nbest_wgrad_pair_bf16(const nbest_gemm_args* a, const nbest_gemm_args* b, hipStream_t st);
+int nbest_wgrad_group_bf16(const nbest_gemm_args* problems, int n, hipStream_t st);
 int nbest_pack_bn_internal(int64_t N);
 int nbest_pack_weights_bf16(const void* src, void* dst, const nbest_matrix_desc* descs, int n_matrices, int n_stages, hipStream_t st);
 
diff --git a/n-best-asr-transformer_amd/hipabi.py b/n-best-asr-transformer_amd/hipabi.py
--- a/n-best-asr-transformer_amd/hipabi.py
+++ b/n-best-asr-transformer_amd/hipabi.py
@@ -12,7 +12,7 @@
 
 EXPORTS = [
     "nbest_version", "nbest_last_error", "nbest_embed_ln_fwd", "nbest_embed_ln_bwd", "nbest_embed_bwd_ws_bytes", "nbest_rows_gather", "nbest_rows_zero", "nbest_rows_add",
-    "nbest_gemm_ws_bytes", "nbest_gemm", "nbest_wgrad_pair_ws_bytes", "nbest_wgrad_pair", "nbest_pack_bn", "nbest_pack_weights", "nbest_pack_bn_fp8", "nbest_pack_weights_fp8", "nbest_attention_fwd", "nbest_attention_bwd", "nbest_attention_bwd_ws_bytes", "nbest_attention_keep_bytes", "nbest_attention_fwd_keep", "nbest_attention_bwd_keep", "nbest_layernorm_fwd",
+    "nbest_gemm_ws_bytes", "nbest_gemm", "nbest_wgrad_pair_ws_bytes", "nbest_wgrad_pair", "nbest_wgrad_group", "nbest_pack_bn", "nbest_pack_weights", "nbest_pack_bn_fp8", "nbest_pack_weights_fp8", "nbest_attention_fwd", "nbest_attention_bwd", "nbest_attention_bwd_ws_bytes", "nbest_attention_keep_bytes", "nbest_attention_fwd_keep", "nbest_attention_bwd_keep", "nbest_layernorm_fwd",
     "nbest_layernorm_bwd", "nbest_rowred_ws_bytes", "nbest_colsum", "nbest_heads_ws_bytes", "nbest_stc_heads",
     "nbest_stc_heads_vjp", "nbest_cls_mse", "nbest_cls_grad_scatter", "nbest_stc_decode", "nbest_stream_stamp", "nbest_fp8_amax_fold", "nbest_bertadam_chunk", "nbest_bertadam_step", "nbest_bertadam_norms", "nbest_bertadam_update",
     "nbest_adam_clip_coef", "nbest_adam_update", "nbest_adam_step",
@@ -78,6 +78,7 @@
                 ("word_perm", C.c_void_p), ("aamax_prev", C.c_void_p), ("aamax_new", C.c_void_p), ("fp8_act", C.c_int32), ("pad4", C.c_int32),
                 ("first_trainable", C.c_int32), ("no_input_grad", C.c_int32), ("wgrad_skip_host", C.c_void_p),
                 ("base_ids", C.c_void_p), ("alpha", C.c_void_p), ("no_param_grad", C.c_int32), ("pad5", C.c_int32)]
+    wgrad_group = property(lambda self: self.pad5, lambda self, v: setattr(self, "pad5", int(v)))
 
 
 _lib = None
@@ -107,6 +108,7 @@
         L.nbest_gemm.argtypes = [C.POINTER(GemmArgs), C.c_void_p]
         L.nbest_wgrad_pair_ws_bytes.argtypes = [C.POINTER(GemmArgs), C.POINTER(GemmArgs)]
         L.nbest_wgrad_pair.argtypes = [C.POINTER(GemmArgs), C.POINTER(GemmArgs), C.c_void_p]
+        L.nbest_wgrad_group.argtypes = [C.POINTER(GemmArgs), C.c_int32, C.c_void_p]
         L.nbest_encoder_act_bytes.argtypes = [C.POINTER(EncoderDesc)]
         L.nbest_encoder_ws_bytes.argtypes = [C.POINTER(EncoderDesc)]
         L.nbest_encoder_wgrad_launches_per_layer.argtypes = [C.POINTER(EncoderDesc)]
@@ -298,6 +300,27 @@
     return outs
 
 
+WGRAD_GROUP_PLAN, WGRAD_GROUP_NEVER, WGRAD_GROUP_ALWAYS = 0, 1, 2
+
+
+def wgrad_group(problems, outs=None, accumulate=False):
+    n = len(problems)
+    gs = (GemmArgs * max(n, 1))()
+    res = []
+    for i, (dY, X) in enumerate(problems):
+        M, N = dY.shape[1], X.shape[1]
+        out = outs[i] if outs is not None else torch.empty(M, N, dtype=torch.float32, device=X.device)
+        g = gs[i]
+        g.A, g.B, g.C = dY.data_ptr(), X.data_ptr(), out.data_ptr()
+        g.M, g.N, g.K = M, N, X.shape[0]
+        g.lda, g.ldb, g.ldc = dY.stride(0), X.stride(0), out.stride(0)
+        g.trans_a = g.trans_b = 1
+        g.epilogue, g.dtype, g.accumulate = EPI_F32_SPLITK, dtype_code(X.dtype), int(accumulate)
+        res.append(out)
+    check(lib().nbest_wgrad_group(gs, n, stream_ptr()), "wgrad_group")
+    return res
+
+
 def rows_gather(table, rows, cap):
     H = table.shape[1]
     ids = torch.empty(cap, dtype=torch.long, device=table.device)
diff --git a/n-best-asr-transformer_amd/model.py b/n-best-asr-transformer_amd/model.py
--- a/n-best-asr-transformer_amd/model.py
+++ b/n-best-asr-transformer_amd/model.py
@@ -82,6 +82,7 @@
         d.layers_host = C.cast(a.layer_offsets, C.POINTER(hb.LayerOffsets))
         d.drop_stream_base = 1000 * slot if train else 0
         d.first_trainable = first_trainable
+        d.wgrad_group = model.wgrad_group
         if model.fp8_forward and train:
             d.w8, d.w8_inv_scale = a.w8.data_ptr(), a.w8_inv_scale.data_ptr()
         self.desc = d
@@ -146,11 +147,12 @@
 
 class NBestSTCModel(nn.Module):
     def __init__(self, cfg: EncoderConfig, labels: LabelSpace, device="cuda", compute_dtype=torch.bfloat16, dropout=0.0,
-                 seed=999, fp8_forward=False, fp8_backward=None):
+                 seed=999, fp8_forward=False, fp8_backward=None, wgrad_group=hb.WGRAD_GROUP_PLAN):
         super().__init__()
         self.cfg, self.labels, self.compute_dtype = cfg, labels, compute_dtype
         self.dropout = float(dropout)
         self.device = torch.device(device)
+        self.wgrad_group = int(wgrad_group)
         self.arena = ParamArena(cfg, labels, self.device, compute_dtype)
         self.fp8_forward = bool(fp8_forward)
         self.fp8_backward = self.fp8_forward if fp8_backward is None else bool(fp8_backward)
```

After: 12530, median of 6. +3.8%, better.
